# LinXueyuanStdio/LaTeX_OCR

Measured on AMD Instinct MI355X. Metric: formula-images/sec training step (batch 64, 128x512), higher is better.
Workload: dtype bf16

## Files before the change

### latex_ocr_amd/csrc/decoder_kernels.h

```cpp
#pragma once
#include "lxo_common.h"
struct Slabs { const float* p; int n; long long stride; int ld; };
struct Drop { unsigned thr; float inv_keep; unsigned seed; int t, row0, rows_total; };
struct DetScratch { float* p; size_t floats; };
int lxo_k_det_reduce(const float* part, int nslot, long long stride, int N, float* out, hipStream_t st);
int lxo_k_rowmean(int dt, const void* img, float* mean, int B, int R, int C, hipStream_t st);
int lxo_k_embed_gather(int dt, const float* table, const float* start, const int* formula, void* out, int B, int T, int D, int Dp, int V, hipStream_t st);
int lxo_k_embed_rows(int dt, const float* table, const float* start, const int* ids, void* out, int n, int D, int Dp, int V, hipStream_t st);
int lxo_k_embed_table(int dt, const float* table, const float* start, void* out, int V, int D, int Dp, hipStream_t st);
int lxo_k_lstm_fwd(const float* z, Slabs zs, const float* c_prev, float* gates, float* c_out, float* h_out, float* ht_out, int ldh, Drop dr, int B, int U, hipStream_t st);
int lxo_k_lstm_bwd(const float* gates, const float* c_prev, const float* c_cur, Slabs s1, Slabs s3, Slabs s4, int off4,
                   float* dcc, float* dz, Drop dr, int carry_rows, int B, int U, hipStream_t st);
int lxo_k_tanh_bwd(const float* a, int lda, Slabs carry, const float* o, int ldo, float* g, int ldg, void* gb, int ldgb, Drop dr, int carry_rows, int rows, int cols, hipStream_t st);
int lxo_k_slab_reduce(Slabs sl, float* o, int ldo, int rows, int cols, hipStream_t st);
int lxo_k_tanh_finalize(Slabs sl, float* o, int ldo, Drop dr, int rows, int cols, hipStream_t st);
int lxo_k_attn_fwd(int dt, const void* att_img, const void* img, const float* att_h, Slabs ahs, float* att_h_out, const float* beta, float* alpha, float* part,
                   float* ctx, int ldctx, void* ctxb, int ldcb, int nv, int R, int Rp, int E, int C, int beam, int nch, int rev, hipStream_t st, const void* att_exp = nullptr);
int lxo_k_att_exp(const void* att_img, void* att_exp, long long n, hipStream_t st);
int lxo_k_attn_bwd(int dt, const void* att_img, const void* att_exp, const void* img, const float* att_h, const float* beta, const float* alpha,
                   Slabs dcs, int dcoff, float* dctx_out, int lddc, const float* ctx, int ldctx, float* de, float* datth,
                   int nv, int R, int Rp, int E, int C, int nch, int rev, hipStream_t st);
int lxo_k_datt_img(int dt, const void* att_img, const float* att_h, const float* beta, const float* de, void* dout, float* dbeta,
                   int T, int B, int R, int Rp, int E, DetScratch det, hipStream_t st);
int lxo_k_add_mean_grad(float* dimg, const float* dmean, int B, int R, int C, hipStream_t st);
int lxo_k_ce_loss(int dt, const float* logits, const int* formula, const int* lengths, void* dlogits, float* loss_acc, float inv_ntok,
                  const float* ntok_dev, const unsigned* chain_err, int B, int T, int V, int Vp, DetScratch det, hipStream_t st);
int lxo_k_score(int dt, const float* logits, const int* formula, const int* lengths, float* logp_out, int* top1_out, float* seq_out,
                const unsigned* chain_err, int B, int T, int V, int Vp, hipStream_t st);
int lxo_k_colsum_det(const void* a, int bf16, long long lda, float* out, long long M, int N, DetScratch det, hipStream_t st);
int lxo_k_colsum(const float* a, long long lda, float* out, long long M, int N, DetScratch det, hipStream_t st);
int lxo_k_embed_scatter(const float* demb, const int* formula, float* dtable, float* dstart, int B, int T, int D, int V, int det, hipStream_t st);
int lxo_k_init_bwd(const float* dcc, Slabs dxh, const float* c0, const float* rec0, int ldr, float* dpre, int B, int U, int O, hipStream_t st);
struct DecPrefix { const int* ids; const int* len; int ld; int lim; };
struct DecAllow { const unsigned* bits; int ld; };
int lxo_k_argmax(const float* logits, int Vp, int V, int n, int id_end, int* ids_step, int* ids_out, int max_steps, int step,
                 int* finished, int* n_unfinished, hipStream_t st, float* logp_out = nullptr,
                 const DecPrefix* prefix = nullptr, const DecAllow* allow = nullptr);
int lxo_k_beam_step(float* logits, int Vp, int V, int nimg, int k, int id_end, int time, float div_gamma, float div_prob, int div_seed,
                    float* scratch, float* logp, int* finished,
                    int* ids_step, int* parents_step, int* ids_out, int* par_out, int max_steps, int* n_unfinished, hipStream_t st,
                    float* scores_out = nullptr,
                    const DecPrefix* prefix = nullptr, const DecAllow* allow = nullptr);
int lxo_k_beam_gather(float* rec, int ldr, int XH, float* cs, int U, const int* parents, int k, float* tmp_rec, float* tmp_cs, int n, void* recb, int ldrb, hipStream_t st);
int lxo_k_tile_rows(const float* src, int lds, float* dst, int ldd, int n, int k, int cols, hipStream_t st);
int lxo_k_global_norm_scale(long long n, const float* g, float clip, float* sumsq_tmp, float* out, hipStream_t st);
int lxo_k_chain_guard(const unsigned* err_fwd, const unsigned* err_bwd, const float* probe, float* scale, int have_scale, unsigned* status, hipStream_t st);
int lxo_k_chain_poison(const unsigned* err_fwd, const unsigned* err_bwd, float* probe, hipStream_t st);
int lxo_k_adam(float* p, const float* g, float* m, float* v, long long n, float lr_t, float b1, float b2, float eps, const float* scale, hipStream_t st);
int lxo_k_simple_opt(float* p, const float* g, float* slot, long long n, float lr, int mode, const float* scale, hipStream_t st);
```

### latex_ocr_amd/csrc/decoder_kernels.hip

```cpp
#include "decoder_kernels.h"
#include "api_util.h"
#include "drop.h"
#include <stdlib.h>

namespace {


LXO_DEV void load4(const float* p, float (&v)[4]) {
    f32x4 a = *reinterpret_cast<const f32x4*>(p);
    v[0] = a[0]; v[1] = a[1]; v[2] = a[2]; v[3] = a[3];
}
LXO_DEV void load4(const bf16_t* p, float (&v)[4]) {
    u32x2 a = *reinterpret_cast<const u32x2*>(p);
    v[0] = __uint_as_float(a[0] << 16); v[1] = __uint_as_float(a[0] & 0xffff0000u);
    v[2] = __uint_as_float(a[1] << 16); v[3] = __uint_as_float(a[1] & 0xffff0000u);
}
LXO_DEV void store4(float* p, const float (&v)[4]) { f32x4 a = {v[0], v[1], v[2], v[3]}; *reinterpret_cast<f32x4*>(p) = a; }
LXO_DEV void store4(bf16_t* p, const float (&v)[4]) { u32x2 a = {pack_bf2(v[0], v[1]), pack_bf2(v[2], v[3])}; *reinterpret_cast<u32x2*>(p) = a; }

LXO_DEV float slab_sum(const Slabs& sl, long long row, int col) {
    float v = 0.f;
    const float* q = sl.p + row * sl.ld + col;
    for (int s = 0; s < sl.n; ++s) v += q[(long long)s * sl.stride];
    return v;
// ... 108 lines not shown
        float cp = 0.f;
        if (ok) {
            cp = c_prev[(long long)b * U + u + q];
            const f32x4 zz = *reinterpret_cast<const f32x4*>(z + (long long)b * 4 * U + q * U + u) + slab_sum4(zs, b, q * U + u);
            f32x4 a;
#pragma unroll
            for (int e = 0; e < 4; ++e)
                a[e] = (q == 1) ? tanhf(zz[e]) : sigmoidf_(q == 2 ? zz[e] + 1.0f : zz[e]);
            if (gates) *reinterpret_cast<f32x4*>(gates + (long long)b * 4 * U + q * U + u) = a;
#pragma unroll
            for (int e = 0; e < 4; ++e) act[ugl][q][e] = a[e];
        }
        __syncthreads();
        if (ok) {
            const float gi = act[ugl][0][q], gj = act[ugl][1][q], gf = act[ugl][2][q], go = act[ugl][3][q];
            const float c = gf * cp + gi * gj;
            const float h = go * tanhf(c);
            c_out[(long long)b * U + u + q] = c;
            h_out[(long long)b * ldh + u + q] = h;
            ht_out[(long long)b * ldh + u + q] = h * drop_scale(dr, 1u, b, u + q, U);
        }
        __syncthreads();
    }
}

LXO_DEV f32x4 slab_part4(const Slabs& sl, long long row, int col, int q) {
    f32x4 v = {0.f, 0.f, 0.f, 0.f};
    const float* p = sl.p + row * sl.ld + col;
    for (int s0 = q; s0 < sl.n; s0 += 32) {
        f32x4 t[8];
#pragma unroll
        for (int j = 0; j < 8; ++j) {
            const f32x4 z = {0.f, 0.f, 0.f, 0.f};
            t[j] = (s0 + 4 * j < sl.n) ? *reinterpret_cast<const f32x4*>(p + (long long)(s0 + 4 * j) * sl.stride) : z;
        }
#pragma unroll
        for (int j = 0; j < 8; ++j) v += t[j];
    }
    return v;
}

__global__ __launch_bounds__(256) void lstm_bwd_kernel(const float* __restrict__ gates, const float* __restrict__ c_prev,
                                                      const float* __restrict__ c_cur, Slabs s1, Slabs s3, Slabs s4, int off4,
                                                      float* __restrict__ dcc, float* __restrict__ dz, Drop dr, int carry_rows,
                                                      int B, int U) {
    __shared__ float ex[64][4][8 + 1];
    const int total = B * (U >> 2);
    const int q = threadIdx.x & 3, ugl = threadIdx.x >> 2;
    for (int base = blockIdx.x * 64; base < total; base += gridDim.x * 64) {
        const int ug = base + ugl;
        const bool ok = ug < total;
        const int b = ok ? ug / (U >> 2) : 0, u = ok ? (ug - b * (U >> 2)) << 2 : 0;
        float gi = 0.f, gj = 0.f, gf = 0.f, go = 0.f, cc = 0.f, cp = 0.f, dci = 0.f;
        if (ok) {
            const float* gr = gates + (long long)b * 4 * U + u + q;
            gi = gr[0]; gj = gr[U]; gf = gr[2 * U]; go = gr[3 * U];
            cc = c_cur[(long long)b * U + u + q]; cp = c_prev[(long long)b * U + u + q]; dci = dcc[(long long)b * U + u + q];
            const f32x4 pm = slab_part4(s1, b, u, q) + slab_part4(s3, b, u, q);
            f32x4 pc = {0.f, 0.f, 0.f, 0.f};
            if (b < carry_rows) pc = slab_part4(s4, b, off4 + u, q);
#pragma unroll
            for (int e = 0; e < 4; ++e) { ex[ugl][q][e] = pm[e]; ex[ugl][q][4 + e] = pc[e]; }
        }
        __syncthreads();
        if (ok) {
            const float dhm = ex[ugl][0][q] + ex[ugl][1][q] + ex[ugl][2][q] + ex[ugl][3][q];
            const float dhc = ex[ugl][0][4 + q] + ex[ugl][1][4 + q] + ex[ugl][2][4 + q] + ex[ugl][3][4 + q];
            const float dh = dhm * drop_scale(dr, 1u, b, u + q, U) + dhc;
            const float tc = tanhf(cc);
            const float dc = dci + dh * go * (1.f - tc * tc);
            float* dzr = dz + (long long)b * 4 * U + u + q;
            dzr[0] = dc * gj * gi * (1.f - gi);
            dzr[U] = dc * gi * (1.f - gj * gj);
            dzr[2 * U] = dc * cp * gf * (1.f - gf);
            dzr[3 * U] = dh * tc * go * (1.f - go);
            dcc[(long long)b * U + u + q] = dc * gf;
        }
        __syncthreads();
    }
}

__global__ __launch_bounds__(256) void tanh_bwd_kernel(const float* __restrict__ a, int lda, Slabs carry,
                                                      const float* __restrict__ o, int ldo, float* __restrict__ g, int ldg,
                                                      bf16_t* __restrict__ gb, int ldgb, Drop dr, int carry_rows, int rows, int cols) {
    const int total = rows * (cols >> 2);
    for (int i = blockIdx.x * 256 + threadIdx.x; i < total; i += gridDim.x * 256) {
        const int r = i / (cols >> 2), c = (i - r * (cols >> 2)) << 2;
        const f32x4 ov = *reinterpret_cast<const f32x4*>(o + (long long)r * ldo + c);
        f32x4 d = *reinterpret_cast<const f32x4*>(a + (long long)r * lda + c);
        if (r < carry_rows) d += slab_sum4(carry, r, c);
        f32x4 out;
#pragma unroll
        for (int e = 0; e < 4; ++e) {
            const float sc = drop_scale(dr, 2u, r, c + e, cols);
            const float th = (dr.thr == 0u) ? ov[e] : ov[e] / dr.inv_keep;
            out[e] = d[e] * sc * (1.f - th * th);
        }
        *reinterpret_cast<f32x4*>(g + (long long)r * ldg + c) = out;
        if (gb) { u32x2 pk = {pack_bf2(out[0], out[1]), pack_bf2(out[2], out[3])}; *reinterpret_cast<u32x2*>(gb + (long long)r * ldgb + c) = pk; }
    }
}
__global__ __launch_bounds__(256) void tanh_finalize_kernel(Slabs sl, float* __restrict__ o, int ldo, Drop dr, int rows, int cols) {
    const int total = rows * (cols >> 2);
    for (int i = blockIdx.x * 256 + threadIdx.x; i < total; i += gridDim.x * 256) {
        const int r = i / (cols >> 2), c = (i - r * (cols >> 2)) << 2;
        const f32x4 v = slab_sum4(sl, r, c);
        f32x4 out;
#pragma unroll
        for (int e = 0; e < 4; ++e) out[e] = tanhf(v[e]) * drop_scale(dr, 2u, r, c + e, cols);
        *reinterpret_cast<f32x4*>(o + (long long)r * ldo + c) = out;
    }
}

constexpr int ATT_W = 8;

template <typename CT> LXO_DEV float tanh_ct(float x);
template <> LXO_DEV float tanh_ct<float>(float x) { return tanhf(x); }
template <> LXO_DEV float tanh_ct<bf16_t>(float x) { return 1.f - 2.f * __builtin_amdgcn_rcpf(__expf(2.f * x) + 1.f); }

template <typename CT, int KCT, int ATT_U>
__global__ __launch_bounds__(512) void attn_fwd_part_kernel(const CT* __restrict__ att_img, const CT* __restrict__ img,
                                                           const float* __restrict__ att_h, Slabs ahs, float* __restrict__ att_h_out,
                                                           const float* __restrict__ beta,
                                                           float* __restrict__ alpha, float* __restrict__ part,
                                                           int R, int Rp, int E, int C, int beam, int nch, int rows_per, int rev) {
    __shared__ float redc[ATT_W][512];
    __shared__ float red[2 * ATT_W];
    const int ch = blockIdx.x, v = blockIdx.y, bi = v / beam;
    const int tid = threadIdx.x, lane = tid & 63, wave = tid >> 6;
    const int r0 = ch * rows_per;
    const int n = min(R, r0 + rows_per) - r0;
    const CT* ai = att_img + ((long long)bi * R + r0) * E;
    const CT* im = img + ((long long)bi * R + r0) * C;
    float* pout = part + ((long long)v * nch + ch) * (C + 2);
    constexpr int KC = KCT;
    float ah[KCT][4], bt[KCT][4];
#pragma unroll
    for (int kc = 0; kc < KCT; ++kc) {
        const int k0 = kc * 256 + lane * 4;
#pragma unroll
        for (int j = 0; j < 4; ++j) { ah[kc][j] = 0.f; bt[kc][j] = 0.f; }
        if (kc < KC && k0 < E) {
            const f32x4 a4 = ahs.n > 0 ? slab_sum4(ahs, v, k0) : *reinterpret_cast<const f32x4*>(att_h + (long long)v * E + k0);
            const f32x4 b4 = *reinterpret_cast<const f32x4*>(beta + k0);
#pragma unroll
            for (int j = 0; j < 4; ++j) { ah[kc][j] = a4[j]; bt[kc][j] = b4[j]; }
            if (ahs.n > 0 && att_h_out && ch == 0 && wave == 0) *reinterpret_cast<f32x4*>(att_h_out + (long long)v * E + k0) = a4;
        }
    }
    const int c0 = lane * 8;
    const bool cok = c0 < C;
    float m = -3.0e38f, l = 0.f, acc[8];
#pragma unroll
    for (int e = 0; e < 8; ++e) acc[e] = 0.f;
    const int c0l = cok ? c0 : 0;
    const int nit = n > wave ? (n - wave + ATT_W * ATT_U - 1) / (ATT_W * ATT_U) : 0;
    for (int it = 0; it < nit; ++it) {
        const int base = wave + ATT_W * ATT_U * (rev ? nit - 1 - it : it);
        float xi[ATT_U][8], pt[ATT_U];
#pragma unroll
        for (int u = 0; u < ATT_U; ++u) {
            const int r = min(base + ATT_W * u, n - 1);
            load8(im + (long long)r * C + c0l, xi[u]);
            pt[u] = 0.f;
        }
#pragma unroll
        for (int kc = 0; kc < KCT; ++kc) {
// ... 702 lines not shown
                    const int t = t0 + tt, tc = min(t, T - 1);
                    load4(att_h + ((long long)tc * B + b) * E + k0, a[tt]);
                    f32x4 dq = *reinterpret_cast<const f32x4*>(de + ((long long)tc * B + b) * Rp + rbase);
#pragma unroll
                    for (int rr = 0; rr < 4; ++rr) d[tt][rr] = (t < T && rbase + rr < R) ? dq[rr] : 0.f;
                    if constexpr (is_bf16<CT>::value) {
#pragma unroll
                        for (int j = 0; j < 4; ++j) a[tt][j] = __builtin_amdgcn_exp2f(fminf(fmaxf(a[tt][j] * 2.8853900817779268f, -120.f), 120.f));
                    }
                }
#pragma unroll
                for (int tt = 0; tt < 4; ++tt) {
                    if (d[tt][0] == 0.f && d[tt][1] == 0.f && d[tt][2] == 0.f && d[tt][3] == 0.f) continue;
#pragma unroll
                    for (int rr = 0; rr < 4; ++rr) {
                        const float dd = d[tt][rr];
                        if constexpr (is_bf16<CT>::value) {
                            const f32x2 d4 = {4.f * dd, 4.f * dd}, d2 = {dd, dd}, one = {1.f, 1.f};
                            sumd += dd;
#pragma unroll
                            for (int h = 0; h < 2; ++h) {
                                const f32x2 xs = {x[rr][kc][2 * h], x[rr][kc][2 * h + 1]}, as = {a[tt][2 * h], a[tt][2 * h + 1]};
                                const f32x2 w = __builtin_elementwise_fma(xs, as, one);
                                const f32x2 r = {__builtin_amdgcn_rcpf(w[0]), __builtin_amdgcn_rcpf(w[1])};
                                const f32x2 q = __builtin_elementwise_fma(-r, r, r);
                                f32x2 ac = {acc[rr][kc][2 * h], acc[rr][kc][2 * h + 1]}, dv = {db[kc][2 * h], db[kc][2 * h + 1]};
                                ac = __builtin_elementwise_fma(d4, q, ac);
                                dv = __builtin_elementwise_fma(d2, r, dv);
                                acc[rr][kc][2 * h] = ac[0]; acc[rr][kc][2 * h + 1] = ac[1];
                                db[kc][2 * h] = dv[0]; db[kc][2 * h + 1] = dv[1];
                            }
                        } else {
#pragma unroll
                            for (int j = 0; j < 4; ++j) {
                                const float tau = tanh_ct<CT>(x[rr][kc][j] + a[tt][j]);
                                acc[rr][kc][j] = fmaf(dd, 1.f - tau * tau, acc[rr][kc][j]);
                                db[kc][j] = fmaf(dd, tau, db[kc][j]);
                            }
                        }
                    }
                }
            }
        }
    }
#pragma unroll
    for (int rr = 0; rr < 4; ++rr)
#pragma unroll
        for (int kc = 0; kc < KCT; ++kc) {
            const int k0 = kc * 256 + lane * 4;
            if (rbase + rr < R && kc < KC && k0 < E) {
                float o[4];
#pragma unroll
                for (int j = 0; j < 4; ++j) o[j] = acc[rr][kc][j] * bt[kc][j];
                store4(dout + ((long long)b * R + rbase + rr) * E + k0, o);
            }
        }
#pragma unroll
    for (int kc = 0; kc < KCT; ++kc) {
        const int k0 = kc * 256 + lane * 4;
        if (kc < KC && k0 < E) {
#pragma unroll
            for (int j = 0; j < 4; ++j) redb[wave][k0 + j] = is_bf16<CT>::value ? sumd - 2.f * db[kc][j] : db[kc][j];
        }
    }
    __syncthreads();
    if (dbeta_part) {
        float* slot = dbeta_part + ((long long)blockIdx.y * gridDim.x + blockIdx.x) * E;
        for (int k = tid; k < E; k += 256) slot[k] = redb[0][k] + redb[1][k] + redb[2][k] + redb[3][k];
        return;
    }
    for (int k = tid; k < E; k += 256) atomicAdd(&dbeta[k], redb[0][k] + redb[1][k] + redb[2][k] + redb[3][k]);
}

__global__ __launch_bounds__(256) void add_mean_grad_kernel(float* __restrict__ dimg, const float* __restrict__ dmean, int B, int R, int C) {
    const long long total = (long long)B * R * C;
    const float inv = 1.0f / (float)R;
    for (long long i = (long long)blockIdx.x * 256 + threadIdx.x; i < total; i += (long long)gridDim.x * 256) {
        const int c = (int)(i % C);
        const int b = (int)(i / ((long long)R * C));
        dimg[i] += dmean[(long long)b * C + c] * inv;
    }
}

template <typename CT>
__global__ __launch_bounds__(256) void ce_loss_kernel(const float* __restrict__ logits, const int* __restrict__ formula,
                                                     const int* __restrict__ lengths, CT* __restrict__ dlogits,
                                                     float* __restrict__ loss_acc, float* __restrict__ loss_part, float inv_ntok, const float* __restrict__ ntok_dev,
                                                     const unsigned* __restrict__ chain_err, int B, int T, int V, int Vp) {
    __shared__ float red[8];
    if (chain_err && blockIdx.x == 0 && threadIdx.x == 0 && chain_err[0] != 0u) atomicAdd(&loss_acc[0], __uint_as_float(0x7fc00000u));
    if (ntok_dev) inv_ntok = 1.0f / ntok_dev[0];
    const int lane = threadIdx.x & 63, wave = threadIdx.x >> 6;
    float ce_sum = 0.f, n_sum = 0.f;
    for (int row = blockIdx.x * 4 + wave; row < T * B; row += gridDim.x * 4) {
        const int t = row / B, b = row - t * B;
        const float* lg = logits + (long long)row * Vp;
        CT* dl = dlogits + (long long)row * Vp;
        const bool valid = t < lengths[b];
        int tgt = formula[(long long)b * T + t];
        tgt = tgt < 0 ? 0 : (tgt >= V ? V - 1 : tgt);
        float m = -3.0e38f;
        for (int j = lane; j < V; j += 64) m = fmaxf(m, lg[j]);
        m = wave_max(m);
        float l = 0.f;
        for (int j = lane; j < V; j += 64) l += expf(lg[j] - m);
        l = wave_sum(l);
        const float lse = m + logf(l);
        const float scale = valid ? inv_ntok : 0.f;
        for (int j = lane; j < Vp; j += 64) {
            float g = 0.f;
            if (j < V) g = (expf(lg[j] - lse) - (j == tgt ? 1.f : 0.f)) * scale;
            dl[j] = from_f32<CT>(g);
        }
        if (valid) { ce_sum += lse - lg[tgt]; n_sum += 1.0f; }
    }
    if (lane == 0) { red[wave] = ce_sum; red[4 + wave] = n_sum; }
    __syncthreads();
    if (threadIdx.x == 0) {
        const float c = red[0] + red[1] + red[2] + red[3], n = red[4] + red[5] + red[6] + red[7];
        if (loss_part) { loss_part[2 * blockIdx.x] = c; loss_part[2 * blockIdx.x + 1] = n; }
        else if (n > 0.f) { atomicAdd(&loss_acc[0], c); atomicAdd(&loss_acc[1], n); }
    }
}

template <typename CT, int KV>
__global__ __launch_bounds__(256) void ce_loss_rows_kernel(const float* __restrict__ logits, const int* __restrict__ formula,
                                                          const int* __restrict__ lengths, CT* __restrict__ dlogits,
                                                          float* __restrict__ loss_acc, float* __restrict__ loss_part, float inv_ntok, const float* __restrict__ ntok_dev,
                                                          const unsigned* __restrict__ chain_err, int B, int T, int V, int Vp) {
    __shared__ float red[8];
    if (chain_err && blockIdx.x == 0 && threadIdx.x == 0 && chain_err[0] != 0u) atomicAdd(&loss_acc[0], __uint_as_float(0x7fc00000u));
    if (ntok_dev) inv_ntok = 1.0f / ntok_dev[0];
    const int lane = threadIdx.x & 63, wave = threadIdx.x >> 6;
    float ce_sum = 0.f, n_sum = 0.f;
    for (int row = blockIdx.x * 4 + wave; row < T * B; row += gridDim.x * 4) {
        const int t = row / B, b = row - t * B;
        const float* lg = logits + (long long)row * Vp;
        CT* dl = dlogits + (long long)row * Vp;
        const bool valid = t < lengths[b];
        int tgt = formula[(long long)b * T + t];
        tgt = tgt < 0 ? 0 : (tgt >= V ? V - 1 : tgt);
        const float xt = lg[tgt];
        float x[KV];
#pragma unroll
        for (int q = 0; q < KV / 4; ++q) {
            const int j0 = 4 * (lane + 64 * q);
            const f32x4 v = *reinterpret_cast<const f32x4*>(lg + (j0 < Vp ? j0 : 0));
#pragma unroll
            for (int e = 0; e < 4; ++e) x[4 * q + e] = (j0 + e < V) ? v[e] : -3.0e38f;
        }
        float m = x[0];
#pragma unroll
        for (int e = 1; e < KV; ++e) m = fmaxf(m, x[e]);
        m = wave_max(m);
        float l = 0.f;
#pragma unroll
        for (int e = 0; e < KV; ++e) l += is_bf16<CT>::value ? __expf(x[e] - m) : expf(x[e] - m);
        l = wave_sum(l);
        const float lse = m + logf(l);
        const float scale = valid ? inv_ntok : 0.f;
#pragma unroll
        for (int q = 0; q < KV / 4; ++q) {
            const int j0 = 4 * (lane + 64 * q);
            if (j0 >= Vp) continue;
            float g[4];
#pragma unroll
            for (int e = 0; e < 4; ++e) {
                const int j = j0 + e;
                const float pr = is_bf16<CT>::value ? __expf(x[4 * q + e] - lse) : expf(x[4 * q + e] - lse);
                g[e] = j < V ? (pr - (j == tgt ? 1.f : 0.f)) * scale : 0.f;
            }
            if constexpr (is_bf16<CT>::value) { const u32x2 pk = {pack_bf2(g[0], g[1]), pack_bf2(g[2], g[3])}; *reinterpret_cast<u32x2*>(dl + j0) = pk; }
            else { const f32x4 gv = {g[0], g[1], g[2], g[3]}; *reinterpret_cast<f32x4*>(dl + j0) = gv; }
        }
        if (valid) { ce_sum += lse - xt; n_sum += 1.0f; }
    }
    if (lane == 0) { red[wave] = ce_sum; red[4 + wave] = n_sum; }
    __syncthreads();
    if (threadIdx.x == 0) {
        const float c = red[0] + red[1] + red[2] + red[3], n = red[4] + red[5] + red[6] + red[7];
        if (loss_part) { loss_part[2 * blockIdx.x] = c; loss_part[2 * blockIdx.x + 1] = n; }
        else if (n > 0.f) { atomicAdd(&loss_acc[0], c); atomicAdd(&loss_acc[1], n); }
    }
}

__global__ __launch_bounds__(256) void colsum_kernel(const float* __restrict__ a, int lda, float* __restrict__ out, int M, int N, int rows_per_block) {
    const int n = blockIdx.x * 256 + threadIdx.x;
    const int m0 = blockIdx.y * rows_per_block, m1 = min(M, m0 + rows_per_block);
    if (n >= N) return;
    float s = 0.f;
    for (int m = m0; m < m1; ++m) s += a[(long long)m * lda + n];
    atomicAdd(&out[n], s);
}

__global__ __launch_bounds__(256) void colsum4_kernel(const float* __restrict__ a, int lda, float* __restrict__ out, int M, int N, int rows_per_block) {
    __shared__ f32x4 red[4][64];
    const int cq = threadIdx.x & 63, ry = threadIdx.x >> 6;
    const int n = (blockIdx.x * 64 + cq) * 4;
    const int m0 = blockIdx.y * rows_per_block, m1 = min(M, m0 + rows_per_block);
    const int nl = n < N ? n : 0;
    f32x4 s = {0.f, 0.f, 0.f, 0.f};
    for (int mb = m0 + ry; mb < m1; mb += 32) {
        f32x4 v[8];
#pragma unroll
        for (int u = 0; u < 8; ++u) { const int m = min(mb + 4 * u, m1 - 1); v[u] = *reinterpret_cast<const f32x4*>(a + (long long)m * lda + nl); }
#pragma unroll
        for (int u = 0; u < 8; ++u) if (mb + 4 * u < m1) s += v[u];
    }
    red[ry][cq] = s;
    __syncthreads();
    if (ry == 0 && n < N) {
        const f32x4 t = red[0][cq] + red[1][cq] + red[2][cq] + red[3][cq];
#pragma unroll
        for (int e = 0; e < 4; ++e) atomicAdd(&out[n + e], t[e]);
    }
}


template <typename AT>
__global__ __launch_bounds__(256) void colsum_part_kernel(const AT* __restrict__ a, long long lda, float* __restrict__ part, long long M, int N, int rows_per) {
    const int n = blockIdx.x * 256 + threadIdx.x;
    const long long m0 = (long long)blockIdx.y * rows_per, m1 = m0 + rows_per < M ? m0 + rows_per : M;
    if (n >= N) return;
    float s = 0.f;
    for (long long mb = m0; mb < m1; mb += 8) {
        float v[8];
#pragma unroll
        for (int u = 0; u < 8; ++u) { const long long m = mb + u < m1 ? mb + u : m1 - 1; v[u] = to_f32(a[m * lda + n]); }
#pragma unroll
        for (int u = 0; u < 8; ++u) if (mb + u < m1) s += v[u];
    }
    part[(long long)blockIdx.y * N + n] = s;
}
__global__ __launch_bounds__(256) void det_reduce_kernel(const float* __restrict__ part, int nslot, long long stride, int N, float* __restrict__ out) {
    __shared__ float gs[16][16];
    const int c = threadIdx.x & 15, g = threadIdx.x >> 4;
    const int n = blockIdx.x * 16 + c;
    const int per = (nslot + 15) / 16;
    const int q0 = g * per, q1 = min(nslot, q0 + per);
    float s = 0.f;
    if (n < N) {
        for (int q = q0; q < q1; q += 8) {
            float v[8];
#pragma unroll
            for (int u = 0; u < 8; ++u) v[u] = part[(long long)min(q + u, q1 - 1) * stride + n];
#pragma unroll
            for (int u = 0; u < 8; ++u) if (q + u < q1) s += v[u];
        }
    }
    gs[g][c] = s;
    __syncthreads();
    if (g == 0 && n < N) {
        float tsum = gs[0][c];
#pragma unroll
        for (int k = 1; k < 16; ++k) tsum += gs[k][c];
        out[n] += tsum;
    }
}

__global__ __launch_bounds__(256) void embed_scatter_kernel(const float* __restrict__ demb, const int* __restrict__ formula,
                                                           float* __restrict__ dtable, float* __restrict__ dstart,
                                                           int B, int T, int D, int V) {
    const long long total = (long long)T * B * D;
    for (long long i = (long long)blockIdx.x * 256 + threadIdx.x; i < total; i += (long long)gridDim.x * 256) {
        const int d = (int)(i % D);
        const long long row = i / D;
        const int b = (int)(row % B), t = (int)(row / B);
        const float g = demb[i];
        if (t == 0) atomicAdd(&dstart[d], g);
        else {
            int id = formula[(long long)b * T + t - 1];
            id = id < 0 ? 0 : (id >= V ? V - 1 : id);
            atomicAdd(&dtable[(long long)id * D + d], g);
        }
    }
}

__global__ __launch_bounds__(256) void embed_scatter_rows_kernel(const float* __restrict__ demb, const int* __restrict__ formula,
                                                                float* __restrict__ dtable, float* __restrict__ dstart,
                                                                int B, int T, int D, int V, int det) {
    constexpr int CH = 2048;
    __shared__ int list[CH];
    __shared__ float part[256];
    __shared__ int cnt;
    __shared__ int wcnt[4];
    const int id = blockIdx.x;
    const int tid = threadIdx.x;
    const int rpw = 256 / D, r = tid / D, c = tid - r * D;
    float sum = 0.f;
    const int total = T * B;
    const int per = (total + (int)gridDim.y - 1) / (int)gridDim.y;
    const int s0 = blockIdx.y * per, s1 = min(total, s0 + per);
    for (int base = s0; base < s1; base += CH) {
        if (tid == 0) cnt = 0;
        __syncthreads();
        if (det) {
            for (int jb = base; jb < min(s1, base + CH); jb += 256) {
                const int j = jb + tid;
                int row = -1;
                if (j < min(s1, base + CH)) {
                    const int b = j / T, tt = j - b * T;
                    if (id == V) { if (j < B) row = j; }
                    else if (tt + 1 < T) { int tok = formula[j]; tok = tok < 0 ? 0 : (tok >= V ? V - 1 : tok); if (tok == id) row = (tt + 1) * B + b; }
                }
                const unsigned long long m = __ballot(row >= 0);
                const int lane = tid & 63, wv = tid >> 6;
                if (lane == 0) wcnt[wv] = __builtin_popcountll(m);
                __syncthreads();
                int off = cnt;
                for (int w = 0; w < wv; ++w) off += wcnt[w];
                if (row >= 0) list[off + __builtin_popcountll(m & ((1ull << lane) - 1ull))] = row;
                __syncthreads();
                if (tid == 0) cnt += wcnt[0] + wcnt[1] + wcnt[2] + wcnt[3];
                __syncthreads();
            }
        } else
        for (int j = base + tid; j < min(s1, base + CH); j += 256) {
            const int b = j / T, tt = j - b * T;
            if (id == V) { if (j < B) list[atomicAdd(&cnt, 1)] = j; continue; }
            if (tt + 1 >= T) continue;
            int tok = formula[j]; tok = tok < 0 ? 0 : (tok >= V ? V - 1 : tok);
            if (tok == id) list[atomicAdd(&cnt, 1)] = (tt + 1) * B + b;
        }
        __syncthreads();
        const int n = cnt;
        if (r < rpw) {
            for (int k = r; k < n; k += 4 * rpw) {
                float v[4];
#pragma unroll
                for (int u = 0; u < 4; ++u) { const int kk = min(k + u * rpw, n - 1); v[u] = demb[(long long)list[kk] * D + c]; }
#pragma unroll
                for (int u = 0; u < 4; ++u) if (k + u * rpw < n) sum += v[u];
            }
        }
        __syncthreads();
    }
    part[tid] = (r < rpw) ? sum : 0.f;
    __syncthreads();
    if (tid < D) {
        float t = 0.f;
// ... 555 lines not shown
    const float gn = sqrtf(ss);
    out[1] = gn;
    out[0] = clip > 0.f ? clip / fmaxf(gn, clip) : 1.0f;
}
__global__ void chain_guard_kernel(const unsigned* __restrict__ err_fwd, const unsigned* __restrict__ err_bwd, const float* __restrict__ probe,
                                   float* __restrict__ scale, int have_scale, unsigned* __restrict__ status) {
    const unsigned ef = err_fwd ? err_fwd[0] : 0u, eb = err_bwd ? err_bwd[0] : 0u;
    const float pv = probe ? probe[0] : 0.f;
    const bool drop = (ef | eb) != 0u || pv != pv;
    if (status) { status[0] = ef; status[1] = eb; status[2] = drop ? 1u : 0u; }
    scale[0] = drop ? __uint_as_float(0x7fc00000u) : (have_scale ? scale[0] : 1.0f);
}
__global__ void chain_poison_kernel(const unsigned* __restrict__ err_fwd, const unsigned* __restrict__ err_bwd, float* __restrict__ probe) {
    if ((err_fwd && err_fwd[0]) || (err_bwd && err_bwd[0])) probe[0] = __uint_as_float(0x7fc00000u);
}
__global__ __launch_bounds__(256) void adam_kernel(float* __restrict__ p, const float* __restrict__ g, float* __restrict__ m, float* __restrict__ v,
                                                  long long n, float lr_t, float b1, float b2, float eps, const float* __restrict__ scale) {
    const float sc = scale ? scale[0] : 1.0f;
    if (sc != sc) return;
    for (long long i = (long long)blockIdx.x * 256 + threadIdx.x; i < n; i += (long long)gridDim.x * 256) {
        const float gi = g[i] * sc;
        const float mi = b1 * m[i] + (1.f - b1) * gi;
        const float vi = b2 * v[i] + (1.f - b2) * gi * gi;
        m[i] = mi; v[i] = vi;
        p[i] -= lr_t * mi / (sqrtf(vi) + eps);
    }
}

__global__ __launch_bounds__(256) void simple_opt_kernel(float* __restrict__ p, const float* __restrict__ g, float* __restrict__ slot,
                                                        long long n, float lr, int mode, const float* __restrict__ scale) {
    const float sc = scale ? scale[0] : 1.0f;
    if (sc != sc) return;
    for (long long i = (long long)blockIdx.x * 256 + threadIdx.x; i < n; i += (long long)gridDim.x * 256) {
        const float gi = g[i] * sc;
        if (mode == 1) p[i] -= lr * gi;
        else if (mode == 2) { const float a = slot[i] + gi * gi; slot[i] = a; p[i] -= lr * gi / sqrtf(a); }
        else { const float ms = 0.9f * slot[i] + 0.1f * gi * gi; slot[i] = ms; p[i] -= lr * gi / sqrtf(ms + 1e-10f); }
    }
}

inline int grid1(long long items, int per_block = 256, int cap = 2048) {
    long long g = (items + per_block - 1) / per_block;
    return (int)(g < 1 ? 1 : (g > cap ? cap : g));
}
}

#define LAUNCH(kern, grid, ...) hipLaunchKernelGGL(kern, dim3(grid), dim3(256), 0, st, __VA_ARGS__)
#define BYCT(dt, kern, grid, ...) do { if ((dt) == LXO_BF16) LAUNCH((kern<bf16_t>), grid, __VA_ARGS__); else LAUNCH((kern<float>), grid, __VA_ARGS__); } while (0)
#define DONE return (int)hipGetLastError()

int lxo_k_rowmean(int dt, const void* img, float* mean, int B, int R, int C, hipStream_t st) {
    if (C % 64) return -2;
    if (dt == LXO_BF16) LAUNCH((rowmean_kernel<bf16_t>), dim3(C / 64, B), (const bf16_t*)img, mean, R, C);
    else LAUNCH((rowmean_kernel<float>), dim3(C / 64, B), (const float*)img, mean, R, C);
    DONE;
}
int lxo_k_embed_gather(int dt, const float* table, const float* start, const int* formula, void* out, int B, int T, int D, int Dp, int V, hipStream_t st) {
    const int g = grid1((long long)T * B * Dp);
    if (dt == LXO_BF16) LAUNCH((embed_gather_kernel<bf16_t>), g, table, start, formula, (bf16_t*)out, B, T, D, Dp, V);
    else LAUNCH((embed_gather_kernel<float>), g, table, start, formula, (float*)out, B, T, D, Dp, V);
    DONE;
}
int lxo_k_embed_rows(int dt, const float* table, const float* start, const int* ids, void* out, int n, int D, int Dp, int V, hipStream_t st) {
    const int g = grid1((long long)n * Dp);
    if (dt == LXO_BF16) LAUNCH((embed_rows_kernel<bf16_t>), g, table, start, ids, (bf16_t*)out, n, D, Dp, V);
    else LAUNCH((embed_rows_kernel<float>), g, table, start, ids, (float*)out, n, D, Dp, V);
    DONE;
}
int lxo_k_embed_table(int dt, const float* table, const float* start, void* out, int V, int D, int Dp, hipStream_t st) {
    const int g = grid1((long long)(V + 1) * Dp);
    if (dt == LXO_BF16) LAUNCH((embed_table_kernel<bf16_t>), g, table, start, (bf16_t*)out, V, D, Dp);
    else LAUNCH((embed_table_kernel<float>), g, table, start, (float*)out, V, D, Dp);
    DONE;
}
int lxo_k_lstm_fwd(const float* z, Slabs zs, const float* c_prev, float* gates, float* c_out, float* h_out, float* ht_out, int ldh, Drop dr, int B, int U, hipStream_t st) {
    LAUNCH(lstm_fwd_kernel, grid1((long long)B * U), z, zs, c_prev, gates, c_out, h_out, ht_out, ldh, dr, B, U);
    DONE;
}
int lxo_k_lstm_bwd(const float* gates, const float* c_prev, const float* c_cur, Slabs s1, Slabs s3, Slabs s4, int off4,
                   float* dcc, float* dz, Drop dr, int carry_rows, int B, int U, hipStream_t st) {
    LAUNCH(lstm_bwd_kernel, grid1((long long)B * U), gates, c_prev, c_cur, s1, s3, s4, off4, dcc, dz, dr, carry_rows, B, U);
    DONE;
}
int lxo_k_tanh_bwd(const float* a, int lda, Slabs carry, const float* o, int ldo, float* g, int ldg, void* gb, int ldgb, Drop dr, int carry_rows, int rows, int cols, hipStream_t st) {
    LAUNCH(tanh_bwd_kernel, grid1((long long)rows * cols / 4), a, lda, carry, o, ldo, g, ldg, (bf16_t*)gb, ldgb, dr, carry_rows, rows, cols);
    DONE;
}
__global__ __launch_bounds__(256) static void slab_reduce_kernel(Slabs sl, float* __restrict__ o, int ldo, int rows, int cols) {
    const int total = rows * (cols >> 2);
    for (int i = blockIdx.x * 256 + threadIdx.x; i < total; i += gridDim.x * 256) {
        const int r = i / (cols >> 2), c = (i - r * (cols >> 2)) << 2;
        *reinterpret_cast<f32x4*>(o + (long long)r * ldo + c) = slab_sum4(sl, r, c);
    }
}
int lxo_k_slab_reduce(Slabs sl, float* o, int ldo, int rows, int cols, hipStream_t st) {
    LAUNCH(slab_reduce_kernel, grid1((long long)rows * cols / 4), sl, o, ldo, rows, cols);
    DONE;
}
int lxo_k_tanh_finalize(Slabs sl, float* o, int ldo, Drop dr, int rows, int cols, hipStream_t st) {
    LAUNCH(tanh_finalize_kernel, grid1((long long)rows * cols / 4), sl, o, ldo, dr, rows, cols);
    DONE;
}
static int att_u(int rows_per) {
    static int forced = -1;
    if (forced < 0) { const char* e = getenv("LXO_ATT_U"); forced = e ? atoi(e) : 0; }
    if (forced == 7 || forced == 8) return forced;
    return (rows_per + 55) / 56 <= (rows_per + 63) / 64 ? 7 : 8;
}
int lxo_k_attn_fwd(int dt, const void* att_img, const void* img, const float* att_h, Slabs ahs, float* att_h_out, const float* beta, float* alpha, float* part,
                   float* ctx, int ldctx, void* ctxb, int ldcb, int nv, int R, int Rp, int E, int C, int beam, int nch, int rev, hipStream_t st, const void* att_exp) {
    if (E > 1024 || C > 512 || nch < 1 || nch > 32) return -2;
    const int rows_per = cdiv(R, nch);
    dim3 grid(nch, nv);
    static int split = -1;
    if (split < 0) { const char* e = getenv("LXO_ATT_SPLIT"); split = (e && e[0] == '1') ? 1 : 0; }
    const int epl = dt == LXO_BF16 ? 8 : 4;
    if (split && ahs.n == 0 && att_h && R <= 1024 && C % 64 == 0 && E % epl == 0 && E <= 64 * epl && ((E / epl) & (E / epl - 1)) == 0) {
        if (dt == LXO_BF16) {
            hipLaunchKernelGGL((attn_scores_kernel<bf16_t, 8>), grid, dim3(512), 0, st, (const bf16_t*)att_img, att_h, beta, part, R, Rp, E, beam, rows_per);
            hipLaunchKernelGGL((attn_ctx_kernel<bf16_t, 8>), dim3(C / 64, nv), dim3(512), 0, st, (const bf16_t*)img, part, alpha, ctx, ldctx, (bf16_t*)ctxb, ldcb, R, Rp, C, beam);
        } else {
            hipLaunchKernelGGL((attn_scores_kernel<float, 8>), grid, dim3(512), 0, st, (const float*)att_img, att_h, beta, part, R, Rp, E, beam, rows_per);
            hipLaunchKernelGGL((attn_ctx_kernel<float, 8>), dim3(C / 64, nv), dim3(512), 0, st, (const float*)img, part, alpha, ctx, ldctx, (bf16_t*)ctxb, ldcb, R, Rp, C, beam);
        }
        DONE;
    }
    static int beam_shared = -1;
    if (beam_shared < 0) { const char* e = getenv("LXO_ATT_BEAM_SHARED"); beam_shared = (e && e[0] == '0') ? 0 : 1; }
    if (beam_shared && (beam == 2 || beam == 3 || beam == 5 || (beam == 1 && att_exp && dt == LXO_BF16)) && ahs.n == 0 && att_h && E <= 256 && C <= 512 && nv % beam == 0) {
        const int nimg = nv / beam;
        int nb = cdiv(512, nimg);
        if (nb > 16) nb = 16;
        const int by_rows = R / 32 > 0 ? R / 32 : 1;
        if (nb > by_rows) nb = by_rows;
        const int need = cdiv(R, 1024);
        if (nb < need) nb = need;
        const int rpb = cdiv(R, nb);
        const dim3 gb(nb, nimg);
#define ABM(CT_, U_, NB_, X_, OCC_, AI_) hipLaunchKernelGGL((attn_fwd_part_beam_kernel<CT_, U_, NB_, X_, OCC_>), gb, dim3(512), 0, st, (const CT_*)(AI_), (const CT_*)img, att_h, beta, alpha, part, R, Rp, E, C, nb, rpb, rev)
        if (dt == LXO_BF16 && att_exp) { if (beam == 1) ABM(bf16_t, 4, 1, true, 4, att_exp); else if (beam == 2) ABM(bf16_t, 4, 2, true, 4, att_exp); else if (beam == 3) ABM(bf16_t, 4, 3, true, 4, att_exp); else ABM(bf16_t, 2, 5, true, 4, att_exp); }
        else if (dt == LXO_BF16) { if (beam == 2) ABM(bf16_t, 4, 2, false, 2, att_img); else if (beam == 3) ABM(bf16_t, 4, 3, false, 2, att_img); else ABM(bf16_t, 4, 5, false, 2, att_img); }
        else { if (beam == 2) ABM(float, 4, 2, false, 2, att_img); else if (beam == 3) ABM(float, 4, 3, false, 2, att_img); else ABM(float, 4, 5, false, 2, att_img); }
#undef ABM
        hipLaunchKernelGGL(attn_fwd_combine_kernel, dim3(4, nv), dim3(256), 0, st, part, alpha, ctx, ldctx, (bf16_t*)ctxb, ldcb, R, Rp, C, nb, rpb);
        DONE;
    }
#define AF_ARGS att_h, ahs, att_h_out, beta, alpha, part, R, Rp, E, C, beam, nch, rows_per, rev
    if (dt == LXO_BF16) {
        if (E <= 256) { if (att_u(rows_per) == 8) hipLaunchKernelGGL((attn_fwd_part_kernel<bf16_t, 1, 8>), grid, dim3(512), 0, st, (const bf16_t*)att_img, (const bf16_t*)img, AF_ARGS); else hipLaunchKernelGGL((attn_fwd_part_kernel<bf16_t, 1, 7>), grid, dim3(512), 0, st, (const bf16_t*)att_img, (const bf16_t*)img, AF_ARGS); }
        else { if (att_u(rows_per) == 8) hipLaunchKernelGGL((attn_fwd_part_kernel<bf16_t, 4, 8>), grid, dim3(512), 0, st, (const bf16_t*)att_img, (const bf16_t*)img, AF_ARGS); else hipLaunchKernelGGL((attn_fwd_part_kernel<bf16_t, 4, 7>), grid, dim3(512), 0, st, (const bf16_t*)att_img, (const bf16_t*)img, AF_ARGS); }
    } else {
        if (E <= 256) { if (att_u(rows_per) == 8) hipLaunchKernelGGL((attn_fwd_part_kernel<float, 1, 8>), grid, dim3(512), 0, st, (const float*)att_img, (const float*)img, AF_ARGS); else hipLaunchKernelGGL((attn_fwd_part_kernel<float, 1, 7>), grid, dim3(512), 0, st, (const float*)att_img, (const float*)img, AF_ARGS); }
        else { if (att_u(rows_per) == 8) hipLaunchKernelGGL((attn_fwd_part_kernel<float, 4, 8>), grid, dim3(512), 0, st, (const float*)att_img, (const float*)img, AF_ARGS); else hipLaunchKernelGGL((attn_fwd_part_kernel<float, 4, 7>), grid, dim3(512), 0, st, (const float*)att_img, (const float*)img, AF_ARGS); }
    }
#undef AF_ARGS
    hipLaunchKernelGGL(attn_fwd_combine_kernel, dim3(4, nv), dim3(256), 0, st, part, alpha, ctx, ldctx, (bf16_t*)ctxb, ldcb, R, Rp, C, nch, rows_per);
    DONE;
}
int lxo_k_att_exp(const void* att_img, void* att_exp, long long n, hipStream_t st) {
    if (n % 8) return -2;
    LAUNCH(att_exp_kernel, grid1(n / 8, 256, 4096), (const bf16_t*)att_img, (bf16_t*)att_exp, n / 8);
    DONE;
}
int lxo_k_attn_bwd(int dt, const void* att_img, const void* att_exp, const void* img, const float* att_h, const float* beta, const float* alpha,
                   Slabs dcs, int dcoff, float* dctx_out, int lddc, const float* ctx, int ldctx, float* de, float* datth,
                   int nv, int R, int Rp, int E, int C, int nch, int rev, hipStream_t st) {
    if (E > 1024 || C > 512 || nch < 1 || nch > 32) return -2;
    const int rows_per = cdiv(R, nch);
    dim3 grid(nch, nv);
    static int stream2 = -1;
    if (stream2 < 0) { const char* e = getenv("LXO_ATT_BWD2"); stream2 = (e && e[0] == '1') ? 1 : 0; }
    if (stream2 && dt == LXO_BF16 && E == 256 && C == 512 && dcs.n == 1 && lddc % 4 == 0 && ldctx % 4 == 0 && (long long)rows_per * 1024 < (1LL << 31)) {
        const float* dctx = dcs.p + dcoff;
        if (dctx_out) return -2;
        hipLaunchKernelGGL((attn_bwd_stream_kernel<4>), grid, dim3(512), 0, st, (const bf16_t*)att_img, (const bf16_t*)img, att_h, beta, alpha, dctx, dcs.ld,
                           ctx, ldctx, de, datth, R, Rp, rows_per, rev);
        DONE;
    }
#define AB_ARGS att_h, beta, alpha, dcs, dcoff, dctx_out, lddc, ctx, ldctx, de, datth, R, Rp, E, C, rows_per, rev
    if (dt == LXO_BF16 && att_exp && E <= 256) {
        if (att_u(rows_per) == 8) hipLaunchKernelGGL((attn_bwd_part_kernel<bf16_t, 1, 8, true>), grid, dim3(512), 0, st, (const bf16_t*)att_exp, (const bf16_t*)img, AB_ARGS);
        else hipLaunchKernelGGL((attn_bwd_part_kernel<bf16_t, 1, 7, true>), grid, dim3(512), 0, st, (const bf16_t*)att_exp, (const bf16_t*)img, AB_ARGS);
    } else if (dt == LXO_BF16) {
        if (E <= 256) { if (att_u(rows_per) == 8) hipLaunchKernelGGL((attn_bwd_part_kernel<bf16_t, 1, 8>), grid, dim3(512), 0, st, (const bf16_t*)att_img, (const bf16_t*)img, AB_ARGS); else hipLaunchKernelGGL((attn_bwd_part_kernel<bf16_t, 1, 7>), grid, dim3(512), 0, st, (const bf16_t*)att_img, (const bf16_t*)img, AB_ARGS); }
        else { if (att_u(rows_per) == 8) hipLaunchKernelGGL((attn_bwd_part_kernel<bf16_t, 4, 8>), grid, dim3(512), 0, st, (const bf16_t*)att_img, (const bf16_t*)img, AB_ARGS); else hipLaunchKernelGGL((attn_bwd_part_kernel<bf16_t, 4, 7>), grid, dim3(512), 0, st, (const bf16_t*)att_img, (const bf16_t*)img, AB_ARGS); }
    } else {
        if (E <= 256) { if (att_u(rows_per) == 8) hipLaunchKernelGGL((attn_bwd_part_kernel<float, 1, 8>), grid, dim3(512), 0, st, (const float*)att_img, (const float*)img, AB_ARGS); else hipLaunchKernelGGL((attn_bwd_part_kernel<float, 1, 7>), grid, dim3(512), 0, st, (const float*)att_img, (const float*)img, AB_ARGS); }
        else { if (att_u(rows_per) == 8) hipLaunchKernelGGL((attn_bwd_part_kernel<float, 4, 8>), grid, dim3(512), 0, st, (const float*)att_img, (const float*)img, AB_ARGS); else hipLaunchKernelGGL((attn_bwd_part_kernel<float, 4, 7>), grid, dim3(512), 0, st, (const float*)att_img, (const float*)img, AB_ARGS); }
    }
#undef AB_ARGS
    DONE;
}
int lxo_k_det_reduce(const float* part, int nslot, long long stride, int N, float* out, hipStream_t st) {
    if (nslot <= 0 || N <= 0) return 0;
    hipLaunchKernelGGL(det_reduce_kernel, dim3(cdiv(N, 16)), dim3(256), 0, st, part, nslot, stride, N, out);
    DONE;
}
int lxo_k_datt_img(int dt, const void* att_img, const float* att_h, const float* beta, const float* de, void* dout, float* dbeta,
                   int T, int B, int R, int Rp, int E, DetScratch det, hipStream_t st) {
    dim3 grid(cdiv(R, 16), B);
    if (E > 1024) return -2;
    float* part = nullptr;
    if (det.p) { if ((size_t)grid.x * grid.y * E > det.floats) return -6; part = det.p; }
    if (dt == LXO_BF16) {
        if (E <= 256) hipLaunchKernelGGL((datt_img_kernel<bf16_t, 1>), grid, dim3(256), 0, st, (const bf16_t*)att_img, att_h, beta, de, (bf16_t*)dout, dbeta, part, T, B, R, Rp, E);
        else hipLaunchKernelGGL((datt_img_kernel<bf16_t, 4>), grid, dim3(256), 0, st, (const bf16_t*)att_img, att_h, beta, de, (bf16_t*)dout, dbeta, part, T, B, R, Rp, E);
    } else {
        if (E <= 256) hipLaunchKernelGGL((datt_img_kernel<float, 1>), grid, dim3(256), 0, st, (const float*)att_img, att_h, beta, de, (float*)dout, dbeta, part, T, B, R, Rp, E);
        else hipLaunchKernelGGL((datt_img_kernel<float, 4>), grid, dim3(256), 0, st, (const float*)att_img, att_h, beta, de, (float*)dout, dbeta, part, T, B, R, Rp, E);
    }
    if (part) return lxo_k_det_reduce(part, (int)(grid.x * grid.y), E, E, dbeta, st);
    DONE;
}
int lxo_k_add_mean_grad(float* dimg, const float* dmean, int B, int R, int C, hipStream_t st) {
    LAUNCH(add_mean_grad_kernel, grid1((long long)B * R * C), dimg, dmean, B, R, C);
    DONE;
}
int lxo_k_ce_loss(int dt, const float* logits, const int* formula, const int* lengths, void* dlogits, float* loss_acc, float inv_ntok,
                  const float* ntok_dev, const unsigned* chain_err, int B, int T, int V, int Vp, DetScratch det, hipStream_t st) {
    int g = cdiv(T * B, 4);
    float* part = (det.p && det.floats >= 1024) ? det.p : nullptr;
    if (Vp % 4 == 0 && Vp <= 1024 && (((uintptr_t)logits | (uintptr_t)dlogits) & 15) == 0) {
        if (g > (part ? 512 : 2048)) g = part ? 512 : 2048;
#define CE_ROWS(CT_, KV_) LAUNCH((ce_loss_rows_kernel<CT_, KV_>), g, logits, formula, lengths, (CT_*)dlogits, loss_acc, part, inv_ntok, ntok_dev, chain_err, B, T, V, Vp)
        if (dt == LXO_BF16) { if (Vp <= 256) CE_ROWS(bf16_t, 4); else if (Vp <= 512) CE_ROWS(bf16_t, 8); else CE_ROWS(bf16_t, 16); }
        else { if (Vp <= 256) CE_ROWS(float, 4); else if (Vp <= 512) CE_ROWS(float, 8); else CE_ROWS(float, 16); }
#undef CE_ROWS
        if (part) return lxo_k_det_reduce(part, g, 2, 2, loss_acc, st);
        DONE;
    }
    if (g > 512) g = 512;
    if (dt == LXO_BF16) LAUNCH((ce_loss_kernel<bf16_t>), g, logits, formula, lengths, (bf16_t*)dlogits, loss_acc, part, inv_ntok, ntok_dev, chain_err, B, T, V, Vp);
    else LAUNCH((ce_loss_kernel<float>), g, logits, formula, lengths, (float*)dlogits, loss_acc, part, inv_ntok, ntok_dev, chain_err, B, T, V, Vp);
    if (part) return lxo_k_det_reduce(part, g, 2, 2, loss_acc, st);
    DONE;
}
int lxo_k_score(int dt, const float* logits, const int* formula, const int* lengths, float* logp_out, int* top1_out, float* seq_out,
                const unsigned* chain_err, int B, int T, int V, int Vp, hipStream_t st) {
    int g = cdiv(T * B, 4);
    if (Vp % 4 == 0 && Vp <= 1024 && ((uintptr_t)logits & 15) == 0) {
        if (g > 2048) g = 2048;
#define SC_ROWS(BF_, KV_) LAUNCH((score_rows_kernel<BF_, KV_>), g, logits, formula, lengths, logp_out, top1_out, chain_err, B, T, V, Vp)
        if (dt == LXO_BF16) { if (Vp <= 256) SC_ROWS(true, 4); else if (Vp <= 512) SC_ROWS(true, 8); else SC_ROWS(true, 16); }
        else { if (Vp <= 256) SC_ROWS(false, 4); else if (Vp <= 512) SC_ROWS(false, 8); else SC_ROWS(false, 16); }
#undef SC_ROWS
    } else {
        LAUNCH(score_kernel, g > 512 ? 512 : g, logits, formula, lengths, logp_out, top1_out, chain_err, B, T, V, Vp);
    }
    if (seq_out) LAUNCH(score_seq_kernel, cdiv(B, 256), logp_out, lengths, seq_out, chain_err, B, T);
    DONE;
}
int lxo_k_colsum_det(const void* a, int bf16, long long lda, float* out, long long M, int N, DetScratch det, hipStream_t st) {
    if (!det.p) return -6;
    if (M <= 0 || N <= 0) return 0;
    long long maxslots = (long long)(det.floats / (size_t)N);
    if (maxslots < 1) return -6;
    if (maxslots > 1024) maxslots = 1024;
    long long rows_per = (M + maxslots - 1) / maxslots;
    if (rows_per < 64) rows_per = 64;
    const int nrb = (int)((M + rows_per - 1) / rows_per);
    if (bf16) hipLaunchKernelGGL((colsum_part_kernel<bf16_t>), dim3(cdiv(N, 256), nrb), dim3(256), 0, st, (const bf16_t*)a, lda, det.p, M, N, (int)rows_per);
    else hipLaunchKernelGGL((colsum_part_kernel<float>), dim3(cdiv(N, 256), nrb), dim3(256), 0, st, (const float*)a, lda, det.p, M, N, (int)rows_per);
    return lxo_k_det_reduce(det.p, nrb, N, N, out, st);
}
int lxo_k_colsum(const float* a, long long lda, float* out, long long M, int N, DetScratch det, hipStream_t st) {
    if (det.p) return lxo_k_colsum_det(a, 0, lda, out, M, N, det, st);
    const int rpb = 64;
    if (N % 4 == 0 && lda % 4 == 0 && ((uintptr_t)a & 15) == 0 && M > 0)
        hipLaunchKernelGGL(colsum4_kernel, dim3(cdiv(N, 256), cdiv((int)M, rpb)), dim3(256), 0, st, a, (int)lda, out, (int)M, N, rpb);
    else
    hipLaunchKernelGGL(colsum_kernel, dim3(cdiv(N, 256), cdiv((int)M, rpb)), dim3(256), 0, st, a, (int)lda, out, (int)M, N, rpb);
    DONE;
}
int lxo_k_embed_scatter(const float* demb, const int* formula, float* dtable, float* dstart, int B, int T, int D, int V, int det, hipStream_t st) {
    if (D <= 256) { hipLaunchKernelGGL(embed_scatter_rows_kernel, dim3(V + 1, det ? 1 : 16), dim3(256), 0, st, demb, formula, dtable, dstart, B, T, D, V, det); DONE; }
    if (det) return -2;
    LAUNCH(embed_scatter_kernel, grid1((long long)T * B * D), demb, formula, dtable, dstart, B, T, D, V);
    DONE;
}
int lxo_k_init_bwd(const float* dcc, Slabs dxh, const float* c0, const float* rec0, int ldr, float* dpre, int B, int U, int O, hipStream_t st) {
    LAUNCH(init_bwd_kernel, grid1((long long)B * (2 * U + O)), dcc, dxh, c0, rec0, ldr, dpre, B, U, O);
    DONE;
}
#define DEC_VARIANT(KERNEL, grid, block, ...)                                                                         \
    do {                                                                                                               \
        if (prefix && allow) hipLaunchKernelGGL((KERNEL<true, true>), dim3(grid), dim3(block), 0, st, __VA_ARGS__);    \
        else if (prefix) hipLaunchKernelGGL((KERNEL<true, false>), dim3(grid), dim3(block), 0, st, __VA_ARGS__);       \
        else if (allow) hipLaunchKernelGGL((KERNEL<false, true>), dim3(grid), dim3(block), 0, st, __VA_ARGS__);        \
        else hipLaunchKernelGGL((KERNEL<false, false>), dim3(grid), dim3(block), 0, st, __VA_ARGS__);                  \
    } while (0)
int lxo_k_argmax(const float* logits, int Vp, int V, int n, int id_end, int* ids_step, int* ids_out, int max_steps, int step,
                 int* finished, int* n_unfinished, hipStream_t st, float* logp_out, const DecPrefix* prefix, const DecAllow* allow) {
    const DecPrefix pf = prefix ? *prefix : DecPrefix{};
    const DecAllow al = allow ? *allow : DecAllow{};
    DEC_VARIANT(argmax_kernel, cdiv(n, 4), 256, logits, Vp, V, n, id_end, ids_step, ids_out, max_steps, step, finished, n_unfinished, logp_out, pf, al);
    DONE;
}
int lxo_k_beam_step(float* logits, int Vp, int V, int nimg, int k, int id_end, int time, float div_gamma, float div_prob, int div_seed,
                    float* scratch, float* logp, int* finished,
                    int* ids_step, int* parents_step, int* ids_out, int* par_out, int max_steps, int* n_unfinished, hipStream_t st,
                    float* scores_out, const DecPrefix* prefix, const DecAllow* allow) {
    if (k > 16 || k > V) return -2;
    DivPen dp = {0.f, 0u, (unsigned)div_seed, scratch};
    if (div_gamma > 0.f && div_gamma != 1.f && div_prob > 0.f) {
        dp.log_gamma = logf(div_gamma);
        dp.thr = div_prob >= 1.f ? 16777216u : (unsigned)(div_prob * 16777216.0f);
    }
    static int fast = -1;
    if (fast < 0) { const char* e = getenv("LXO_BEAM_FAST"); fast = (e && e[0] == '0') ? 0 : 1; }
    const DecPrefix pf = prefix ? *prefix : DecPrefix{};
    const DecAllow al = allow ? *allow : DecAllow{};
    if (fast && dp.log_gamma == 0.f && (long long)k * V <= BS_TH * BS_NPT && k * BS_NW <= 64) {
        DEC_VARIANT(beam_step_fast_kernel, nimg, BS_TH, logits, Vp, V, k, id_end, time, logp, finished, ids_step, parents_step, ids_out, par_out, max_steps, n_unfinished, scores_out, pf, al);
    } else
        DEC_VARIANT(beam_step_kernel, nimg, 256, logits, Vp, V, k, id_end, time, dp, logp, finished, ids_step, parents_step, ids_out, par_out, max_steps, n_unfinished, scores_out, pf, al);
    DONE;
}
// ... 37 lines not shown
```

### latex_ocr_amd/csrc/model_decoder.hip

```cpp
#include "plan.h"
#include "impl.h"
#include "gemm.h"
#include "decoder_kernels.h"
#include "rstep.h"
#include "xdec.h"
#include "dimg.h"
#include "api_util.h"
#include "timing.h"

namespace {
int nt(const Plan& P, bool a_f32, bool c_f32, bool small, const void* A, int lda, const void* Bp, int ldb, void* C, int ldc,
       int M, int N, int K, const float* bias, int act, bool accumulate, hipStream_t st) {
    GemmNT g; memset(&g, 0, sizeof(g));
    g.A = A; g.Bp = Bp; g.C = C; g.M = M; g.N = N; g.K = K; g.lda = lda; g.ldb = ldb; g.ldc = ldc;
    g.bias = bias; g.act = act; g.alpha = 1.f; g.accumulate = accumulate ? 1 : 0; g.addend_rows = 1;
    if (P.s.dtype == LXO_F32) { a_f32 = true; c_f32 = true; }
    return lxo_launch_gemm_nt(P.s.dtype, a_f32, c_f32, small, g, st);
}
int tn(const Plan& P, bool a_f32, bool b_f32, const void* A, int lda, const void* B, int ldb, float* C, int ldc,
       int M, int I, int J, hipStream_t st, DetScratch det = DetScratch{nullptr, 0}) {
    GemmTN g; memset(&g, 0, sizeof(g));
    g.A = A; g.B = B; g.C = C; g.M = M; g.I = I; g.J = J; g.lda = lda; g.ldb = ldb; g.ldc = ldc;
    const int tiles = cdiv(I, 128) * cdiv(J, 128);
    int ns = cdiv(512, tiles);
    const int maxs = M / 64 > 0 ? M / 64 : 1;
    if (ns > maxs) ns = maxs;
    g.nsplit = ns < 1 ? 1 : ns; g.nbatch = 1; g.atomic = 1;
    if (P.bf && P.det()) { if (det.p) { g.det_slab = det.p; g.det_floats = det.floats; } else g.nsplit = 1; }
    if (P.s.dtype == LXO_F32) { a_f32 = true; b_f32 = true; }
    return lxo_launch_gemm_tn(P.s.dtype, a_f32, b_f32, g, st);
}
int slab(const Plan& P, const float* A, int lda, const void* Bp, int ldb, float* out, int M, int N, int K, hipStream_t st) {
    GemmNT g; memset(&g, 0, sizeof(g));
    g.A = A; g.Bp = Bp; g.M = M; g.N = N; g.K = K; g.lda = lda; g.ldb = ldb; g.ldc = N; g.alpha = 1.f; g.addend_rows = 1;
    return lxo_launch_gemm_slab(P.s.dtype, g, out, (long long)M * N, st);
}
Slabs view(const float* p, int K, int M, int N) { Slabs s = {p, K / 128, (long long)M * N, N}; return s; }
const Slabs kNoSlabs = {nullptr, 0, 0, 0};
}

static bool att_alternate() {
    static int v = -1;
    if (v < 0) { const char* e = getenv("LXO_ATT_ALT"); v = (e && atoi(e) == 0) ? 0 : 1; }
    return v == 1;
}
static bool fused_steps(const Plan& P);
static int rs_dense(const Plan& P, const float* A, int lda, const void* W, int ldw, float* out, int ldo, int M, int N, int K,
                    const float* bias, bool tanh_act, bool accumulate, hipStream_t st) {
    RStep a; memset(&a, 0, sizeof(a));
    a.M = M; a.N = N; a.K = K; a.U = P.s.U; a.O = P.s.O; a.zx_row = -1;
    a.A = A; a.lda = lda; a.W = W; a.ldw = ldw; a.out = out; a.ldo = ldo; a.bias = bias; a.accumulate = accumulate ? 1 : 0;
    a.epi = tanh_act ? RS_TANH_O : RS_PLAIN;
    a.dr.inv_keep = 1.f;
    return lxo_launch_rstep(P.s.dtype, 0, a, st);
}

static int attention_prepare(const Plan& P, const float* prm, const void* wp, void* ws, int beam, hipStream_t st) {
    const int B = P.s.B, C = P.s.C, E = P.s.E, U = P.s.U, O = P.s.O;
    RC(nt(P, false, false, false, P.ws<void>(ws, W_IMG), C, P.pk(wp, K_ATT_IMG_T), C, P.ws<void>(ws, W_ATT_IMG), E,
          B * P.R, E, C, nullptr, 0, false, st));
    RC(lxo_k_rowmean(P.s.dtype, P.ws<void>(ws, W_IMG), P.ws<float>(ws, W_MEAN), B, P.R, C, st));
    float* rec0 = P.ws<float>(ws, W_REC);
    float* cs0 = P.ws<float>(ws, W_CS);
    const char* wt = (const char*)P.pk(wp, K_INIT_T);
    float* mean = P.ws<float>(ws, W_MEAN);
    if (beam <= 1 && fused_steps(P)) {
        RC(rs_dense(P, mean, C, wt, C, cs0, U, B, U, C, prm + P.poff[P_BC0], true, false, st));
        RC(rs_dense(P, mean, C, wt + (size_t)U * C * P.esz, C, rec0 + O, P.REC, B, U, C, prm + P.poff[P_BH0], true, false, st));
        RC(rs_dense(P, mean, C, wt + (size_t)2 * U * C * P.esz, C, rec0, P.REC, B, O, C, prm + P.poff[P_BO0], true, false, st));
    } else if (beam <= 1) {
        RC(nt(P, true, true, true, mean, C, wt, C, cs0, U, B, U, C, prm + P.poff[P_BC0], 2, false, st));
        RC(nt(P, true, true, true, mean, C, wt + (size_t)U * C * P.esz, C, rec0 + O, P.REC, B, U, C, prm + P.poff[P_BH0], 2, false, st));
        RC(nt(P, true, true, true, mean, C, wt + (size_t)2 * U * C * P.esz, C, rec0, P.REC, B, O, C, prm + P.poff[P_BO0], 2, false, st));
    } else {
        float* tmp = P.ws<float>(ws, W_BEAM_TMP);
        float* tc = tmp; float* th = tmp + (size_t)B * U; float* to = th + (size_t)B * U;
        RC(nt(P, true, true, true, mean, C, wt, C, tc, U, B, U, C, prm + P.poff[P_BC0], 2, false, st));
        RC(nt(P, true, true, true, mean, C, wt + (size_t)U * C * P.esz, C, th, U, B, U, C, prm + P.poff[P_BH0], 2, false, st));
        RC(nt(P, true, true, true, mean, C, wt + (size_t)2 * U * C * P.esz, C, to, O, B, O, C, prm + P.poff[P_BO0], 2, false, st));
        RC(lxo_k_tile_rows(tc, U, cs0, U, B * beam, beam, U, st));
        RC(lxo_k_tile_rows(th, U, rec0 + O, P.REC, B * beam, beam, U, st));
        RC(lxo_k_tile_rows(to, O, rec0, P.REC, B * beam, beam, O, st));
    }
    return 0;
}

static thread_local hipStream_t g_side = nullptr;
static thread_local hipEvent_t g_ev_fork = nullptr, g_ev_join = nullptr;
int lxo_impl_set_side_stream(hipStream_t s) {
    g_side = s;
    if (s && !g_ev_fork) {
        HIPRC(hipEventCreateWithFlags(&g_ev_fork, hipEventDisableTiming));
        HIPRC(hipEventCreateWithFlags(&g_ev_join, hipEventDisableTiming));
    }
    return 0;
}
static int fork_side(hipStream_t st) { HIPRC(hipEventRecord(g_ev_fork, st)); HIPRC(hipStreamWaitEvent(g_side, g_ev_fork, 0)); return 0; }
static int join_side(hipStream_t st) { HIPRC(hipEventRecord(g_ev_join, g_side)); HIPRC(hipStreamWaitEvent(st, g_ev_join, 0)); return 0; }

static int cell_step(const Plan& P, const float* prm, const void* wp, void* ws, int r0, int nr, int beam,
                     const float* zx_t, const float* rec_prev, const float* cs_prev, float* rec_cur, float* cs_cur,
                     float* gates_t, float* atth_t, float* alpha_t, Drop dr, hipStream_t st) {
    const int C = P.s.C, E = P.s.E, U = P.s.U, O = P.s.O;
    const size_t r = (size_t)r0;
    float* s1 = P.ws<float>(ws, W_S_K1) + r * (P.XH / 128) * 4 * U;
    float* s2 = P.ws<float>(ws, W_S_K2) + r * (U / 128) * E;
    float* s4 = P.ws<float>(ws, W_S_K4) + r * (P.HC / 128) * O;
    zx_t += r * 4 * U; rec_prev += r * P.REC; cs_prev += r * U; rec_cur += r * P.REC; cs_cur += r * U;
    if (gates_t) gates_t += r * 4 * U;
    atth_t += r * E; alpha_t += r * P.Rp;
    const char* att_img = (const char*)P.ws<void>(ws, W_ATT_IMG) + (r / beam) * P.R * E * P.esz;
    const char* img = (const char*)P.ws<void>(ws, W_IMG) + (r / beam) * P.R * C * P.esz;
    float* part = P.ws<float>(ws, W_APART) + r * 32 * (C + 2);
    RC(slab(P, rec_prev, P.REC, P.pk(wp, K_LSTM_RT), P.ldRT, s1, nr, 4 * U, P.XH, st));
    RC(lxo_k_lstm_fwd(zx_t, view(s1, P.XH, nr, 4 * U), cs_prev, gates_t, cs_cur, rec_cur + O, rec_cur + P.OFF_HT, P.REC, dr, nr, U, st));
    RC(slab(P, rec_cur + P.OFF_HT, P.REC, P.pk(wp, K_ATT_H_T), P.ldAHT, s2, nr, E, U, st));
    RC(lxo_k_attn_fwd(P.s.dtype, att_img, img, nullptr, view(s2, U, nr, E), atth_t,
                      prm + P.poff[P_BETA], alpha_t, part, rec_cur + P.OFF_CTX, P.REC, nullptr, 0, nr, P.R, P.Rp, E, C, beam,
                      P.attn_chunks(nr), 0, st));
    RC(slab(P, rec_cur + P.OFF_HT, P.REC, P.pk(wp, K_OW_T), P.ldOWT, s4, nr, O, P.HC, st));
    RC(lxo_k_tanh_finalize(view(s4, P.HC, nr, O), rec_cur, P.REC, dr, nr, O, st));
    return 0;
}

static int cell_step_fused(const Plan& P, const float* prm, const void* wp, void* ws, int nr, int beam,
                           const float* zx_t, const float* rec_prev, const float* cs_prev, float* rec_cur, float* cs_cur,
                           const bf16_t* recb_prev, bf16_t* recb_cur,
                           float* gates_t, float* atth_t, float* alpha_t, Drop dr, hipStream_t st,
                           const int* zx_idx = nullptr, int zx_row = -1, const int* a_par = nullptr) {
    const int C = P.s.C, E = P.s.E, U = P.s.U, O = P.s.O;
    const bool bf = P.bf;
    const char* att_img = (const char*)P.ws<void>(ws, W_ATT_IMG);
    const char* img = (const char*)P.ws<void>(ws, W_IMG);
    float* part = P.ws<float>(ws, W_APART);
    RStep a; memset(&a, 0, sizeof(a));
    a.M = nr; a.U = U; a.O = O; a.dr = dr; a.zx_row = -1;
    RStep k1 = a;
    k1.A = bf ? (const void*)recb_prev : (const void*)rec_prev; k1.lda = bf ? P.RECB : P.REC;
    k1.W = P.pk(wp, K_LSTM_RT); k1.ldw = P.ldRT; k1.N = 4 * U; k1.K = P.XH; k1.epi = RS_LSTM_FWD;
    k1.zx = zx_t; k1.c_prev = cs_prev; k1.gates = gates_t; k1.c_out = cs_cur;
    k1.zx_idx = zx_idx; k1.zx_vocab = P.s.V; k1.zx_row = zx_row;
    k1.a_par = a_par; k1.a_k = beam;
    k1.out = rec_cur + O; k1.out2 = rec_cur + P.OFF_HT; k1.ldo = P.REC;
    if (bf) { k1.outb = recb_cur + O; k1.out2b = recb_cur + P.OFF_HT; k1.ldob = P.RECB; }
    RC(lxo_launch_rstep(P.s.dtype, bf, k1, st));
    RStep k2 = a;
    k2.A = bf ? (const void*)(recb_cur + P.OFF_HT) : (const void*)(rec_cur + P.OFF_HT); k2.lda = bf ? P.RECB : P.REC;
    k2.W = P.pk(wp, K_ATT_H_T); k2.ldw = P.ldAHT; k2.N = E; k2.K = U; k2.epi = RS_PLAIN;
    k2.out = atth_t; k2.ldo = E;
// ... 22 lines not shown
}
static bool fused_steps(const Plan& P) {
    if (P.s.step_kernels == 1) return false;
    const int ks[7] = {P.XH, P.s.U, P.HC, P.s.O, P.s.E, 4 * P.s.U, P.s.C};
    for (int k : ks) if (!rstep_k_ok(k, P.bf) || !rstep_k_ok(k, false)) return false;
    return true;
}
static int mirror_oh(const Plan& P, void* ws, size_t slot_rows, int rows, hipStream_t st) {
    if (!P.bf) return 0;
    return lxo_k_mirror(P.ws<float>(ws, W_REC) + slot_rows * P.REC, P.REC, P.ws<bf16_t>(ws, W_RECB) + slot_rows * P.RECB, P.RECB, rows, P.XH, st);
}

int lxo_impl_decoder_train_fwd(const Plan& P, const float* prm, const void* wp, void* ws, const int* formula, hipStream_t st) {
    const int B = P.s.B, T = P.s.T, U = P.s.U, O = P.s.O, E = P.s.E, D = P.s.D, V = P.s.V, C = P.s.C;
    RC(attention_prepare(P, prm, wp, ws, 1, st));
    if (P.att_exp()) RC(lxo_k_att_exp(P.ws<void>(ws, W_ATT_IMG), P.ws<void>(ws, W_ATT_EXP), (long long)B * P.R * E, st));
    RC(lxo_k_embed_gather(P.s.dtype, prm + P.poff[P_EMB], prm + P.poff[P_START], formula, P.ws<void>(ws, W_EMB_IN), B, T, D, P.Dp, V, st));
    float* zx = P.ws<float>(ws, W_ZX);
    RC(nt(P, false, true, false, P.ws<void>(ws, W_EMB_IN), P.Dp, P.pk(wp, K_LSTM_XT), P.Dp, zx, 4 * U, T * B, 4 * U, P.Dp,
          prm + P.poff[P_LSTM_B], 0, false, st));
    float* rec = P.ws<float>(ws, W_REC); float* cs = P.ws<float>(ws, W_CS);
    const bool dual = g_side != nullptr && B >= 2 && (B % 2) == 0;
    const int nh = dual ? 2 : 1;
    const bool fused = fused_steps(P) && !dual;
    bool chain_done = false;
    if (fused && P.bf && P.s.step_kernels == 0) {
        RC(mirror_oh(P, ws, 0, B, st));
        XDecFwd x; memset(&x, 0, sizeof(x));
        x.Wrt = (const bf16_t*)P.pk(wp, K_LSTM_RT); x.ldrt = P.ldRT;
        x.Wah = (const bf16_t*)P.pk(wp, K_ATT_H_T); x.ldah = P.ldAHT;
        x.Wow = (const bf16_t*)P.pk(wp, K_OW_T); x.ldow = P.ldOWT;
        x.beta = prm + P.poff[P_BETA];
        x.att_img = P.ws<bf16_t>(ws, W_ATT_IMG); x.img = P.ws<bf16_t>(ws, W_IMG);
        x.att_exp = P.att_exp() ? P.ws<bf16_t>(ws, W_ATT_EXP) : nullptr;
        x.zx = zx; x.rec = rec; x.recb = P.ws<bf16_t>(ws, W_RECB); x.cs = cs;
        x.gates = P.ws<float>(ws, W_GATES); x.atth = P.ws<float>(ws, W_ATTH); x.alpha = P.ws<float>(ws, W_ALPHA);
        x.part = P.ws<float>(ws, W_APART); x.sync = P.ws<unsigned>(ws, W_XSYNC);
        x.T = T; x.B = B; x.R = P.R; x.Rp = P.Rp; x.REC = P.REC; x.RECB = P.RECB;
        x.dr = P.drop(0, 0);
        LxoTimed tm("xdec_fwd", "chain", (double)T * B * P.R * (E + C) * P.esz, st);
        const int rc = lxo_launch_xdec_fwd(x, U, O, C, E, st);
        if (rc == 0) chain_done = true;
        else if (rc != -2) return rc < 0 ? rc : -rc;
    }
    if (P.bf && !chain_done) HIPRC(hipMemsetAsync(P.ws<unsigned>(ws, W_XSYNC), 0, kXDecSyncBytes, st));
    if (fused && !chain_done) {
        bf16_t* recb = P.ws<bf16_t>(ws, W_RECB);
        RC(mirror_oh(P, ws, 0, B, st));
        for (int t = 0; t < T; ++t) {
            const int nr = B;
            if (nr <= 0) break;
            RC(cell_step_fused(P, prm, wp, ws, nr, 1, zx + (size_t)t * B * 4 * U,
                               rec + (size_t)t * B * P.REC, cs + (size_t)t * B * U,
                               rec + (size_t)(t + 1) * B * P.REC, cs + (size_t)(t + 1) * B * U,
                               recb + (size_t)t * B * P.RECB, recb + (size_t)(t + 1) * B * P.RECB,
                               P.ws<float>(ws, W_GATES) + (size_t)t * B * 4 * U,
                               P.ws<float>(ws, W_ATTH) + (size_t)t * B * E,
                               P.ws<float>(ws, W_ALPHA) + (size_t)t * B * P.Rp, P.drop(t, 0), st));
        }
    }
    if (dual) RC(fork_side(st));
    for (int t = 0; t < T && !fused; ++t)
        for (int h = 0; h < nh; ++h) {
            const int hb = B / nh;
            if (hb <= 0) continue;
            RC(cell_step(P, prm, wp, ws, h * hb, hb, 1, zx + (size_t)t * B * 4 * U,
                         rec + (size_t)t * B * P.REC, cs + (size_t)t * B * U,
                         rec + (size_t)(t + 1) * B * P.REC, cs + (size_t)(t + 1) * B * U,
                         P.ws<float>(ws, W_GATES) + (size_t)t * B * 4 * U,
                         P.ws<float>(ws, W_ATTH) + (size_t)t * B * E,
                         P.ws<float>(ws, W_ALPHA) + (size_t)t * B * P.Rp, P.drop(t, h * hb), h ? g_side : st));
        }
    if (dual) RC(join_side(st));
    if (P.bf && fused)
        RC(nt(P, false, true, false, P.ws<bf16_t>(ws, W_RECB) + (size_t)B * P.RECB, P.RECB, P.pk(wp, K_YWO_T), O, P.ws<float>(ws, W_LOGITS), P.Vp,
              T * B, V, O, nullptr, 0, false, st));
    else
        RC(nt(P, true, true, false, rec + (size_t)B * P.REC, P.REC, P.pk(wp, K_YWO_T), O, P.ws<float>(ws, W_LOGITS), P.Vp,
              T * B, V, O, nullptr, 0, false, st));
    return 0;
}

int lxo_impl_ce_loss(const Plan& P, void* ws, const int* formula, const int* lengths, float inv_ntok, const float* ntok_dev, hipStream_t st) {
    HIPRC(hipMemsetAsync(P.ws<float>(ws, W_LOSS), 0, 64, st));
    RC(lxo_k_ce_loss(P.s.dtype, P.ws<float>(ws, W_LOGITS), formula, lengths, P.ws<void>(ws, W_DLOGITS), P.ws<float>(ws, W_LOSS),
                     inv_ntok, ntok_dev, P.bf ? P.ws<unsigned>(ws, W_XSYNC) + 8 * 64 : nullptr, P.s.B, P.s.T, P.s.V, P.Vp,
                     DetScratch{P.ws<float>(ws, W_DET), P.wbytes[W_DET] / 4}, st));
    return 0;
}

int lxo_impl_score_tokens(const Plan& P, void* ws, const int* formula, const int* lengths, float* logp_out, int* top1_out, float* seq_out, hipStream_t st) {
    return lxo_k_score(P.s.dtype, P.ws<float>(ws, W_LOGITS), formula, lengths, logp_out, top1_out, seq_out,
                       P.bf ? P.ws<unsigned>(ws, W_XSYNC) + 8 * 64 : nullptr, P.s.B, P.s.T, P.s.V, P.Vp, st);
}

hipStream_t lxo_impl_encoder_side_stream();
static thread_local hipEvent_t g_dbw_fork = nullptr, g_dbw_fork2 = nullptr, g_dbw_join = nullptr, g_dbw_init = nullptr;

int lxo_impl_decoder_train_bwd(const Plan& P, const float* prm, const void* wp, void* ws, const int* formula, float* grads,
                               int parts, hipStream_t st, bool defer_join, void* ready) {
    const int B = P.s.B, T = P.s.T, C = P.s.C, E = P.s.E, U = P.s.U, O = P.s.O, D = P.s.D, V = P.s.V;
    const int TB = T * B;
    auto gw = [&](int pid) { return grads + P.poff[pid]; };
    float* rec = P.ws<float>(ws, W_REC); float* cs = P.ws<float>(ws, W_CS);
    float* dolog = P.ws<float>(ws, W_DOLOG); float* gall = P.ws<float>(ws, W_G); float* dhc = P.ws<float>(ws, W_DHC);
    float* de = P.ws<float>(ws, W_DE); float* datth = P.ws<float>(ws, W_DATTH); float* dz = P.ws<float>(ws, W_DZ);
    float* dcc = P.ws<float>(ws, W_DCC);
    float* gates = P.ws<float>(ws, W_GATES); float* atth = P.ws<float>(ws, W_ATTH); float* alpha = P.ws<float>(ws, W_ALPHA);
    const void* dlog = P.ws<void>(ws, W_DLOGITS);
    const DetScratch det = P.det_scratch(ws);

    const bool dual = g_side != nullptr && B >= 2 && (B % 2) == 0;
    const bool fused = fused_steps(P) && !dual;
    if (parts & 1) {
        RC(nt(P, false, true, false, dlog, P.Vp, P.pk(wp, K_YWO), P.Vp, dolog, O, TB, O, P.Vp, nullptr, 0, false, st));
        if (P.bf && fused) RC(tn(P, false, false, P.ws<bf16_t>(ws, W_RECB) + (size_t)B * P.RECB, P.RECB, dlog, P.Vp, gw(P_YWO), V, TB, O, V, st, det));
        else RC(tn(P, true, false, rec + (size_t)B * P.REC, P.REC, dlog, P.Vp, gw(P_YWO), V, TB, O, V, st));
    }
    if ((parts & 1) && P.bf) RC(lxo_k_chain_poison(P.ws<unsigned>(ws, W_XSYNC) + 8 * 64, nullptr, grads + P.ptotal - 1, st));
    if (!(parts & 2)) return 0;

    const bool want_chain = fused && P.bf && P.s.step_kernels == 0;
    bool bwd_chain = false;
    auto zero_acc = [&]() -> int {
        HIPRC(hipMemsetAsync(dcc, 0, (size_t)B * U * 4, st));
        HIPRC(hipMemsetAsync(datth, 0, (size_t)TB * E * 4, st));
        return 0;
    };
    if (!want_chain) RC(zero_acc());
    if (P.bf && !want_chain) HIPRC(hipMemsetAsync(P.ws<unsigned>(ws, W_XSYNC) + kXDecBlockBytes / 4, 0, kXDecSyncBytes, st));
    const int nh = dual ? 2 : 1;
    float* dxh = P.ws<float>(ws, W_DXH);
    if (fused) {
        const bool bf = P.bf;
        bf16_t* gb = P.ws<bf16_t>(ws, W_GB); bf16_t* dzb = P.ws<bf16_t>(ws, W_DZB);
        float* carry_h = P.ws<float>(ws, W_CARRYH);
        const char* att_img = (const char*)P.ws<void>(ws, W_ATT_IMG);
        const char* img = (const char*)P.ws<void>(ws, W_IMG);
        const int t_last = T - 1, n_last = B;
        RC(lxo_k_tanh_bwd(dolog + (size_t)t_last * B * O, O, kNoSlabs, rec + (size_t)(t_last + 1) * B * P.REC, P.REC,
                          gall + (size_t)t_last * B * O, O, bf ? gb + (size_t)t_last * B * P.GBP : nullptr, P.GBP, P.drop(t_last, 0), 0, n_last, O, st));
        bool chain_done = false;
        if (want_chain) {
            XDecBwd x; memset(&x, 0, sizeof(x));
            x.Wow = (const bf16_t*)P.pk(wp, K_OW); x.ldow = P.ldOW;
            x.Wah = (const bf16_t*)P.pk(wp, K_ATT_H); x.ldah = P.ldAH;
            x.Wk = (const bf16_t*)P.pk(wp, K_LSTM) + (size_t)D * P.ldK; x.ldk = P.ldK;
            x.beta = prm + P.poff[P_BETA];
            x.att_img = (const bf16_t*)att_img; x.img = (const bf16_t*)img;
            x.att_exp = P.att_exp() ? P.ws<bf16_t>(ws, W_ATT_EXP) : nullptr;
            x.rec = rec; x.REC = P.REC; x.cs = cs; x.gates = gates; x.atth = atth; x.alpha = alpha; x.Rp = P.Rp;
            x.dolog = dolog; x.gall = gall; x.gb = gb; x.GBP = P.GBP; x.dhc = dhc; x.de = de; x.datth = datth; x.datthb = P.ws<bf16_t>(ws, W_DATTHB);
            x.dz = dz; x.dzb = dzb; x.DZBP = P.DZBP; x.carry_h = carry_h; x.dcc = dcc; x.dxh = dxh;
            x.part = P.ws<float>(ws, W_APART);
            x.sync = P.ws<unsigned>(ws, W_XSYNC) + kXDecBlockBytes / 4;
            x.T = T; x.B = B; x.R = P.R;
            x.dr = P.drop(0, 0);
            LxoTimed tm("xdec_bwd", "chain", (double)T * B * P.R * (E + C) * P.esz, st);
            const int rc = lxo_launch_xdec_bwd(x, U, O, C, E, st);
            if (rc == 0) chain_done = bwd_chain = true;
            else if (rc != -2) return rc < 0 ? rc : -rc;
            else { RC(zero_acc()); HIPRC(hipMemsetAsync(x.sync, 0, kXDecSyncBytes, st)); }
        }
        RStep a; memset(&a, 0, sizeof(a));
        a.U = U; a.O = O; a.zx_row = -1;
        for (int t = t_last; t >= 0 && !chain_done; --t) {
            const int nr = B;
            const int nchb = P.det() ? 1 : P.attn_chunks(nr);
            a.M = nr;
            const float* rec_cur = rec + (size_t)(t + 1) * B * P.REC;
            float* g_t = gall + (size_t)t * B * O;
            float* dhc_t = dhc + (size_t)t * B * P.HC;
            float* datth_t = datth + (size_t)t * B * E;
            float* dz_t = dz + (size_t)t * B * 4 * U;
            RStep b1 = a;
            b1.A = bf ? (const void*)(gb + (size_t)t * B * P.GBP) : (const void*)g_t; b1.lda = bf ? P.GBP : O;
            b1.W = P.pk(wp, K_OW); b1.ldw = P.ldOW; b1.N = P.HC; b1.K = O; b1.epi = RS_PLAIN;
            b1.out = dhc_t; b1.ldo = P.HC;
            RC(lxo_launch_rstep(P.s.dtype, bf, b1, st));
            const Slabs dc1 = {dhc_t, 1, 0, P.HC};
            {
            LxoTimed tm("attn_bwd", "part", (double)nr * P.R * (E + C) * P.esz, st);
            RC(lxo_k_attn_bwd(P.s.dtype, att_img, P.att_exp() ? P.ws<void>(ws, W_ATT_EXP) : nullptr, img, atth + (size_t)t * B * E, prm + P.poff[P_BETA],
                              alpha + (size_t)t * B * P.Rp, dc1, U, nullptr, P.HC, rec_cur + P.OFF_CTX, P.REC,
                              de + (size_t)t * B * P.Rp, datth_t, nr, P.R, P.Rp, E, C, nchb, att_alternate() ? (t & 1) : 0, st));
            }
            RStep b3 = a;
            b3.A = datth_t; b3.lda = E;
            b3.W = P.pk(wp, K_ATT_H); b3.ldw = P.ldAH; b3.N = U; b3.K = E; b3.epi = RS_LSTM_BWD;
            b3.dhm = dhc_t; b3.lddhm = P.HC; b3.carry_h = carry_h; b3.carry_rows = (t == t_last) ? 0 : B;
            b3.gates_in = gates + (size_t)t * B * 4 * U; b3.c_prev = cs + (size_t)t * B * U; b3.c_cur = cs + (size_t)(t + 1) * B * U;
            b3.dcc = dcc; b3.out = dz_t; b3.outb = bf ? dzb + (size_t)t * B * P.DZBP : nullptr; b3.ldob = P.DZBP; b3.dr = P.drop(t, 0);
            RC(lxo_launch_rstep(P.s.dtype, 0, b3, st));
            RStep b4 = a;
            b4.A = bf ? (const void*)(dzb + (size_t)t * B * P.DZBP) : (const void*)dz_t; b4.lda = bf ? P.DZBP : 4 * U;
            b4.W = (const char*)P.pk(wp, K_LSTM) + (size_t)D * P.ldK * P.esz; b4.ldw = P.ldK; b4.N = P.XH; b4.K = 4 * U; b4.epi = RS_CARRY;
            if (t == 0) { b4.first = 1; b4.out = dxh; b4.ldo = P.XH; }
            else {
                b4.M = B;
                b4.out = gall + (size_t)(t - 1) * B * O; b4.outb = bf ? gb + (size_t)(t - 1) * B * P.GBP : nullptr; b4.ldob = P.GBP; b4.out2 = carry_h;
                b4.dolog = dolog + (size_t)(t - 1) * B * O; b4.o_prev = rec + (size_t)t * B * P.REC; b4.ldoprev = P.REC;
                b4.dr = P.drop(t - 1, 0);
            }
            RC(lxo_launch_rstep(P.s.dtype, bf, b4, st));
        }
    }
    if (dual) RC(fork_side(st));
    for (int t = T - 1; t >= 0 && !fused; --t) {
        for (int h = 0; h < nh; ++h) {
            const int hb = B / nh;
            if (hb <= 0) continue;
            const int crows = (t == T - 1) ? 0 : hb;
            const int nchb = P.det() ? 1 : P.attn_chunks(hb);
            hipStream_t sh = h ? g_side : st;
            const size_t r0 = (size_t)h * hb;
            float* sb1 = P.ws<float>(ws, W_S_B1) + r0 * (O / 128) * P.HC;
            float* sb3 = P.ws<float>(ws, W_S_B3) + r0 * (E / 128) * U;
            float* sb4 = P.ws<float>(ws, W_S_B4) + r0 * (4 * U / 128) * P.XH;
            const float* rec_cur = rec + ((size_t)(t + 1) * B + r0) * P.REC;
            float* g_t = gall + ((size_t)t * B + r0) * O;
            float* dhc_t = dhc + ((size_t)t * B + r0) * P.HC;
            const char* att_img = (const char*)P.ws<void>(ws, W_ATT_IMG) + r0 * P.R * E * P.esz;
            const char* img = (const char*)P.ws<void>(ws, W_IMG) + r0 * P.R * C * P.esz;
            const Slabs carry = (crows <= 0) ? kNoSlabs : view(sb4, 4 * U, crows, P.XH);
// ... 397 lines not shown
```

### latex_ocr_amd/csrc/rstep.h

```cpp
#pragma once
#include "lxo_common.h"
#include "decoder_kernels.h"

enum RStepEpi {
    RS_PLAIN = 0,
    RS_TANH_O = 1,
    RS_LSTM_FWD = 2,
    RS_LSTM_BWD = 3,
    RS_CARRY = 4,
};

struct RStep {
    const void* A; int lda;
    const void* W; int ldw;
    int M, N, K, epi;
    int U, O;
    float* out; int ldo;
    bf16_t* outb; int ldob;
    float* out2; bf16_t* out2b;
    const float* zx; const float* c_prev; float* gates; float* c_out;
    const int* a_par; int a_k;
    const int* zx_idx; int zx_vocab, zx_row;
    const float* dhm; int lddhm; const float* carry_h; const float* gates_in; const float* c_cur; float* dcc; int carry_rows;
    const float* bias; int accumulate;
    const float* dolog; const float* o_prev; int ldoprev; int first;
    Drop dr;
    unsigned long long* dbg;
};

int lxo_launch_rstep(int dt, int a_bf16, const RStep& p, hipStream_t st);
#include "lxo_debug.h"
int lxo_k_mirror(const float* src, int lds, void* dst, int ldd, int rows, int cols, hipStream_t st);
```

### latex_ocr_amd/csrc/rstep.hip

```cpp
#include "rstep.h"
#include "drop.h"
#include "api_util.h"

namespace {

typedef __attribute__((ext_vector_type(4))) float v4f;

LXO_DEV v4f mfma16_bf16(u32x4 a, u32x4 b, v4f c) {
    return __builtin_amdgcn_mfma_f32_16x16x32_bf16(__builtin_bit_cast(bf16x8_t, a), __builtin_bit_cast(bf16x8_t, b), c, 0, 0, 0);
}

template <bool FAST> LXO_DEV float tanh_e(float x) {
    if constexpr (FAST) return 1.f - 2.f * __builtin_amdgcn_rcpf(__builtin_amdgcn_exp2f(x * 2.8853900817779268f) + 1.f);
    else return tanhf(x);
}
template <bool FAST> LXO_DEV float sigm_e(float x) {
    if constexpr (FAST) return __builtin_amdgcn_rcpf(1.f + __builtin_amdgcn_exp2f(x * -1.4426950408889634f));
    else return sigmoidf_(x);
}

LXO_DEV u32x4 frag8(const bf16_t* p) { return *reinterpret_cast<const u32x4*>(p); }
LXO_DEV u32x4 frag8(const float* p) {
    const f32x4 a = *reinterpret_cast<const f32x4*>(p), b = *reinterpret_cast<const f32x4*>(p + 4);
    u32x4 r = {pack_bf2(a[0], a[1]), pack_bf2(a[2], a[3]), pack_bf2(b[0], b[1]), pack_bf2(b[2], b[3])};
    return r;
}

LXO_DEV void st4(float* p, const float (&v)[4]) { f32x4 a = {v[0], v[1], v[2], v[3]}; *reinterpret_cast<f32x4*>(p) = a; }
LXO_DEV void st4b(bf16_t* p, const float (&v)[4]) { u32x2 a = {pack_bf2(v[0], v[1]), pack_bf2(v[2], v[3])}; *reinterpret_cast<u32x2*>(p) = a; }
LXO_DEV void ld4(const float* p, float (&v)[4]) { const f32x4 a = *reinterpret_cast<const f32x4*>(p); v[0] = a[0]; v[1] = a[1]; v[2] = a[2]; v[3] = a[3]; }

template <typename AT, typename WT, int EPI, int MT, int KC, int NCH, int NBUF>
__global__ __launch_bounds__(256) void rstep_kernel(const void* kA, const void* kW, int k_lda, int k_ldw, int k_M, int k_N, int k_K, int k_U, const int* k_apar, int k_ak, RStep p) {
    constexpr bool BF = is_bf16<WT>::value;
    constexpr int RB = MT / 16;
    constexpr int PITCH = KC + (BF ? 8 : 4);
    constexpr int APL = 16 / (int)sizeof(AT), WPL = 16 / (int)sizeof(WT);
    constexpr int PRA = KC / APL, PRW = KC / WPL;
    constexpr int NA = (MT * PRA) / 64, NW = (16 * PRW) / 64;
    constexpr int KSTEP = BF ? 32 : 16, NS = KC / KSTEP;
    static_assert(NW >= 1 && NA >= 1, "chunk too small");
    __shared__ __attribute__((aligned(16))) WT lds[4][(MT + 16) * PITCH];
    __shared__ float red[4][MT][16 + 1];
    const int tid = threadIdx.x, lane = tid & 63, wave = tid >> 6;
    const int r = lane & 15, g = lane >> 4;
    const int m0 = blockIdx.y * MT;
    const int kq = k_K >> 2;
    WT* As = lds[wave];
    WT* Ws = lds[wave] + MT * PITCH;
    const AT* __restrict__ Ag = reinterpret_cast<const AT*>(kA) + wave * kq;
    const WT* __restrict__ Wg = reinterpret_cast<const WT*>(kW) + wave * kq;
    int aoff[NA], woff[NW];
#pragma unroll
    for (int j = 0; j < NA; ++j) {
        const int i = j * 64 + lane, row = i / PRA, pc = i - row * PRA;
        int m = m0 + row;
        if (m >= k_M) m = k_M - 1;
        if (k_apar) m = (m / k_ak) * k_ak + k_apar[m];
        aoff[j] = m * k_lda + pc * APL;
    }
#pragma unroll
    for (int j = 0; j < NW; ++j) {
        const int i = j * 64 + lane, row = i / PRW, pc = i - row * PRW;
        int nb;
        if constexpr (EPI == RS_LSTM_FWD) nb = (row >> 2) * k_U + blockIdx.x * 4 + (row & 3);
        else nb = blockIdx.x * 16 + row;
        if (nb >= k_N) nb = k_N - 1;
        woff[j] = nb * k_ldw + pc * WPL;
    }
    u32x4 ra[NBUF][NA], rw[NBUF][NW];
#define ISSUE(buf, c) do { const int kb_ = (c) * KC; \
        _Pragma("unroll") for (int j = 0; j < NW; ++j) rw[buf][j] = *reinterpret_cast<const u32x4*>(Wg + woff[j] + kb_); \
        _Pragma("unroll") for (int j = 0; j < NA; ++j) ra[buf][j] = *reinterpret_cast<const u32x4*>(Ag + aoff[j] + kb_); } while (0)
#define STAMP(i) do { if (p.dbg && tid == 0) p.dbg[((long long)blockIdx.y * gridDim.x + blockIdx.x) * 8 + (i)] = __builtin_readcyclecounter(); } while (0)
#pragma unroll
    for (int b = 0; b < NBUF; ++b) if (b < NCH) ISSUE(b, b);
    STAMP(0);

    constexpr int ETH = MT * 4;
    const int row = (tid >> 2) % MT, part = tid & 3;
    const int m = m0 + row;
    const bool mok = m < p.M && tid < ETH;
    const int mc = m < p.M ? m : p.M - 1;
    const int n = blockIdx.x * 16 + part * 4;
    float pz[4] = {0.f, 0.f, 0.f, 0.f}, pcp = 0.f;
    float e0[4], e1[4], e2[4], e3[4], e4[4], e5[4], e6[4], e7[4], e8[4];
    if constexpr (EPI == RS_LSTM_FWD) {
        const int U = p.U, u = blockIdx.x * 4 + part;
        long long zr = mc;
        if (p.zx_idx) { int id = p.zx_idx[mc]; id = id < 0 ? 0 : (id >= p.zx_vocab ? p.zx_vocab - 1 : id); zr = id; }
        else if (p.zx_row >= 0) zr = p.zx_row;
#pragma unroll
        for (int q = 0; q < 4; ++q) pz[q] = p.zx[zr * 4 * U + q * U + u];
        pcp = p.c_prev[(long long)(k_apar ? (mc / k_ak) * k_ak + k_apar[mc] : mc) * U + u];
    } else if constexpr (EPI == RS_LSTM_BWD) {
        const int U = p.U;
        const float* gr = p.gates_in + (long long)mc * 4 * U + n;
        ld4(p.dhm + (long long)mc * p.lddhm + n, e0);
        ld4(p.carry_h + (long long)mc * U + n, e1);
        if (mc >= p.carry_rows) { e1[0] = e1[1] = e1[2] = e1[3] = 0.f; }
        ld4(gr, e2); ld4(gr + U, e3); ld4(gr + 2 * U, e4); ld4(gr + 3 * U, e5);
        ld4(p.c_cur + (long long)mc * U + n, e6); ld4(p.c_prev + (long long)mc * U + n, e7); ld4(p.dcc + (long long)mc * U + n, e8);
    } else if constexpr (EPI == RS_CARRY) {
        if (!p.first && n < p.O) {
            ld4(p.dolog + (long long)mc * p.O + n, e0);
            ld4(p.o_prev + (long long)mc * p.ldoprev + n, e1);
        }
    }
    __builtin_amdgcn_sched_barrier(0);
    STAMP(1);

    v4f acc[RB];
#pragma unroll
    for (int rb = 0; rb < RB; ++rb) acc[rb] = v4f{0.f, 0.f, 0.f, 0.f};
#pragma unroll
    for (int c = 0; c < NCH; ++c) {
        constexpr int dummy = 0; (void)dummy;
        const int b = c % NBUF;
#pragma unroll
        for (int j = 0; j < NW; ++j) {
            const int i = j * 64 + lane, trow = i / PRW, pc = i - trow * PRW;
            *reinterpret_cast<u32x4*>(&Ws[trow * PITCH + pc * WPL]) = rw[b][j];
        }
#pragma unroll
        for (int j = 0; j < NA; ++j) {
            const int i = j * 64 + lane, trow = i / PRA, pc = i - trow * PRA;
            if constexpr (sizeof(AT) == sizeof(WT)) {
                *reinterpret_cast<u32x4*>(&As[trow * PITCH + pc * APL]) = ra[b][j];
            } else {
                const f32x4 f = __builtin_bit_cast(f32x4, ra[b][j]);
                u32x2 v = {pack_bf2(f[0], f[1]), pack_bf2(f[2], f[3])};
                *reinterpret_cast<u32x2*>(&As[trow * PITCH + pc * APL]) = v;
            }
        }
        __builtin_amdgcn_wave_barrier();
        if (c == 0) STAMP(2);
        if (c + NBUF < NCH) ISSUE(b, c + NBUF);
#pragma unroll
        for (int s = 0; s < NS; ++s) {
            if constexpr (BF) {
                const u32x4 bw = *reinterpret_cast<const u32x4*>(&Ws[r * PITCH + s * 32 + g * 8]);
#pragma unroll
                for (int rb = 0; rb < RB; ++rb)
                    acc[rb] = mfma16_bf16(*reinterpret_cast<const u32x4*>(&As[(rb * 16 + r) * PITCH + s * 32 + g * 8]), bw, acc[rb]);
            } else {
                const f32x4 bw = *reinterpret_cast<const f32x4*>(&Ws[r * PITCH + s * 16 + g * 4]);
                f32x4 aw[RB];
#pragma unroll
                for (int rb = 0; rb < RB; ++rb) aw[rb] = *reinterpret_cast<const f32x4*>(&As[(rb * 16 + r) * PITCH + s * 16 + g * 4]);
#pragma unroll
                for (int e = 0; e < 4; ++e)
#pragma unroll
                    for (int rb = 0; rb < RB; ++rb)
                        acc[rb] = __builtin_amdgcn_mfma_f32_16x16x4f32(aw[rb][e], bw[e], acc[rb], 0, 0, 0);
            }
        }
        __builtin_amdgcn_wave_barrier();
        if (c == 0) STAMP(3);
    }
#undef ISSUE
    STAMP(4);
#pragma unroll
    for (int rb = 0; rb < RB; ++rb)
#pragma unroll
        for (int i = 0; i < 4; ++i) red[wave][rb * 16 + g * 4 + i][r] = acc[rb][i];
    __syncthreads();
    STAMP(5);
    if (!mok) return;

    if constexpr (EPI == RS_LSTM_FWD) {
        const int U = p.U, u = blockIdx.x * 4 + part;
        float a[4];
#pragma unroll
        for (int q = 0; q < 4; ++q) {
            const float z = pz[q] + red[0][row][q * 4 + part] + red[1][row][q * 4 + part] + red[2][row][q * 4 + part] + red[3][row][q * 4 + part];
            a[q] = (q == 1) ? tanh_e<BF>(z) : sigm_e<BF>(q == 2 ? z + 1.0f : z);
        }
        const float c = a[2] * pcp + a[0] * a[1];
        const float h = a[3] * tanh_e<BF>(c);
        const float ht = h * drop_scale(p.dr, 1u, m, u, U);
        if (p.gates) {
#pragma unroll
            for (int q = 0; q < 4; ++q) p.gates[(long long)m * 4 * U + q * U + u] = a[q];
        }
        p.c_out[(long long)m * U + u] = c;
        p.out[(long long)m * p.ldo + u] = h;
        p.out2[(long long)m * p.ldo + u] = ht;
        if (p.outb) { p.outb[(long long)m * p.ldob + u] = f2bf(h); p.out2b[(long long)m * p.ldob + u] = f2bf(ht); }
        STAMP(6);
        return;
    } else {
        if (n >= p.N) return;
        float v[4];
#pragma unroll
        for (int e = 0; e < 4; ++e) v[e] = red[0][row][part * 4 + e] + red[1][row][part * 4 + e] + red[2][row][part * 4 + e] + red[3][row][part * 4 + e];
        if constexpr (EPI == RS_PLAIN || EPI == RS_TANH_O) {
            if (p.bias) { float b4[4]; ld4(p.bias + n, b4); for (int e = 0; e < 4; ++e) v[e] += b4[e]; }
            if (p.accumulate) { float o4[4]; ld4(p.out + (long long)m * p.ldo + n, o4); for (int e = 0; e < 4; ++e) v[e] += o4[e]; }
        }
        if constexpr (EPI == RS_PLAIN) {
            st4(p.out + (long long)m * p.ldo + n, v);
            if (p.outb) st4b(p.outb + (long long)m * p.ldob + n, v);
        } else if constexpr (EPI == RS_TANH_O) {
#pragma unroll
            for (int e = 0; e < 4; ++e) v[e] = tanh_e<BF>(v[e]) * drop_scale(p.dr, 2u, m, n + e, p.N);
            st4(p.out + (long long)m * p.ldo + n, v);
            if (p.outb) st4b(p.outb + (long long)m * p.ldob + n, v);
        } else if constexpr (EPI == RS_LSTM_BWD) {
            const int U = p.U;
            float dzi[4], dzj[4], dzf[4], dzo[4], dcn[4];
#pragma unroll
            for (int e = 0; e < 4; ++e) {
                const float dh = (e0[e] + v[e]) * drop_scale(p.dr, 1u, m, n + e, U) + e1[e];
                const float tc = tanh_e<BF>(e6[e]);
                const float dc = e8[e] + dh * e5[e] * (1.f - tc * tc);
                dzi[e] = dc * e3[e] * e2[e] * (1.f - e2[e]);
                dzj[e] = dc * e2[e] * (1.f - e3[e] * e3[e]);
                dzf[e] = dc * e7[e] * e4[e] * (1.f - e4[e]);
                dzo[e] = dh * tc * e5[e] * (1.f - e5[e]);
                dcn[e] = dc * e4[e];
            }
            float* dzr = p.out + (long long)m * 4 * U + n;
            st4(dzr, dzi); st4(dzr + U, dzj); st4(dzr + 2 * U, dzf); st4(dzr + 3 * U, dzo);
            if (p.outb) {
                bf16_t* db = p.outb + (long long)m * p.ldob + n;
                st4b(db, dzi); st4b(db + U, dzj); st4b(db + 2 * U, dzf); st4b(db + 3 * U, dzo);
            }
            st4(p.dcc + (long long)m * U + n, dcn);
        } else if constexpr (EPI == RS_CARRY) {
            const int O = p.O;
            if (p.first) { st4(p.out + (long long)m * p.ldo + n, v); STAMP(6); return; }
            if (n < O) {
#pragma unroll
                for (int e = 0; e < 4; ++e) {
                    const float sc = drop_scale(p.dr, 2u, m, n + e, O);
                    const float th = (p.dr.thr == 0u) ? e1[e] : e1[e] / p.dr.inv_keep;
                    v[e] = (e0[e] + v[e]) * sc * (1.f - th * th);
                }
                st4(p.out + (long long)m * O + n, v);
                if (p.outb) st4b(p.outb + (long long)m * p.ldob + n, v);
            } else {
                st4(p.out2 + (long long)m * p.U + (n - O), v);
            }
        }
        STAMP(6);
    }
}

template <typename AT, typename WT, int EPI, int MT, int KC>
int launch_nch(const RStep& p, dim3 grid, hipStream_t st) {
    const int nch = (p.K / 4) / KC;
    switch (nch) {
    case 1: hipLaunchKernelGGL((rstep_kernel<AT, WT, EPI, MT, KC, 1, 1>), grid, dim3(256), 0, st, p.A, p.W, p.lda, p.ldw, p.M, p.N, p.K, p.U, p.a_par, p.a_k > 0 ? p.a_k : 1, p); break;
    case 2: hipLaunchKernelGGL((rstep_kernel<AT, WT, EPI, MT, KC, 2, 2>), grid, dim3(256), 0, st, p.A, p.W, p.lda, p.ldw, p.M, p.N, p.K, p.U, p.a_par, p.a_k > 0 ? p.a_k : 1, p); break;
    case 4: hipLaunchKernelGGL((rstep_kernel<AT, WT, EPI, MT, KC, 4, 4>), grid, dim3(256), 0, st, p.A, p.W, p.lda, p.ldw, p.M, p.N, p.K, p.U, p.a_par, p.a_k > 0 ? p.a_k : 1, p); break;
    case 8: hipLaunchKernelGGL((rstep_kernel<AT, WT, EPI, MT, KC, 8, 4>), grid, dim3(256), 0, st, p.A, p.W, p.lda, p.ldw, p.M, p.N, p.K, p.U, p.a_par, p.a_k > 0 ? p.a_k : 1, p); break;
    case 16: hipLaunchKernelGGL((rstep_kernel<AT, WT, EPI, MT, KC, 16, 4>), grid, dim3(256), 0, st, p.A, p.W, p.lda, p.ldw, p.M, p.N, p.K, p.U, p.a_par, p.a_k > 0 ? p.a_k : 1, p); break;
    default: return -2;
    }
    return (int)hipGetLastError();
}
template <typename AT, typename WT, int EPI>
int launch_ch(const RStep& p, hipStream_t st) {
    constexpr bool BF = is_bf16<WT>::value;
    constexpr int K0 = (BF && sizeof(AT) == 2) ? 64 : 32;
    constexpr int KMIN = BF ? 32 : 16;
    const int kq = p.K / 4;
    const int ncol = EPI == RS_LSTM_FWD ? p.U / 4 : cdiv(p.N, 16);
    const bool half = ((long long)ncol * cdiv(p.M, 64) <= 128 && p.M > 32) || (p.M > 64 && p.M <= 512);
    static int q16 = -1;
    if (q16 < 0) { const char* e = getenv("LXO_RSTEP_MT16"); q16 = (e && e[0] == '0') ? 0 : 1; }
    const bool quarter = q16 && (long long)ncol * cdiv(p.M, 32) <= 128 && p.M > 16;
    if (kq % K0 == 0) {
        if (quarter) return launch_nch<AT, WT, EPI, 16, K0>(p, dim3(ncol, cdiv(p.M, 16)), st);
        if (half) return launch_nch<AT, WT, EPI, 32, K0>(p, dim3(ncol, cdiv(p.M, 32)), st);
        return launch_nch<AT, WT, EPI, 64, K0>(p, dim3(ncol, cdiv(p.M, 64)), st);
    }
    if constexpr (K0 / 2 >= KMIN) {
        if (kq % (K0 / 2) == 0) return launch_nch<AT, WT, EPI, 64, K0 / 2>(p, dim3(ncol, cdiv(p.M, 64)), st);
    }
    return -2;
}

template <int EPI>
int launch_epi(int dt, bool a_bf16, const RStep& p, hipStream_t st) {
    if (dt == LXO_F32) return launch_ch<float, float, EPI>(p, st);
    return a_bf16 ? launch_ch<bf16_t, bf16_t, EPI>(p, st) : launch_ch<float, bf16_t, EPI>(p, st);
}

__global__ __launch_bounds__(256) void mirror_kernel(const float* __restrict__ src, int lds, bf16_t* __restrict__ dst, int ldd, int rows, int cols) {
    const int total = rows * (cols >> 2);
    for (int i = blockIdx.x * 256 + threadIdx.x; i < total; i += gridDim.x * 256) {
        const int r = i / (cols >> 2), c = (i - r * (cols >> 2)) << 2;
        float v[4];
        ld4(src + (long long)r * lds + c, v);
        st4b(dst + (long long)r * ldd + c, v);
    }
}

}

static thread_local unsigned long long* g_dbg = nullptr;
static thread_local int g_dbg_epi = -1;
extern "C" int lxo_rstep_debug(unsigned long long* buf, int epi) { g_dbg = buf; g_dbg_epi = epi; return 0; }
int lxo_launch_rstep(int dt, int a_bf16, const RStep& p0, hipStream_t st) {
    RStep p = p0;
    p.dbg = (g_dbg && p.epi == g_dbg_epi) ? g_dbg : nullptr;
    if (p.M <= 0 || p.N <= 0) return 0;
    if (p.K % 128 != 0 || p.lda % 8 != 0 || p.ldw % 8 != 0 || p.N % 4 != 0) return -2;
    if (p.epi == RS_LSTM_FWD && (p.U % 4 != 0 || p.N != 4 * p.U)) return -2;
    switch (p.epi) {
    case RS_PLAIN: return launch_epi<RS_PLAIN>(dt, a_bf16 != 0, p, st);
    case RS_TANH_O: return launch_epi<RS_TANH_O>(dt, a_bf16 != 0, p, st);
    case RS_LSTM_FWD: return launch_epi<RS_LSTM_FWD>(dt, a_bf16 != 0, p, st);
    case RS_LSTM_BWD: return launch_epi<RS_LSTM_BWD>(dt, a_bf16 != 0, p, st);
    case RS_CARRY: return launch_epi<RS_CARRY>(dt, a_bf16 != 0, p, st);
    default: return -2;
    }
}

int lxo_k_mirror(const float* src, int lds, void* dst, int ldd, int rows, int cols, hipStream_t st) {
    if (rows <= 0 || cols <= 0) return 0;
    if (cols % 4 != 0 || lds % 4 != 0 || ldd % 4 != 0) return -2;
    int g = cdiv(rows * (cols >> 2), 256);
    if (g > 1024) g = 1024;
    hipLaunchKernelGGL(mirror_kernel, dim3(g), dim3(256), 0, st, src, lds, (bf16_t*)dst, ldd, rows, cols);
    return (int)hipGetLastError();
}
```

### latex_ocr_amd/csrc/xdec.h

```cpp
#pragma once
#include "lxo_common.h"
#include "decoder_kernels.h"
#include "lxo_debug.h"

struct XDecFwd {
    const bf16_t* Wrt; int ldrt;
    const bf16_t* Wah; int ldah;
    const bf16_t* Wow; int ldow;
    const float* beta;
    const bf16_t* att_img;
    const bf16_t* att_exp;
    const bf16_t* img;
    const float* zx;
    float* rec; bf16_t* recb;
    float* cs;
    float* gates;
    float* atth;
    float* alpha;
    float* part;
    unsigned* sync;
    int T, B, R, Rp, REC, RECB;
    Drop dr;
    unsigned long long* dbg;
};

int lxo_launch_xdec_fwd(const XDecFwd& p, int U, int O, int C, int E, hipStream_t st);

struct XDecDec {
    const bf16_t* Wrt; int ldrt; const bf16_t* Wah; int ldah; const bf16_t* Wow; int ldow;
    const bf16_t* Wyo; int ldyo;
    const float* beta;
    const bf16_t* att_exp;
    const bf16_t* img;
    const float* tx;
    float* rec; bf16_t* recb;
    float* cs;
    float* part;
    unsigned* sync;
    int* ids_step;
    int* ids_out;
    int* finished;
    int* unfinished;
    int* stop;
    int B, R, REC, RECB, V, id_end, t0, nsteps, max_steps;
    float* logp_out;
    const int* prefix;
    const int* prefix_len;
    int prefix_ld, prefix_lim;
    const unsigned* allow;
    int allow_ld;
};
int lxo_launch_xdec_dec(const XDecDec& p, int U, int O, int C, int E, hipStream_t st);

struct XDecBwd {
    const bf16_t* Wow; int ldow;
    const bf16_t* Wah; int ldah;
    const bf16_t* Wk; int ldk;
    const float* beta;
    const bf16_t* att_img; const bf16_t* att_exp; const bf16_t* img;
    const float* rec; int REC;
    const float* cs; const float* gates; const float* atth; const float* alpha; int Rp;
    const float* dolog;
    float* gall; bf16_t* gb; int GBP;
    float* dhc;
    float* de;
    float* datth;
    bf16_t* datthb;
    float* dz; bf16_t* dzb; int DZBP;
    float* carry_h;
    float* dcc;
    float* dxh;
    float* part;
    unsigned* sync;
    int T, B, R;
    Drop dr;
    unsigned long long* dbg;
};
int lxo_launch_xdec_bwd(const XDecBwd& p, int U, int O, int C, int E, hipStream_t st);
constexpr size_t kXDecSyncBytes = 4096, kXDecLLBytes = 384u << 10, kXDecBlockBytes = kXDecSyncBytes + kXDecLLBytes;
constexpr size_t kLLFwdHt = 0, kLLFwdAh = 128u << 10, kLLFwdO = 256u << 10;
constexpr size_t kLLBwdGb = 0, kLLBwdDctx = 128u << 10;
```

### latex_ocr_amd/csrc/xdec.hip

```cpp
#include "xdec.h"
#include "drop.h"
#include "api_util.h"
#include <stdlib.h>

#ifdef LXO_HIPSIM
int lxo_launch_xdec_fwd(const XDecFwd&, int, int, int, int, hipStream_t) { return -2; }
int lxo_launch_xdec_bwd(const XDecBwd&, int, int, int, int, hipStream_t) { return -2; }
int lxo_launch_xdec_dec(const XDecDec&, int, int, int, int, hipStream_t) { return -2; }
extern "C" int lxo_xdec_debug(unsigned long long*) { return 0; }
extern "C" int lxo_xdec_debug_bwd(unsigned long long*) { return 0; }
#else

HIP_DYNAMIC_SHARED(char, xdec_dyn_lds)

namespace {
constexpr int XU = 512, XO = 512, XC = 512, XE = 256;
constexpr int XXH = XO + XU, XHC = XU + XC;
constexpr int OFF_H = XO, OFF_HT = XO + XU, OFF_CTX = XO + 2 * XU;
constexpr int XW = 8;
#ifndef LXO_XDEC_LLMASK
#define LXO_XDEC_LLMASK 15
#endif
constexpr int kLL = LXO_XDEC_LLMASK;
#ifndef LXO_XDEC_LLMASK_B
// ... 919 lines not shown
                            p.ids_out[(long long)bb * p.max_steps + (tg - 1)] = vi;
                            if constexpr (SC) p.logp_out[(long long)bb * p.max_steps + (tg - 1)] = (PF && fr >= 0) ? (vf - v) - logf(sr) : -logf(sr);
                            p.ids_step[bb] = vi;
                            const int fo = p.finished[bb] | (vi == p.id_end && fr < 0 ? 1 : 0);
                            p.finished[bb] = fo;
                            unf_l[row] = fo ? 0 : 1;
                        }
                    }
                }
                __syncthreads();
                if (rank == 0 && tid == 0) {
                    int cnt = 0;
#pragma unroll
                    for (int r = 0; r < NB; ++r) cnt += unf_l[r];
                    atomicAdd(p.unfinished + (t - 1), cnt | 0x10000);
                    if (t >= 2) {
                        const int w = __hip_atomic_load(p.unfinished + (t - 2), __ATOMIC_RELAXED, __HIP_MEMORY_SCOPE_AGENT);
                        pr_done = w >> 16; pr_unf = w & 0xffff;
                    }
                }
                if (s_stop) {
                    if (rank == 0 && tid == 0) *reinterpret_cast<volatile int*>(p.stop) = 1;
                    break;
                }
            }
            if (t == T) break;
            if (tid < NB * 16) {
                const int bb = b0 + erow, u = u0 + eu;
                const int id = tg == 0 ? p.V : (t == 0 ? p.ids_step[bb] : ids_l[erow]);
                const float* zr = p.tx + (long long)id * 4 * XU + u;
                float g[4];
#pragma unroll
                for (int q = 0; q < 4; ++q) g[q] = zr[q * XU];
                float cn, h;
                xdec_lstm(g, red, erow, eu, cst[erow][eu], cn, h);
                cst[erow][eu] = cn;
                p.cs[(sn + bb) * XU + u] = cn;
                float* rr = p.rec + (sn + bb) * p.REC;
                bf16_t* rb = p.recb + (sn + bb) * p.RECB;
                rr[OFF_H + u] = h; rr[OFF_HT + u] = h;
                const bf16_t htb = f2bf(h);
                rb[OFF_H + u] = htb; rb[OFF_HT + u] = htb;
                const unsigned mine = (unsigned)htb, other = (unsigned)__shfl_xor((int)mine, 1);
                if (!(eu & 1)) { const u32x2 wv = {mine | (other << 16), (unsigned)(t + 1)}; *reinterpret_cast<u32x2*>(ll_ht + ((bb * 256 + (u >> 1)) * 2)) = wv; }
            }
        }
        __syncthreads();
        xdec_p2<NB, true, false>(p, c, sp, sn, t, rll_ht, ll_ah, red, wahs);
        {
            float ah[4];
            xdec_att_h<true>(ah, c, ro.ab, rll_ah, (unsigned)(t + 1));
            float m = -3.0e38f, l = 0.f, acc[8];
#pragma unroll
            for (int e = 0; e < 8; ++e) acc[e] = 0.f;
            xdec_walk<ATT_U, true>(xiA, xaA, xiB, xaB, ro, tg & 1, ah, bt, m, l, acc, nullptr, lane);
            xdec_p3_publish<NQ, PP>(m, l, acc, c, ro.ab, ro.aq, t, p.part, wred, redc);
        }
        if constexpr (!PP) xbar(xsync, rank, ++ph, err, &s_dead);
#ifdef LXO_TEST_DEC_FAULT
        if (tg == 21 && xcc == 3u && tid == 0) { s_dead = 1; *reinterpret_cast<volatile unsigned*>(err) = 9u; }
#endif
        {
            u32x4 a[4];
            xdec_o_fetch(a, p, c, sn);
            xdec_p4_merge<NB, PP, false>(p, c, sn, t, wgt, nullptr, nullptr, redc, actx, nullptr);
            __syncthreads();
            xdec_o_proj<NB, 8>(a, p, c, sn, t, nullptr, wow, actx, red, ll_o);
        }
        __syncthreads();
    }
    if (tid == 0 && s_dead) *reinterpret_cast<volatile int*>(p.stop) = 1;
}

template <int NB, bool SC, bool PF, bool AL>
int launch_dec_sc(const XDecDec& p, hipStream_t st) { return xdec_launch<xdec_dec_kernel<NB, SC, PF, AL>>(p, st); }
template <int NB, bool PF, bool AL>
int launch_dec_pf(const XDecDec& p, hipStream_t st) { return p.logp_out ? launch_dec_sc<NB, true, PF, AL>(p, st) : launch_dec_sc<NB, false, PF, AL>(p, st); }
template <int NB, bool AL>
int launch_dec_al(const XDecDec& p, hipStream_t st) { return p.prefix ? launch_dec_pf<NB, true, AL>(p, st) : launch_dec_pf<NB, false, AL>(p, st); }
template <int NB>
int launch_dec_nb(const XDecDec& p, hipStream_t st) { return p.allow ? launch_dec_al<NB, true>(p, st) : launch_dec_al<NB, false>(p, st); }

template <int ATT_U>
LXO_DEV void attb_load(u32x4 (&xi)[ATT_U], u32x2 (&xa)[ATT_U], float (&al)[ATT_U], rsrc_t rim, rsrc_t rai, rsrc_t ral, int base, int an, int lane) {
#pragma unroll
    for (int u = 0; u < ATT_U; ++u) {
        const int r = max(min(base + XW * u, an - 1), 0);
        xi[u] = __builtin_amdgcn_raw_buffer_load_b128(rim, lane * 16, r * (XC * 2), 0);
        xa[u] = __builtin_amdgcn_raw_buffer_load_b64(rai, lane * 8, r * (XE * 2), 0);
        al[u] = __uint_as_float(__builtin_amdgcn_raw_buffer_load_b32(ral, 0, r * 4, 0));
    }
}
template <int ATT_U, bool EXPD>
LXO_DEV void attb_block(const u32x4 (&xi)[ATT_U], const u32x2 (&xa)[ATT_U], const float (&al)[ATT_U], int base, int an, const float (&dc)[8],
                        const float (&ah)[4], float s, float (&acc)[4], float* de_row, int lane) {
    float pt[ATT_U];
#pragma unroll
    for (int u = 0; u < ATT_U; ++u) {
        float a = 0.f;
#pragma unroll
        for (int e = 0; e < 4; ++e) {
            a = fmaf(__uint_as_float(xi[u][e] << 16), dc[2 * e], a);
            a = fmaf(__uint_as_float(xi[u][e] & 0xffff0000u), dc[2 * e + 1], a);
        }
        pt[u] = a;
    }
    xsum_rows<ATT_U>(pt);
#pragma unroll
    for (int u = 0; u < ATT_U; ++u) {
        const int r = base + XW * u;
        if (r >= an) continue;
        const float d = al[u] * (pt[u] - s);
        if (lane == 0) de_row[r] = d;
        const float x0 = __uint_as_float(xa[u][0] << 16), x1 = __uint_as_float(xa[u][0] & 0xffff0000u);
        const float x2 = __uint_as_float(xa[u][1] << 16), x3 = __uint_as_float(xa[u][1] & 0xffff0000u);
        if constexpr (EXPD) {
            const float d4 = 4.f * d;
            const float r0 = __builtin_amdgcn_rcpf(fmaf(x0, ah[0], 1.f)), r1 = __builtin_amdgcn_rcpf(fmaf(x1, ah[1], 1.f));
            const float r2 = __builtin_amdgcn_rcpf(fmaf(x2, ah[2], 1.f)), r3 = __builtin_amdgcn_rcpf(fmaf(x3, ah[3], 1.f));
            acc[0] = fmaf(d4, fmaf(-r0, r0, r0), acc[0]); acc[1] = fmaf(d4, fmaf(-r1, r1, r1), acc[1]);
            acc[2] = fmaf(d4, fmaf(-r2, r2, r2), acc[2]); acc[3] = fmaf(d4, fmaf(-r3, r3, r3), acc[3]);
        } else {
            const float t0 = tanh_x(x0 + ah[0]), t1 = tanh_x(x1 + ah[1]), t2 = tanh_x(x2 + ah[2]), t3 = tanh_x(x3 + ah[3]);
            acc[0] = fmaf(d, 1.f - t0 * t0, acc[0]); acc[1] = fmaf(d, 1.f - t1 * t1, acc[1]);
            acc[2] = fmaf(d, 1.f - t2 * t2, acc[2]); acc[3] = fmaf(d, 1.f - t3 * t3, acc[3]);
        }
    }
}

template <int NB, int ATT_U, bool EXPD>
__global__ __launch_bounds__(512) void xdec_bwd_kernel(XDecBwd p) {
    constexpr int NQ = 32 / NB;
    constexpr int QS = 8 / NB;
    __shared__ float red[XW][8][32];
    __shared__ __attribute__((aligned(16))) float redc[XW][XE];
    __shared__ __attribute__((aligned(16))) bf16_t adh[16][XE + 8];
    __shared__ float cst[8][16];
    __shared__ int s_rank, s_dead;

    XChain c = xchain_ticket(p.sync, NB, &s_rank, &s_dead);
    const int tid = c.tid, lane = c.lane, wave = c.wave, r16 = c.r16, g4 = c.g4;
    for (int i = tid; i < 16 * (XE + 8); i += 512) (&adh[0][0])[i] = 0;
    if (tid < 128) (&cst[0][0])[tid] = 0.f;
    __syncthreads();
    if (!xchain_rank(c, &s_rank)) return;
    const int rank = c.rank, b0 = c.b0, arow = c.arow, u0 = rank * 16, n0 = rank * 32;
    const unsigned xcc = c.xcc;
    unsigned* xsync = c.xsync; unsigned* err = c.err;
    const int B = p.B, T = p.T;

    u32x4 wow[2][2], wahb, wk0[4];
    u32x4* wl = reinterpret_cast<u32x4*>(xdec_dyn_lds) + (wave * 12) * 64 + lane;
#pragma unroll
    for (int nt = 0; nt < 2; ++nt)
#pragma unroll
        for (int ks = 0; ks < 2; ++ks)
            wow[nt][ks] = *reinterpret_cast<const u32x4*>(p.Wow + (long long)(n0 + nt * 16 + r16) * p.ldow + wave * 64 + ks * 32 + g4 * 8);
    wahb = *reinterpret_cast<const u32x4*>(p.Wah + (long long)(u0 + r16) * p.ldah + wave * 32 + g4 * 8);
#pragma unroll
    for (int nt = 0; nt < 2; ++nt)
#pragma unroll
        for (int ks = 0; ks < 8; ++ks) {
            const u32x4 w = *reinterpret_cast<const u32x4*>(p.Wk + (long long)(n0 + nt * 16 + r16) * p.ldk + wave * 256 + ks * 32 + g4 * 8);
            const int f = nt * 8 + ks;
            if (f < 4) wk0[f] = w; else wl[(f - 4) * 64] = w;
        }
    float bt[4];
    { const f32x4 b4 = *reinterpret_cast<const f32x4*>(p.beta + lane * 4); bt[0] = b4[0]; bt[1] = b4[1]; bt[2] = b4[2]; bt[3] = b4[3]; }

    const XRole<ATT_U> ro = xdec_role<NB, ATT_U>(c, p.R, p.img, EXPD ? p.att_exp : p.att_img);
    const int ab = ro.ab, aq = ro.aq, ar0 = ro.ar0, an = ro.an, nblk = ro.nblk, anq = ro.anq;
    const rsrc_t imq = ro.imq, aiq = ro.aiq;
    Drop dr = p.dr;
    unsigned ph = 0;
    const long long al_off = an > 0 ? (long long)ab * p.Rp + ar0 : 0;
    u32x4 xiA[ATT_U], xiB[ATT_U]; u32x2 xaA[ATT_U], xaB[ATT_U]; float alA[ATT_U], alB[ATT_U];
    {
        const rsrc_t ral = make_rsrc(p.alpha + (long long)(T - 1) * B * p.Rp + al_off, (unsigned)anq * 4u);
        attb_load<ATT_U>(xiA, xaA, alA, imq, aiq, ral, ro.XBASE(0, (T - 1) & 1), anq, lane);
        attb_load<ATT_U>(xiB, xaB, alB, imq, aiq, ral, ro.XBASE(1, (T - 1) & 1), anq, lane);
    }
    f32x4 cx0, cx1, ahn;
    {
        const float* cp = p.rec + ((long long)T * B + ab) * p.REC + OFF_CTX + lane * 8;
        cx0 = *reinterpret_cast<const f32x4*>(cp); cx1 = *reinterpret_cast<const f32x4*>(cp + 4);
        ahn = *reinterpret_cast<const f32x4*>(p.atth + ((long long)(T - 1) * B + ab) * XE + lane * 4);
    }
    float lg[4], lcc = 0.f, lcp = 0.f, qd = 0.f, qo = 0.f;
#pragma unroll
    for (int q = 0; q < 4; ++q) lg[q] = 0.f;
    const int e3r = min(tid >> 4, NB - 1), e3u = tid & 15;
    const int e4r = min(tid >> 5, NB - 1), e4c = tid & 31;
    unsigned* ll_gb = p.sync + kXDecSyncBytes / 4 + kLLBwdGb / 4;
    unsigned* ll_dc = p.sync + kXDecSyncBytes / 4 + kLLBwdDctx / 4;
    const rsrc_t rll_gb = make_rsrc(ll_gb, (unsigned)B * 256u * 8u);
    const rsrc_t rll_dc = make_rsrc(ll_dc, (unsigned)B * XC * 8u);
    unsigned long long* dbg = p.dbg ? p.dbg + ((long long)(xcc * 32 + rank) * T) * 16 : nullptr;
    auto fwd_values = [&](int ts) {
        const long long sq = (long long)ts * B;
        const int tq = max(ts - 1, 0);
        const float* cp = p.rec + ((long long)(tq + 1) * B + ab) * p.REC + OFF_CTX + lane * 8;
        cx0 = *reinterpret_cast<const f32x4*>(cp); cx1 = *reinterpret_cast<const f32x4*>(cp + 4);
        ahn = *reinterpret_cast<const f32x4*>(p.atth + ((long long)tq * B + ab) * XE + lane * 4);
        const float* gr = p.gates + (sq + b0 + e3r) * 4 * XU + u0 + e3u;
#pragma unroll
        for (int q = 0; q < 4; ++q) lg[q] = gr[q * XU];
        lcc = p.cs[(sq + B + b0 + e3r) * XU + u0 + e3u];
        lcp = p.cs[(sq + b0 + e3r) * XU + u0 + e3u];
        const int nq4 = min(n0 + e4c, XO - 1);
        qd = p.dolog[((long long)tq * B + b0 + e4r) * XO + nq4];
        qo = p.rec[((long long)(tq + 1) * B + b0 + e4r) * p.REC + nq4];
    };
    auto prefetch_b = [&](int ts) {
        const int rv = ts & 1;
        const rsrc_t ralq = make_rsrc(p.alpha + (long long)ts * B * p.Rp + al_off, (unsigned)anq * 4u);
        attb_load<ATT_U>(xiA, xaA, alA, imq, aiq, ralq, wave + XW * ATT_U * (rv ? nblk - 1 : 0), anq, lane);
        attb_load<ATT_U>(xiB, xaB, alB, imq, aiq, ralq, wave + XW * ATT_U * (rv ? nblk - 2 : 1), anq, lane);
    };
    for (int t = T - 1; t >= 0; --t) {
        dr.t = t;
        XSTAMP(T - 1 - t, 0);
        const long long sp = (long long)t * B;
        const rsrc_t rdh = make_rsrc(p.dhc + sp * XHC, (unsigned)B * XHC * 4u);
        {
            const rsrc_t rg = make_rsrc(p.gb + sp * p.GBP, (unsigned)B * p.GBP * 2u);
            u32x4 a[2];
            if ((kLLB & 1) && t < T - 1) {
                u32x4 w[4];
                unsigned off[4];
#pragma unroll
                for (int j = 0; j < 4; ++j) off[j] = (unsigned)(((b0 + arow) * 256 + ((wave * 64 + (j >> 1) * 32 + g4 * 8) >> 1)) * 8 + (j & 1) * 16);
                ll_wait<4>(w, rll_gb, off, (unsigned)(t + 1), err, &s_dead);
#pragma unroll
                for (int ks = 0; ks < 2; ++ks) a[ks] = u32x4{w[2 * ks][0], w[2 * ks][2], w[2 * ks + 1][0], w[2 * ks + 1][2]};
            } else {
#pragma unroll
                for (int ks = 0; ks < 2; ++ks) a[ks] = l2_load16(rg, (unsigned)(((b0 + arow) * p.GBP + wave * 64 + ks * 32 + g4 * 8) * 2));
            }
            v4f acc[2] = {v4f{0.f, 0.f, 0.f, 0.f}, v4f{0.f, 0.f, 0.f, 0.f}};
#pragma unroll
            for (int ks = 0; ks < 2; ++ks) { acc[0] = mfma16(a[ks], wow[0][ks], acc[0]); acc[1] = mfma16(a[ks], wow[1][ks], acc[1]); }
            if (g4 * 4 < NB) {
#pragma unroll
                for (int nt = 0; nt < 2; ++nt)
#pragma unroll
                    for (int i = 0; i < 4; ++i) if (NB >= 4 || i < NB) red[wave][g4 * 4 + i][nt * 16 + r16] = acc[nt][i];
            }
            __syncthreads();
            if (tid < NB * 32) {
                float v = 0.f;
#pragma unroll
                for (int w = 0; w < XW; ++w) v += red[w][e4r][e4c];
                p.dhc[(sp + b0 + e4r) * XHC + n0 + e4c] = v;
                if ((kLLB & 2) && n0 >= XU) {
                    const u32x2 wv = {__float_as_uint(v), (unsigned)(t + 1)};
                    *reinterpret_cast<u32x2*>(ll_dc + (((b0 + e4r) * XC + (n0 - XU) + e4c) * 2)) = wv;
                }
            }
        }
        XSTAMP(T - 1 - t, 1);
        if (!(kLLB & 2)) xbar(xsync, rank, ++ph, err, &s_dead);
        XSTAMP(T - 1 - t, 2);
        {
            float dc[8], ah[4], acc[4] = {0.f, 0.f, 0.f, 0.f};
            if (kLLB & 2) {
                u32x4 w[4];
                unsigned off[4];
#pragma unroll
                for (int j = 0; j < 4; ++j) off[j] = (unsigned)((ab * XC + lane * 8 + 2 * j) * 8);
                ll_wait<4>(w, rll_dc, off, (unsigned)(t + 1), err, &s_dead);
#pragma unroll
                for (int e = 0; e < 8; ++e) dc[e] = __uint_as_float(w[e >> 1][(e & 1) * 2]);
            } else {
                const u32x4 d0 = l2_load16(rdh, (unsigned)((ab * XHC + XU + lane * 8) * 4)), d1 = l2_load16(rdh, (unsigned)((ab * XHC + XU + lane * 8 + 4) * 4));
#pragma unroll
                for (int e = 0; e < 4; ++e) { dc[e] = __uint_as_float(d0[e]); dc[4 + e] = __uint_as_float(d1[e]); }
            }
            float s = 0.f;
#pragma unroll
            for (int e = 0; e < 4; ++e) s = fmaf(cx0[e], dc[e], fmaf(cx1[e], dc[4 + e], s));
            { float sv[1] = {s}; xsum_rows<1>(sv); s = sv[0]; }
#pragma unroll
            for (int j = 0; j < 4; ++j) {
                ah[j] = ahn[j];
                if constexpr (EXPD) ah[j] = __builtin_amdgcn_exp2f(fminf(fmaxf(ah[j] * 2.8853900817779268f, -60.f), 60.f));
            }
            float* de_row = p.de + (sp + ab) * p.Rp + ar0;
            const int rev = t & 1;
            const int tn = max(t - 1, 0);
            const rsrc_t ral = make_rsrc(p.alpha + sp * p.Rp + al_off, (unsigned)anq * 4u);
            const rsrc_t raln = make_rsrc(p.alpha + (long long)tn * B * p.Rp + al_off, (unsigned)anq * 4u);
            if constexpr (kPFB == 0) {
            for (int it = 0; it < nblk; it += 2) {
                const bool moreA = it + 2 < nblk, moreB = it + 3 < nblk;
                attb_block<ATT_U, EXPD>(xiA, xaA, alA, ro.XBASE(it, rev), an, dc, ah, s, acc, de_row, lane);
                __builtin_amdgcn_sched_barrier(0);
                attb_load<ATT_U>(xiA, xaA, alA, imq, aiq, moreA ? ral : raln, moreA ? ro.XBASE(it + 2, rev) : ro.XBASE(0, rev ^ 1), anq, lane);
                __builtin_amdgcn_sched_barrier(0);
                if (it + 1 < nblk) {
                    attb_block<ATT_U, EXPD>(xiB, xaB, alB, ro.XBASE(it + 1, rev), an, dc, ah, s, acc, de_row, lane);
                    __builtin_amdgcn_sched_barrier(0);
                    attb_load<ATT_U>(xiB, xaB, alB, imq, aiq, moreB ? ral : raln, moreB ? ro.XBASE(it + 3, rev) : ro.XBASE(1, rev ^ 1), anq, lane);
                    __builtin_amdgcn_sched_barrier(0);
                }
            }
            } else {
            int it = 0;
            for (; it + 3 < nblk; it += 2) {
                attb_block<ATT_U, EXPD>(xiA, xaA, alA, ro.XBASE(it, rev), an, dc, ah, s, acc, de_row, lane);
                __builtin_amdgcn_sched_barrier(0);
                attb_load<ATT_U>(xiA, xaA, alA, imq, aiq, ral, ro.XBASE(it + 2, rev), anq, lane);
                __builtin_amdgcn_sched_barrier(0);
                attb_block<ATT_U, EXPD>(xiB, xaB, alB, ro.XBASE(it + 1, rev), an, dc, ah, s, acc, de_row, lane);
                __builtin_amdgcn_sched_barrier(0);
                attb_load<ATT_U>(xiB, xaB, alB, imq, aiq, ral, ro.XBASE(it + 3, rev), anq, lane);
                __builtin_amdgcn_sched_barrier(0);
            }
            const int rem = nblk - it;
            if (rem >= 1) attb_block<ATT_U, EXPD>(xiA, xaA, alA, ro.XBASE(it, rev), an, dc, ah, s, acc, de_row, lane);
            if (rem == 3) { __builtin_amdgcn_sched_barrier(0); attb_load<ATT_U>(xiA, xaA, alA, imq, aiq, ral, ro.XBASE(it + 2, rev), anq, lane); __builtin_amdgcn_sched_barrier(0); }
            if (rem >= 2) attb_block<ATT_U, EXPD>(xiB, xaB, alB, ro.XBASE(it + 1, rev), an, dc, ah, s, acc, de_row, lane);
            if (rem == 3) attb_block<ATT_U, EXPD>(xiA, xaA, alA, ro.XBASE(it + 2, rev), an, dc, ah, s, acc, de_row, lane);
            }
            fwd_values(t);
#pragma unroll
            for (int j = 0; j < 4; ++j) redc[wave][lane * 4 + j] = acc[j] * bt[j];
            __syncthreads();
            if (tid < XE) {
                float v = 0.f;
#pragma unroll
                for (int w = 0; w < XW; ++w) v += redc[w][tid];
                if constexpr (kLLB & 4) {
                    const float other = __shfl_xor(v, 1);
                    if (!(tid & 1)) *reinterpret_cast<u32x2*>(reinterpret_cast<unsigned*>(p.part) + (((long long)ab * NQ + aq) * (XE / 2) + (tid >> 1)) * 2) = pack28(v, other, tag8_of(t));
                } else p.part[((long long)ab * NQ + aq) * XE + tid] = v;
            }
        }
        XSTAMP(T - 1 - t, 3);
        if constexpr (!(kLLB & 4)) xbar(xsync, rank, ++ph, err, &s_dead);
        XSTAMP(T - 1 - t, 4);
        {
            const rsrc_t rpart = make_rsrc(p.part + (long long)b0 * NQ * XE, (unsigned)(NB * NQ * XE) * 4u);
            const rsrc_t rcar = make_rsrc(p.carry_h, (unsigned)B * XU * 4u);
            const int srow = wave / QS, sqg = wave - srow * QS;
            u32x4 pc[4];
            if constexpr (kLLB & 4) {
                unsigned off[4];
#pragma unroll
                for (int j = 0; j < 4; ++j) off[j] = (unsigned)((((srow * NQ + sqg * 4 + j) * (XE / 2)) + lane * 2) * 8);
                ll_wait8<4>(pc, rpart, off, tag8_of(t), err, &s_dead);
                XSTAMP(T - 1 - t, 12);
            } else {
#pragma unroll
            for (int j = 0; j < 4; ++j) pc[j] = l2_load16(rpart, (unsigned)((((srow * NQ + sqg * 4 + j) * XE) + lane * 4) * 4));
            }
            const float dhm = l2_load4(rdh, (unsigned)(((b0 + e3r) * XHC + u0 + e3u) * 4));
            const float chv = l2_load4(rcar, (unsigned)(((b0 + e3r) * XU + u0 + e3u) * 4));
            {
                f32x4 v;
                if constexpr (kLLB & 4) {
#pragma unroll
                    for (int h = 0; h < 2; ++h) {
                        v[2 * h] = (unpack28_lo(pc[0][2 * h]) + unpack28_lo(pc[1][2 * h])) + (unpack28_lo(pc[2][2 * h]) + unpack28_lo(pc[3][2 * h]));
                        v[2 * h + 1] = (unpack28_hi(pc[0][2 * h], pc[0][2 * h + 1]) + unpack28_hi(pc[1][2 * h], pc[1][2 * h + 1])) + (unpack28_hi(pc[2][2 * h], pc[2][2 * h + 1]) + unpack28_hi(pc[3][2 * h], pc[3][2 * h + 1]));
                    }
                } else {
#pragma unroll
                for (int e = 0; e < 4; ++e) v[e] = (__uint_as_float(pc[0][e]) + __uint_as_float(pc[1][e])) + (__uint_as_float(pc[2][e]) + __uint_as_float(pc[3][e]));
                }
                *reinterpret_cast<f32x4*>(&redc[wave][lane * 4]) = v;
            }
            __syncthreads();
            if (kPFB == 1 && t > 0) prefetch_b(t - 1);
            if (tid < NB * 64) {
                const int row = tid >> 6, k4 = (tid & 63) * 4;
                f32x4 v = *reinterpret_cast<const f32x4*>(&redc[row * QS][k4]);
#pragma unroll
                for (int g = 1; g < QS; ++g) { const f32x4 w = *reinterpret_cast<const f32x4*>(&redc[row * QS + g][k4]); v += w; }
                const u32x2 vb = {pack_bf2(v[0], v[1]), pack_bf2(v[2], v[3])};
                *reinterpret_cast<u32x2*>(&adh[row][k4]) = vb;
                if (rank == row) {
                    *reinterpret_cast<f32x4*>(p.datth + (sp + b0 + row) * XE + k4) = v;
                    if (p.datthb) *reinterpret_cast<u32x2*>(p.datthb + (sp + b0 + row) * XE + k4) = vb;
                }
            }
            __syncthreads();
            const u32x4 a = *reinterpret_cast<const u32x4*>(&adh[r16][wave * 32 + g4 * 8]);
            v4f acc = v4f{0.f, 0.f, 0.f, 0.f};
            acc = mfma16(a, wahb, acc);
            if (g4 * 4 < NB) {
#pragma unroll
                for (int i = 0; i < 4; ++i) if (NB >= 4 || i < NB) red[wave][g4 * 4 + i][r16] = acc[i];
            }
            __syncthreads();
            if (tid < NB * 16) {
                float v = 0.f;
#pragma unroll
                for (int w = 0; w < XW; ++w) v += red[w][e3r][e3u];
                const int bb = b0 + e3r, u = u0 + e3u;
                const float dh = (dhm + v) * drop_scale(dr, 1u, bb, u, XU) + (t == T - 1 ? 0.f : chv);
                const float tc = tanh_x(lcc);
                const float dcv = cst[e3r][e3u] + dh * lg[3] * (1.f - tc * tc);
                const float dzi = dcv * lg[1] * lg[0] * (1.f - lg[0]);
                const float dzj = dcv * lg[0] * (1.f - lg[1] * lg[1]);
                const float dzf = dcv * lcp * lg[2] * (1.f - lg[2]);
                const float dzo = dh * tc * lg[3] * (1.f - lg[3]);
                cst[e3r][e3u] = dcv * lg[2];
                float* dzr = p.dz + (sp + bb) * 4 * XU + u;
                dzr[0] = dzi; dzr[XU] = dzj; dzr[2 * XU] = dzf; dzr[3 * XU] = dzo;
                bf16_t* db = p.dzb + (sp + bb) * p.DZBP + u;
                db[0] = f2bf(dzi); db[XU] = f2bf(dzj); db[2 * XU] = f2bf(dzf); db[3 * XU] = f2bf(dzo);
            }
        }
        XSTAMP(T - 1 - t, 5);
        xbar(xsync, rank, ++ph, err, &s_dead);
        XSTAMP(T - 1 - t, 6);
        {
            const rsrc_t rdz = make_rsrc(p.dzb + sp * p.DZBP, (unsigned)B * p.DZBP * 2u);
            u32x4 a[8];
#pragma unroll
            for (int ks = 0; ks < 8; ++ks) a[ks] = l2_load16(rdz, (unsigned)(((b0 + arow) * p.DZBP + wave * 256 + ks * 32 + g4 * 8) * 2));
            v4f acc[2] = {v4f{0.f, 0.f, 0.f, 0.f}, v4f{0.f, 0.f, 0.f, 0.f}};
#pragma unroll
            for (int ks = 0; ks < 8; ++ks) {
                acc[0] = mfma16(a[ks], ks < 4 ? wk0[ks < 4 ? ks : 0] : wl[(ks - 4) * 64], acc[0]);
                acc[1] = mfma16(a[ks], wl[(8 + ks - 4) * 64], acc[1]);
            }
            if (g4 * 4 < NB) {
#pragma unroll
                for (int nt = 0; nt < 2; ++nt)
#pragma unroll
                    for (int i = 0; i < 4; ++i) if (NB >= 4 || i < NB) red[wave][g4 * 4 + i][nt * 16 + r16] = acc[nt][i];
            }
            __syncthreads();
            if (kPFB == 3 && t > 0) prefetch_b(t - 1);
            if (tid < NB * 32) {
                float v = 0.f;
#pragma unroll
                for (int w = 0; w < XW; ++w) v += red[w][e4r][e4c];
                const int bb = b0 + e4r, n = n0 + e4c;
                if (t == 0) p.dxh[(long long)bb * XXH + n] = v;
                else if (n < XO) {
                    Drop dq = dr; dq.t = t - 1;
                    const float sc = drop_scale(dq, 2u, bb, n, XO);
                    const float th = (dq.thr == 0u) ? qo : qo / dq.inv_keep;
                    const float g = (qd + v) * sc * (1.f - th * th);
                    p.gall[(sp - B + bb) * XO + n] = g;
                    const bf16_t gbv = f2bf(g);
                    p.gb[(sp - B + bb) * p.GBP + n] = gbv;
                    if (kLLB & 1) {
                        const unsigned mine = (unsigned)gbv, other = (unsigned)__shfl_xor((int)mine, 1);
                        if (!(e4c & 1)) { const u32x2 wv = {mine | (other << 16), (unsigned)t}; *reinterpret_cast<u32x2*>(ll_gb + ((bb * 256 + (n >> 1)) * 2)) = wv; }
                    }
                } else p.carry_h[(long long)bb * XU + (n - XO)] = v;
            }
        }
        XSTAMP(T - 1 - t, 7);
        if (kLLB & 1) __syncthreads();
        else xbar(xsync, rank, ++ph, err, &s_dead);
        XSTAMP(T - 1 - t, 8);
    }
    if (tid < NB * 16) p.dcc[(long long)(b0 + e3r) * XU + u0 + e3u] = cst[e3r][e3u];
}

template <int NB>
int launch_bwd_nb(const XDecBwd& p, hipStream_t st) {
    return p.att_exp ? xdec_launch<xdec_bwd_kernel<NB, 4, true>>(p, st) : xdec_launch<xdec_bwd_kernel<NB, 4, false>>(p, st);
}
}

static int xdec_gate(int& on, const char* own, int U, int O, int C, int E, int B, int R, int rows_max) {
    if (on < 0) { const char* e = own ? getenv(own) : nullptr; const char* f = getenv("LXO_XDEC"); on = ((e && e[0] == '0') || (f && f[0] == '0')) ? 0 : 1; }
    if (!on) return 0;
    if (U != XU || O != XO || C != XC || E != XE) return 0;
    if (B % 8 != 0 || B > 64) return 0;
    const int nb = B / 8;
    if (nb != 1 && nb != 2 && nb != 4 && nb != 8) return 0;
    const int nq = 32 / nb, rows_per = (R + nq - 1) / nq;
    if (rows_per > rows_max || rows_per < 1) return 0;
    static int dev_ok = -1;
    if (dev_ok < 0) {
        int dev = 0; hipDeviceProp_t pr;
        dev_ok = (hipGetDevice(&dev) == hipSuccess && hipGetDeviceProperties(&pr, dev) == hipSuccess && pr.multiProcessorCount == 256) ? 1 : 0;
    }
    return dev_ok ? nb : 0;
}

static thread_local unsigned long long* g_xdbg = nullptr;
extern "C" int lxo_xdec_debug(unsigned long long* buf) { g_xdbg = buf; return 0; }
int lxo_launch_xdec_fwd(const XDecFwd& p0, int U, int O, int C, int E, hipStream_t st) {
    XDecFwd p = p0;
    p.dbg = g_xdbg;
    static int on = -1;
    const int nb = xdec_gate(on, nullptr, U, O, C, E, p.B, p.R, SCMAX);
    if (!nb || p.T < 1) return -2;
    if ((long long)p.B * p.RECB * 2 >= (1LL << 31) || p.ldrt % 8 || p.ldah % 8 || p.ldow % 8 || p.RECB % 8) return -2;
    HIPRC(hipMemsetAsync(p.sync, 0, kXDecBlockBytes, st));
    if (kLL & 4) HIPRC(hipMemsetAsync(p.part, 0, (size_t)p.B * (32 / nb) * PLW * 8, st));

    static int forced = -1;
    if (forced < 0) { const char* e = getenv("LXO_XDEC_U"); forced = e ? atoi(e) : 0; }
    int att_u = 4;
    if (forced >= 4 && forced <= 7) att_u = forced;
    switch (nb) {
    case 1: return launch_nb<1>(p, att_u, st);
    case 2: return launch_nb<2>(p, att_u, st);
    case 4: return launch_nb<4>(p, att_u, st);
    default: return launch_nb<8>(p, att_u, st);
    }
}
int lxo_launch_xdec_dec(const XDecDec& p, int U, int O, int C, int E, hipStream_t st) {
    static int on = -1;
    const int nb = xdec_gate(on, "LXO_XDEC_DEC", U, O, C, E, p.B, p.R, 1 << 30);
    if (!nb || p.nsteps < 1 || p.nsteps > 16 || p.V < 1 || p.V > 512 || !p.stop) return -2;
    if ((long long)p.B * p.RECB * 2 >= (1LL << 31) || p.ldrt % 8 || p.ldah % 8 || p.ldow % 8 || p.ldyo % 8 || p.RECB % 8 || !p.att_exp) return -2;
    HIPRC(hipMemsetAsync(p.sync, 0, 8 * 64 * 4, st));
    HIPRC(hipMemsetAsync(p.sync + 8 * 64 + 1, 0, kXDecBlockBytes - (8 * 64 + 1) * 4, st));
    HIPRC(hipMemsetAsync(p.sync + kXDecBlockBytes / 4 + kXDecSyncBytes / 4, 0, (size_t)p.B * 32 * 8 * (p.logp_out ? (p.prefix ? 3 : 2) : 1), st));
    if (kLL & 4) HIPRC(hipMemsetAsync(p.part, 0, (size_t)p.B * (32 / nb) * PLW * 8, st));
    switch (nb) {
    case 1: return launch_dec_nb<1>(p, st);
    case 2: return launch_dec_nb<2>(p, st);
    case 4: return launch_dec_nb<4>(p, st);
    default: return launch_dec_nb<8>(p, st);
    }
}
static thread_local unsigned long long* g_xdbg_b = nullptr;
extern "C" int lxo_xdec_debug_bwd(unsigned long long* buf) { g_xdbg_b = buf; return 0; }
int lxo_launch_xdec_bwd(const XDecBwd& p0, int U, int O, int C, int E, hipStream_t st) {
    XDecBwd p = p0;
    p.dbg = g_xdbg_b;
    static int on = -1;
    const int nb = xdec_gate(on, "LXO_XDEC_BWD", U, O, C, E, p.B, p.R, SCMAX);
    if (!nb || p.T < 1) return -2;
    if (p.ldow % 8 || p.ldah % 8 || p.ldk % 8 || p.GBP % 8 || p.DZBP % 8 || p.REC % 4 || (long long)p.B * p.DZBP * 2 >= (1LL << 31)) return -2;
    HIPRC(hipMemsetAsync(p.sync, 0, kXDecBlockBytes, st));
    if (kLLB & 4) HIPRC(hipMemsetAsync(p.part, 0, (size_t)p.B * (32 / nb) * XE * 4, st));
    switch (nb) {
    case 1: return launch_bwd_nb<1>(p, st);
    case 2: return launch_bwd_nb<2>(p, st);
    case 4: return launch_bwd_nb<4>(p, st);
    default: return launch_bwd_nb<8>(p, st);
    }
}
#endif
```

Baseline: 8674.

## Fuse small launches: ticketed CE loss reduce, merged memsets, poison in tanh_bwd

Several unrelated launch-reduction changes land together. The CE loss kernel now does its deterministic final reduction in the last block via an atomic ticket, replacing the separate det_reduce launch and the loss memset. The chain-poison check moves into tanh_bwd, the two xdec memsets become one zeroing kernel, and the three init dense projections are fused into a single rstep launch. The backward xdec kernel also stages alpha and de through shared memory instead of per-block buffer loads and stores. Together these add last-block ticket logic and more shared-memory use, which must stay correct across calls.

```diff
diff --git a/latex_ocr_amd/csrc/decoder_kernels.h b/latex_ocr_amd/csrc/decoder_kernels.h
--- a/latex_ocr_amd/csrc/decoder_kernels.h
+++ b/latex_ocr_amd/csrc/decoder_kernels.h
@@ -11,7 +11,8 @@
 int lxo_k_lstm_fwd(const float* z, Slabs zs, const float* c_prev, float* gates, float* c_out, float* h_out, float* ht_out, int ldh, Drop dr, int B, int U, hipStream_t st);
 int lxo_k_lstm_bwd(const float* gates, const float* c_prev, const float* c_cur, Slabs s1, Slabs s3, Slabs s4, int off4,
                    float* dcc, float* dz, Drop dr, int carry_rows, int B, int U, hipStream_t st);
-int lxo_k_tanh_bwd(const float* a, int lda, Slabs carry, const float* o, int ldo, float* g, int ldg, void* gb, int ldgb, Drop dr, int carry_rows, int rows, int cols, hipStream_t st);
+int lxo_k_tanh_bwd(const float* a, int lda, Slabs carry, const float* o, int ldo, float* g, int ldg, void* gb, int ldgb, Drop dr, int carry_rows, int rows, int cols, hipStream_t st,
+                   const unsigned* poison_err = nullptr, float* poison_probe = nullptr);
 int lxo_k_slab_reduce(Slabs sl, float* o, int ldo, int rows, int cols, hipStream_t st);
 int lxo_k_tanh_finalize(Slabs sl, float* o, int ldo, Drop dr, int rows, int cols, hipStream_t st);
 int lxo_k_attn_fwd(int dt, const void* att_img, const void* img, const float* att_h, Slabs ahs, float* att_h_out, const float* beta, float* alpha, float* part,
@@ -24,7 +25,7 @@
                    int T, int B, int R, int Rp, int E, DetScratch det, hipStream_t st);
 int lxo_k_add_mean_grad(float* dimg, const float* dmean, int B, int R, int C, hipStream_t st);
 int lxo_k_ce_loss(int dt, const float* logits, const int* formula, const int* lengths, void* dlogits, float* loss_acc, float inv_ntok,
-                  const float* ntok_dev, const unsigned* chain_err, int B, int T, int V, int Vp, DetScratch det, hipStream_t st);
+                  const float* ntok_dev, const unsigned* chain_err, unsigned* ticket, int B, int T, int V, int Vp, DetScratch det, hipStream_t st);
 int lxo_k_score(int dt, const float* logits, const int* formula, const int* lengths, float* logp_out, int* top1_out, float* seq_out,
                 const unsigned* chain_err, int B, int T, int V, int Vp, hipStream_t st);
 int lxo_k_colsum_det(const void* a, int bf16, long long lda, float* out, long long M, int N, DetScratch det, hipStream_t st);
diff --git a/latex_ocr_amd/csrc/decoder_kernels.hip b/latex_ocr_amd/csrc/decoder_kernels.hip
--- a/latex_ocr_amd/csrc/decoder_kernels.hip
+++ b/latex_ocr_amd/csrc/decoder_kernels.hip
@@ -214,7 +214,9 @@
 
 __global__ __launch_bounds__(256) void tanh_bwd_kernel(const float* __restrict__ a, int lda, Slabs carry,
                                                       const float* __restrict__ o, int ldo, float* __restrict__ g, int ldg,
-                                                      bf16_t* __restrict__ gb, int ldgb, Drop dr, int carry_rows, int rows, int cols) {
+                                                      bf16_t* __restrict__ gb, int ldgb, Drop dr, int carry_rows, int rows, int cols,
+                                                      const unsigned* __restrict__ poison_err, float* __restrict__ poison_probe) {
+    if (poison_err && blockIdx.x == 0 && threadIdx.x == 0 && poison_err[0]) poison_probe[0] = __uint_as_float(0x7fc00000u);
     const int total = rows * (cols >> 2);
     for (int i = blockIdx.x * 256 + threadIdx.x; i < total; i += gridDim.x * 256) {
         const int r = i / (cols >> 2), c = (i - r * (cols >> 2)) << 2;
@@ -1083,13 +1085,58 @@
     }
 }
 
+LXO_DEV float det_reduce_tree(const float* part, int nslot, long long stride, int N, int n, float (*gs)[16]) {
+    const int c = threadIdx.x & 15, g = threadIdx.x >> 4;
+    const int per = (nslot + 15) / 16;
+    const int q0 = g * per, q1 = min(nslot, q0 + per);
+    float s = 0.f;
+    if (n < N) {
+        for (int q = q0; q < q1; q += 8) {
+            float v[8];
+#pragma unroll
+            for (int u = 0; u < 8; ++u) v[u] = part[(long long)min(q + u, q1 - 1) * stride + n];
+#pragma unroll
+            for (int u = 0; u < 8; ++u) if (q + u < q1) s += v[u];
+        }
+    }
+    gs[g][c] = s;
+    __syncthreads();
+    float tsum = 0.f;
+    if (g == 0 && n < N) {
+        tsum = gs[0][c];
+#pragma unroll
+        for (int k = 1; k < 16; ++k) tsum += gs[k][c];
+    }
+    return tsum;
+}
+LXO_DEV void ce_loss_finish(float* loss_part, float* loss_acc, unsigned* ticket, const unsigned* chain_err) {
+    __shared__ float gs[16][16];
+    __shared__ int s_last;
+    if (threadIdx.x == 0) {
+        __threadfence();
+        s_last = atomicAdd(ticket, 1u) == gridDim.x - 1 ? 1 : 0;
+    }
+    __syncthreads();
+    if (!s_last) return;
+    __threadfence();
+    const int n = threadIdx.x & 15;
+    const float tsum = det_reduce_tree(loss_part, (int)gridDim.x, 2, 2, n, gs);
+    if (threadIdx.x < 16) {
+        float v = 0.f;
+        if (n == 0 && chain_err && chain_err[0] != 0u) v += __uint_as_float(0x7fc00000u);
+        if (n < 2) v += tsum;
+        loss_acc[n] = v;
+    }
+    if (threadIdx.x == 0) *ticket = 0u;
+}
+
 template <typename CT>
 __global__ __launch_bounds__(256) void ce_loss_kernel(const float* __restrict__ logits, const int* __restrict__ formula,
                                                      const int* __restrict__ lengths, CT* __restrict__ dlogits,
                                                      float* __restrict__ loss_acc, float* __restrict__ loss_part, float inv_ntok, const float* __restrict__ ntok_dev,
-                                                     const unsigned* __restrict__ chain_err, int B, int T, int V, int Vp) {
+                                                     const unsigned* __restrict__ chain_err, unsigned* __restrict__ ticket, int B, int T, int V, int Vp) {
     __shared__ float red[8];
-    if (chain_err && blockIdx.x == 0 && threadIdx.x == 0 && chain_err[0] != 0u) atomicAdd(&loss_acc[0], __uint_as_float(0x7fc00000u));
+    if (!ticket && chain_err && blockIdx.x == 0 && threadIdx.x == 0 && chain_err[0] != 0u) atomicAdd(&loss_acc[0], __uint_as_float(0x7fc00000u));
     if (ntok_dev) inv_ntok = 1.0f / ntok_dev[0];
     const int lane = threadIdx.x & 63, wave = threadIdx.x >> 6;
     float ce_sum = 0.f, n_sum = 0.f;
@@ -1122,15 +1169,16 @@
         if (loss_part) { loss_part[2 * blockIdx.x] = c; loss_part[2 * blockIdx.x + 1] = n; }
         else if (n > 0.f) { atomicAdd(&loss_acc[0], c); atomicAdd(&loss_acc[1], n); }
     }
+    if (ticket) ce_loss_finish(loss_part, loss_acc, ticket, chain_err);
 }
 
 template <typename CT, int KV>
 __global__ __launch_bounds__(256) void ce_loss_rows_kernel(const float* __restrict__ logits, const int* __restrict__ formula,
                                                           const int* __restrict__ lengths, CT* __restrict__ dlogits,
                                                           float* __restrict__ loss_acc, float* __restrict__ loss_part, float inv_ntok, const float* __restrict__ ntok_dev,
-                                                          const unsigned* __restrict__ chain_err, int B, int T, int V, int Vp) {
+                                                          const unsigned* __restrict__ chain_err, unsigned* __restrict__ ticket, int B, int T, int V, int Vp) {
     __shared__ float red[8];
-    if (chain_err && blockIdx.x == 0 && threadIdx.x == 0 && chain_err[0] != 0u) atomicAdd(&loss_acc[0], __uint_as_float(0x7fc00000u));
+    if (!ticket && chain_err && blockIdx.x == 0 && threadIdx.x == 0 && chain_err[0] != 0u) atomicAdd(&loss_acc[0], __uint_as_float(0x7fc00000u));
     if (ntok_dev) inv_ntok = 1.0f / ntok_dev[0];
     const int lane = threadIdx.x & 63, wave = threadIdx.x >> 6;
     float ce_sum = 0.f, n_sum = 0.f;
@@ -1183,6 +1231,7 @@
         if (loss_part) { loss_part[2 * blockIdx.x] = c; loss_part[2 * blockIdx.x + 1] = n; }
         else if (n > 0.f) { atomicAdd(&loss_acc[0], c); atomicAdd(&loss_acc[1], n); }
     }
+    if (ticket) ce_loss_finish(loss_part, loss_acc, ticket, chain_err);
 }
 
 __global__ __launch_bounds__(256) void colsum_kernel(const float* __restrict__ a, int lda, float* __restrict__ out, int M, int N, int rows_per_block) {
@@ -1235,28 +1284,9 @@
 }
 __global__ __launch_bounds__(256) void det_reduce_kernel(const float* __restrict__ part, int nslot, long long stride, int N, float* __restrict__ out) {
     __shared__ float gs[16][16];
-    const int c = threadIdx.x & 15, g = threadIdx.x >> 4;
-    const int n = blockIdx.x * 16 + c;
-    const int per = (nslot + 15) / 16;
-    const int q0 = g * per, q1 = min(nslot, q0 + per);
-    float s = 0.f;
-    if (n < N) {
-        for (int q = q0; q < q1; q += 8) {
-            float v[8];
-#pragma unroll
-            for (int u = 0; u < 8; ++u) v[u] = part[(long long)min(q + u, q1 - 1) * stride + n];
-#pragma unroll
-            for (int u = 0; u < 8; ++u) if (q + u < q1) s += v[u];
-        }
-    }
-    gs[g][c] = s;
-    __syncthreads();
-    if (g == 0 && n < N) {
-        float tsum = gs[0][c];
-#pragma unroll
-        for (int k = 1; k < 16; ++k) tsum += gs[k][c];
-        out[n] += tsum;
-    }
+    const int n = blockIdx.x * 16 + (threadIdx.x & 15);
+    const float tsum = det_reduce_tree(part, nslot, stride, N, n, gs);
+    if ((threadIdx.x >> 4) == 0 && n < N) out[n] += tsum;
 }
 
 __global__ __launch_bounds__(256) void embed_scatter_kernel(const float* __restrict__ demb, const int* __restrict__ formula,
@@ -1978,8 +2008,9 @@
     LAUNCH(lstm_bwd_kernel, grid1((long long)B * U), gates, c_prev, c_cur, s1, s3, s4, off4, dcc, dz, dr, carry_rows, B, U);
     DONE;
 }
-int lxo_k_tanh_bwd(const float* a, int lda, Slabs carry, const float* o, int ldo, float* g, int ldg, void* gb, int ldgb, Drop dr, int carry_rows, int rows, int cols, hipStream_t st) {
-    LAUNCH(tanh_bwd_kernel, grid1((long long)rows * cols / 4), a, lda, carry, o, ldo, g, ldg, (bf16_t*)gb, ldgb, dr, carry_rows, rows, cols);
+int lxo_k_tanh_bwd(const float* a, int lda, Slabs carry, const float* o, int ldo, float* g, int ldg, void* gb, int ldgb, Drop dr, int carry_rows, int rows, int cols, hipStream_t st,
+                   const unsigned* poison_err, float* poison_probe) {
+    LAUNCH(tanh_bwd_kernel, grid1((long long)rows * cols / 4), a, lda, carry, o, ldo, g, ldg, (bf16_t*)gb, ldgb, dr, carry_rows, rows, cols, poison_err, poison_probe);
     DONE;
 }
 __global__ __launch_bounds__(256) static void slab_reduce_kernel(Slabs sl, float* __restrict__ o, int ldo, int rows, int cols) {
@@ -2113,22 +2144,23 @@
     DONE;
 }
 int lxo_k_ce_loss(int dt, const float* logits, const int* formula, const int* lengths, void* dlogits, float* loss_acc, float inv_ntok,
-                  const float* ntok_dev, const unsigned* chain_err, int B, int T, int V, int Vp, DetScratch det, hipStream_t st) {
+                  const float* ntok_dev, const unsigned* chain_err, unsigned* ticket, int B, int T, int V, int Vp, DetScratch det, hipStream_t st) {
     int g = cdiv(T * B, 4);
     float* part = (det.p && det.floats >= 1024) ? det.p : nullptr;
+    if (!part) ticket = nullptr;
     if (Vp % 4 == 0 && Vp <= 1024 && (((uintptr_t)logits | (uintptr_t)dlogits) & 15) == 0) {
         if (g > (part ? 512 : 2048)) g = part ? 512 : 2048;
-#define CE_ROWS(CT_, KV_) LAUNCH((ce_loss_rows_kernel<CT_, KV_>), g, logits, formula, lengths, (CT_*)dlogits, loss_acc, part, inv_ntok, ntok_dev, chain_err, B, T, V, Vp)
+#define CE_ROWS(CT_, KV_) LAUNCH((ce_loss_rows_kernel<CT_, KV_>), g, logits, formula, lengths, (CT_*)dlogits, loss_acc, part, inv_ntok, ntok_dev, chain_err, ticket, B, T, V, Vp)
         if (dt == LXO_BF16) { if (Vp <= 256) CE_ROWS(bf16_t, 4); else if (Vp <= 512) CE_ROWS(bf16_t, 8); else CE_ROWS(bf16_t, 16); }
         else { if (Vp <= 256) CE_ROWS(float, 4); else if (Vp <= 512) CE_ROWS(float, 8); else CE_ROWS(float, 16); }
 #undef CE_ROWS
-        if (part) return lxo_k_det_reduce(part, g, 2, 2, loss_acc, st);
+        if (part && !ticket) return lxo_k_det_reduce(part, g, 2, 2, loss_acc, st);
         DONE;
     }
     if (g > 512) g = 512;
-    if (dt == LXO_BF16) LAUNCH((ce_loss_kernel<bf16_t>), g, logits, formula, lengths, (bf16_t*)dlogits, loss_acc, part, inv_ntok, ntok_dev, chain_err, B, T, V, Vp);
-    else LAUNCH((ce_loss_kernel<float>), g, logits, formula, lengths, (float*)dlogits, loss_acc, part, inv_ntok, ntok_dev, chain_err, B, T, V, Vp);
-    if (part) return lxo_k_det_reduce(part, g, 2, 2, loss_acc, st);
+    if (dt == LXO_BF16) LAUNCH((ce_loss_kernel<bf16_t>), g, logits, formula, lengths, (bf16_t*)dlogits, loss_acc, part, inv_ntok, ntok_dev, chain_err, ticket, B, T, V, Vp);
+    else LAUNCH((ce_loss_kernel<float>), g, logits, formula, lengths, (float*)dlogits, loss_acc, part, inv_ntok, ntok_dev, chain_err, ticket, B, T, V, Vp);
+    if (part && !ticket) return lxo_k_det_reduce(part, g, 2, 2, loss_acc, st);
     DONE;
 }
 int lxo_k_score(int dt, const float* logits, const int* formula, const int* lengths, float* logp_out, int* top1_out, float* seq_out,
diff --git a/latex_ocr_amd/csrc/model_decoder.hip b/latex_ocr_amd/csrc/model_decoder.hip
--- a/latex_ocr_amd/csrc/model_decoder.hip
+++ b/latex_ocr_amd/csrc/model_decoder.hip
@@ -55,6 +55,18 @@
     return lxo_launch_rstep(P.s.dtype, 0, a, st);
 }
 
+static int rs_dense3(const Plan& P, const float* A, int lda, const void* const (&W)[3], int ldw, float* const (&out)[3], const int (&ldo)[3],
+                     int M, int N, int K, const float* const (&bias)[3], bool tanh_act, hipStream_t st) {
+    RStep a; memset(&a, 0, sizeof(a));
+    a.M = M; a.N = N; a.K = K; a.U = P.s.U; a.O = P.s.O; a.zx_row = -1;
+    a.A = A; a.lda = lda; a.W = W[0]; a.ldw = ldw; a.out = out[0]; a.ldo = ldo[0]; a.bias = bias[0];
+    a.nz = 3;
+    for (int z = 0; z < 2; ++z) { a.Wz[z] = W[z + 1]; a.outz[z] = out[z + 1]; a.ldoz[z] = ldo[z + 1]; a.biasz[z] = bias[z + 1]; }
+    a.epi = tanh_act ? RS_TANH_O : RS_PLAIN;
+    a.dr.inv_keep = 1.f;
+    return lxo_launch_rstep(P.s.dtype, 0, a, st);
+}
+
 static int attention_prepare(const Plan& P, const float* prm, const void* wp, void* ws, int beam, hipStream_t st) {
     const int B = P.s.B, C = P.s.C, E = P.s.E, U = P.s.U, O = P.s.O;
     RC(nt(P, false, false, false, P.ws<void>(ws, W_IMG), C, P.pk(wp, K_ATT_IMG_T), C, P.ws<void>(ws, W_ATT_IMG), E,
@@ -64,7 +76,10 @@
     float* cs0 = P.ws<float>(ws, W_CS);
     const char* wt = (const char*)P.pk(wp, K_INIT_T);
     float* mean = P.ws<float>(ws, W_MEAN);
-    if (beam <= 1 && fused_steps(P)) {
+    if (beam <= 1 && fused_steps(P) && U == O) {
+        RC(rs_dense3(P, mean, C, {wt, wt + (size_t)U * C * P.esz, wt + (size_t)2 * U * C * P.esz}, C, {cs0, rec0 + O, rec0}, {U, P.REC, P.REC},
+                     B, U, C, {prm + P.poff[P_BC0], prm + P.poff[P_BH0], prm + P.poff[P_BO0]}, true, st));
+    } else if (beam <= 1 && fused_steps(P)) {
         RC(rs_dense(P, mean, C, wt, C, cs0, U, B, U, C, prm + P.poff[P_BC0], true, false, st));
         RC(rs_dense(P, mean, C, wt + (size_t)U * C * P.esz, C, rec0 + O, P.REC, B, U, C, prm + P.poff[P_BH0], true, false, st));
         RC(rs_dense(P, mean, C, wt + (size_t)2 * U * C * P.esz, C, rec0, P.REC, B, O, C, prm + P.poff[P_BO0], true, false, st));
@@ -253,9 +268,10 @@
 }
 
 int lxo_impl_ce_loss(const Plan& P, void* ws, const int* formula, const int* lengths, float inv_ntok, const float* ntok_dev, hipStream_t st) {
-    HIPRC(hipMemsetAsync(P.ws<float>(ws, W_LOSS), 0, 64, st));
+    unsigned* xs = P.bf ? P.ws<unsigned>(ws, W_XSYNC) : nullptr;
+    if (!xs) HIPRC(hipMemsetAsync(P.ws<float>(ws, W_LOSS), 0, 64, st));
     RC(lxo_k_ce_loss(P.s.dtype, P.ws<float>(ws, W_LOGITS), formula, lengths, P.ws<void>(ws, W_DLOGITS), P.ws<float>(ws, W_LOSS),
-                     inv_ntok, ntok_dev, P.bf ? P.ws<unsigned>(ws, W_XSYNC) + 8 * 64 : nullptr, P.s.B, P.s.T, P.s.V, P.Vp,
+                     inv_ntok, ntok_dev, xs ? xs + 8 * 64 : nullptr, xs ? xs + kXDecLossTicketWord : nullptr, P.s.B, P.s.T, P.s.V, P.Vp,
                      DetScratch{P.ws<float>(ws, W_DET), P.wbytes[W_DET] / 4}, st));
     return 0;
 }
@@ -288,7 +304,8 @@
         if (P.bf && fused) RC(tn(P, false, false, P.ws<bf16_t>(ws, W_RECB) + (size_t)B * P.RECB, P.RECB, dlog, P.Vp, gw(P_YWO), V, TB, O, V, st, det));
         else RC(tn(P, true, false, rec + (size_t)B * P.REC, P.REC, dlog, P.Vp, gw(P_YWO), V, TB, O, V, st));
     }
-    if ((parts & 1) && P.bf) RC(lxo_k_chain_poison(P.ws<unsigned>(ws, W_XSYNC) + 8 * 64, nullptr, grads + P.ptotal - 1, st));
+    const bool poison_in_tanh = (parts & 1) && (parts & 2) && P.bf && fused;
+    if ((parts & 1) && P.bf && !poison_in_tanh) RC(lxo_k_chain_poison(P.ws<unsigned>(ws, W_XSYNC) + 8 * 64, nullptr, grads + P.ptotal - 1, st));
     if (!(parts & 2)) return 0;
 
     const bool want_chain = fused && P.bf && P.s.step_kernels == 0;
@@ -310,7 +327,8 @@
         const char* img = (const char*)P.ws<void>(ws, W_IMG);
         const int t_last = T - 1, n_last = B;
         RC(lxo_k_tanh_bwd(dolog + (size_t)t_last * B * O, O, kNoSlabs, rec + (size_t)(t_last + 1) * B * P.REC, P.REC,
-                          gall + (size_t)t_last * B * O, O, bf ? gb + (size_t)t_last * B * P.GBP : nullptr, P.GBP, P.drop(t_last, 0), 0, n_last, O, st));
+                          gall + (size_t)t_last * B * O, O, bf ? gb + (size_t)t_last * B * P.GBP : nullptr, P.GBP, P.drop(t_last, 0), 0, n_last, O, st,
+                          poison_in_tanh ? P.ws<unsigned>(ws, W_XSYNC) + 8 * 64 : nullptr, grads + P.ptotal - 1));
         bool chain_done = false;
         if (want_chain) {
             XDecBwd x; memset(&x, 0, sizeof(x));
diff --git a/latex_ocr_amd/csrc/rstep.h b/latex_ocr_amd/csrc/rstep.h
--- a/latex_ocr_amd/csrc/rstep.h
+++ b/latex_ocr_amd/csrc/rstep.h
@@ -23,6 +23,7 @@
     const int* zx_idx; int zx_vocab, zx_row;
     const float* dhm; int lddhm; const float* carry_h; const float* gates_in; const float* c_cur; float* dcc; int carry_rows;
     const float* bias; int accumulate;
+    int nz; const void* Wz[2]; float* outz[2]; int ldoz[2]; const float* biasz[2];
     const float* dolog; const float* o_prev; int ldoprev; int first;
     Drop dr;
     unsigned long long* dbg;
diff --git a/latex_ocr_amd/csrc/rstep.hip b/latex_ocr_amd/csrc/rstep.hip
--- a/latex_ocr_amd/csrc/rstep.hip
+++ b/latex_ocr_amd/csrc/rstep.hip
@@ -46,6 +46,11 @@
     const int r = lane & 15, g = lane >> 4;
     const int m0 = blockIdx.y * MT;
     const int kq = k_K >> 2;
+    float* out_ = p.out; int ldo_ = p.ldo; const float* bias_ = p.bias;
+    if constexpr (EPI == RS_PLAIN || EPI == RS_TANH_O) {
+        if (blockIdx.z == 1) { kW = p.Wz[0]; out_ = p.outz[0]; ldo_ = p.ldoz[0]; bias_ = p.biasz[0]; }
+        else if (blockIdx.z == 2) { kW = p.Wz[1]; out_ = p.outz[1]; ldo_ = p.ldoz[1]; bias_ = p.biasz[1]; }
+    }
     WT* As = lds[wave];
     WT* Ws = lds[wave] + MT * PITCH;
     const AT* __restrict__ Ag = reinterpret_cast<const AT*>(kA) + wave * kq;
@@ -195,16 +200,16 @@
 #pragma unroll
         for (int e = 0; e < 4; ++e) v[e] = red[0][row][part * 4 + e] + red[1][row][part * 4 + e] + red[2][row][part * 4 + e] + red[3][row][part * 4 + e];
         if constexpr (EPI == RS_PLAIN || EPI == RS_TANH_O) {
-            if (p.bias) { float b4[4]; ld4(p.bias + n, b4); for (int e = 0; e < 4; ++e) v[e] += b4[e]; }
-            if (p.accumulate) { float o4[4]; ld4(p.out + (long long)m * p.ldo + n, o4); for (int e = 0; e < 4; ++e) v[e] += o4[e]; }
+            if (bias_) { float b4[4]; ld4(bias_ + n, b4); for (int e = 0; e < 4; ++e) v[e] += b4[e]; }
+            if (p.accumulate) { float o4[4]; ld4(out_ + (long long)m * ldo_ + n, o4); for (int e = 0; e < 4; ++e) v[e] += o4[e]; }
         }
         if constexpr (EPI == RS_PLAIN) {
-            st4(p.out + (long long)m * p.ldo + n, v);
+            st4(out_ + (long long)m * ldo_ + n, v);
             if (p.outb) st4b(p.outb + (long long)m * p.ldob + n, v);
         } else if constexpr (EPI == RS_TANH_O) {
 #pragma unroll
             for (int e = 0; e < 4; ++e) v[e] = tanh_e<BF>(v[e]) * drop_scale(p.dr, 2u, m, n + e, p.N);
-            st4(p.out + (long long)m * p.ldo + n, v);
+            st4(out_ + (long long)m * ldo_ + n, v);
             if (p.outb) st4b(p.outb + (long long)m * p.ldob + n, v);
         } else if constexpr (EPI == RS_LSTM_BWD) {
             const int U = p.U;
@@ -271,13 +276,14 @@
     static int q16 = -1;
     if (q16 < 0) { const char* e = getenv("LXO_RSTEP_MT16"); q16 = (e && e[0] == '0') ? 0 : 1; }
     const bool quarter = q16 && (long long)ncol * cdiv(p.M, 32) <= 128 && p.M > 16;
+    const int gz = p.nz > 1 ? p.nz : 1;
     if (kq % K0 == 0) {
-        if (quarter) return launch_nch<AT, WT, EPI, 16, K0>(p, dim3(ncol, cdiv(p.M, 16)), st);
-        if (half) return launch_nch<AT, WT, EPI, 32, K0>(p, dim3(ncol, cdiv(p.M, 32)), st);
-        return launch_nch<AT, WT, EPI, 64, K0>(p, dim3(ncol, cdiv(p.M, 64)), st);
+        if (quarter) return launch_nch<AT, WT, EPI, 16, K0>(p, dim3(ncol, cdiv(p.M, 16), gz), st);
+        if (half) return launch_nch<AT, WT, EPI, 32, K0>(p, dim3(ncol, cdiv(p.M, 32), gz), st);
+        return launch_nch<AT, WT, EPI, 64, K0>(p, dim3(ncol, cdiv(p.M, 64), gz), st);
     }
     if constexpr (K0 / 2 >= KMIN) {
-        if (kq % (K0 / 2) == 0) return launch_nch<AT, WT, EPI, 64, K0 / 2>(p, dim3(ncol, cdiv(p.M, 64)), st);
+        if (kq % (K0 / 2) == 0) return launch_nch<AT, WT, EPI, 64, K0 / 2>(p, dim3(ncol, cdiv(p.M, 64), gz), st);
     }
     return -2;
 }
@@ -309,6 +315,7 @@
     if (p.M <= 0 || p.N <= 0) return 0;
     if (p.K % 128 != 0 || p.lda % 8 != 0 || p.ldw % 8 != 0 || p.N % 4 != 0) return -2;
     if (p.epi == RS_LSTM_FWD && (p.U % 4 != 0 || p.N != 4 * p.U)) return -2;
+    if (p.nz > 1 && (p.nz > 3 || (p.epi != RS_PLAIN && p.epi != RS_TANH_O) || p.outb)) return -2;
     switch (p.epi) {
     case RS_PLAIN: return launch_epi<RS_PLAIN>(dt, a_bf16 != 0, p, st);
     case RS_TANH_O: return launch_epi<RS_TANH_O>(dt, a_bf16 != 0, p, st);
diff --git a/latex_ocr_amd/csrc/xdec.h b/latex_ocr_amd/csrc/xdec.h
--- a/latex_ocr_amd/csrc/xdec.h
+++ b/latex_ocr_amd/csrc/xdec.h
@@ -79,4 +79,5 @@
 int lxo_launch_xdec_bwd(const XDecBwd& p, int U, int O, int C, int E, hipStream_t st);
 constexpr size_t kXDecSyncBytes = 4096, kXDecLLBytes = 384u << 10, kXDecBlockBytes = kXDecSyncBytes + kXDecLLBytes;
 constexpr size_t kLLFwdHt = 0, kLLFwdAh = 128u << 10, kLLFwdO = 256u << 10;
+constexpr int kXDecLossTicketWord = 8 * 64 + 16;
 constexpr size_t kLLBwdGb = 0, kLLBwdDctx = 128u << 10;
diff --git a/latex_ocr_amd/csrc/xdec.hip b/latex_ocr_amd/csrc/xdec.hip
--- a/latex_ocr_amd/csrc/xdec.hip
+++ b/latex_ocr_amd/csrc/xdec.hip
@@ -1025,18 +1025,15 @@
 int launch_dec_nb(const XDecDec& p, hipStream_t st) { return p.allow ? launch_dec_al<NB, true>(p, st) : launch_dec_al<NB, false>(p, st); }
 
 template <int ATT_U>
-LXO_DEV void attb_load(u32x4 (&xi)[ATT_U], u32x2 (&xa)[ATT_U], float (&al)[ATT_U], rsrc_t rim, rsrc_t rai, rsrc_t ral, int base, int an, int lane) {
-#pragma unroll
-    for (int u = 0; u < ATT_U; ++u) {
-        const int r = max(min(base + XW * u, an - 1), 0);
-        xi[u] = __builtin_amdgcn_raw_buffer_load_b128(rim, lane * 16, r * (XC * 2), 0);
-        xa[u] = __builtin_amdgcn_raw_buffer_load_b64(rai, lane * 8, r * (XE * 2), 0);
-        al[u] = __uint_as_float(__builtin_amdgcn_raw_buffer_load_b32(ral, 0, r * 4, 0));
-    }
+LXO_DEV int attb_alpha_slot(int r) {
+    const int q = r % (XW * ATT_U);
+    return r - q + (q % XW) * ATT_U + q / XW;
 }
 template <int ATT_U, bool EXPD>
-LXO_DEV void attb_block(const u32x4 (&xi)[ATT_U], const u32x2 (&xa)[ATT_U], const float (&al)[ATT_U], int base, int an, const float (&dc)[8],
-                        const float (&ah)[4], float s, float (&acc)[4], float* de_row, int lane) {
+LXO_DEV void attb_block(const u32x4 (&xi)[ATT_U], const u32x2 (&xa)[ATT_U], const float* als, int base, int an, const float (&dc)[8],
+                        const float (&ah)[4], float s, float (&acc)[4], float* des, int lane) {
+    static_assert(ATT_U == 4, "one 16-byte LDS read carries a wave's alpha values of a block");
+    const f32x4 al = *reinterpret_cast<const f32x4*>(als + (base - base % XW) + (base % XW) * ATT_U);
     float pt[ATT_U];
 #pragma unroll
     for (int u = 0; u < ATT_U; ++u) {
@@ -1054,7 +1051,7 @@
         const int r = base + XW * u;
         if (r >= an) continue;
         const float d = al[u] * (pt[u] - s);
-        if (lane == 0) de_row[r] = d;
+        if (lane == 0) des[r] = d;
         const float x0 = __uint_as_float(xa[u][0] << 16), x1 = __uint_as_float(xa[u][0] & 0xffff0000u);
         const float x2 = __uint_as_float(xa[u][1] << 16), x3 = __uint_as_float(xa[u][1] & 0xffff0000u);
         if constexpr (EXPD) {
@@ -1079,6 +1076,8 @@
     __shared__ __attribute__((aligned(16))) float redc[XW][XE];
     __shared__ __attribute__((aligned(16))) bf16_t adh[16][XE + 8];
     __shared__ float cst[8][16];
+    __shared__ __attribute__((aligned(16))) float als[SCMAX];
+    __shared__ float des[SCMAX];
     __shared__ int s_rank, s_dead;
 
     XChain c = xchain_ticket(p.sync, NB, &s_rank, &s_dead);
@@ -1117,11 +1116,22 @@
     Drop dr = p.dr;
     unsigned ph = 0;
     const long long al_off = an > 0 ? (long long)ab * p.Rp + ar0 : 0;
-    u32x4 xiA[ATT_U], xiB[ATT_U]; u32x2 xaA[ATT_U], xaB[ATT_U]; float alA[ATT_U], alB[ATT_U];
+    float alq = 0.f;
+    auto alpha_request = [&](int ts) {
+        const rsrc_t ral = make_rsrc(p.alpha + (long long)ts * B * p.Rp + al_off, (unsigned)anq * 4u);
+        alq = __uint_as_float(__builtin_amdgcn_raw_buffer_load_b32(ral, tid * 4, 0, 0));
+    };
+    auto alpha_stage = [&](int ts) {
+        if (tid < an) als[attb_alpha_slot<ATT_U>(tid)] = alq;
+        const float* ap = p.alpha + (long long)ts * B * p.Rp + al_off;
+#pragma unroll 1
+        for (int i = tid + 512; i < an; i += 512) als[attb_alpha_slot<ATT_U>(i)] = ap[i];
+    };
+    u32x4 xiA[ATT_U], xiB[ATT_U]; u32x2 xaA[ATT_U], xaB[ATT_U];
+    alpha_request(T - 1);
     {
-        const rsrc_t ral = make_rsrc(p.alpha + (long long)(T - 1) * B * p.Rp + al_off, (unsigned)anq * 4u);
-        attb_load<ATT_U>(xiA, xaA, alA, imq, aiq, ral, ro.XBASE(0, (T - 1) & 1), anq, lane);
-        attb_load<ATT_U>(xiB, xaB, alB, imq, aiq, ral, ro.XBASE(1, (T - 1) & 1), anq, lane);
+        att_load<ATT_U>(xiA, xaA, imq, aiq, ro.XBASE(0, (T - 1) & 1), anq, lane);
+        att_load<ATT_U>(xiB, xaB, imq, aiq, ro.XBASE(1, (T - 1) & 1), anq, lane);
     }
     f32x4 cx0, cx1, ahn;
     {
@@ -1129,6 +1139,7 @@
         cx0 = *reinterpret_cast<const f32x4*>(cp); cx1 = *reinterpret_cast<const f32x4*>(cp + 4);
         ahn = *reinterpret_cast<const f32x4*>(p.atth + ((long long)(T - 1) * B + ab) * XE + lane * 4);
     }
+    alpha_stage(T - 1);
     float lg[4], lcc = 0.f, lcp = 0.f, qd = 0.f, qo = 0.f;
 #pragma unroll
     for (int q = 0; q < 4; ++q) lg[q] = 0.f;
@@ -1156,9 +1167,8 @@
     };
     auto prefetch_b = [&](int ts) {
         const int rv = ts & 1;
-        const rsrc_t ralq = make_rsrc(p.alpha + (long long)ts * B * p.Rp + al_off, (unsigned)anq * 4u);
-        attb_load<ATT_U>(xiA, xaA, alA, imq, aiq, ralq, wave + XW * ATT_U * (rv ? nblk - 1 : 0), anq, lane);
-        attb_load<ATT_U>(xiB, xaB, alB, imq, aiq, ralq, wave + XW * ATT_U * (rv ? nblk - 2 : 1), anq, lane);
+        att_load<ATT_U>(xiA, xaA, imq, aiq, wave + XW * ATT_U * (rv ? nblk - 1 : 0), anq, lane);
+        att_load<ATT_U>(xiB, xaB, imq, aiq, wave + XW * ATT_U * (rv ? nblk - 2 : 1), anq, lane);
     };
     for (int t = T - 1; t >= 0; --t) {
         dr.t = t;
@@ -1189,6 +1199,7 @@
 #pragma unroll
                     for (int i = 0; i < 4; ++i) if (NB >= 4 || i < NB) red[wave][g4 * 4 + i][nt * 16 + r16] = acc[nt][i];
             }
+            if (t < T - 1) alpha_stage(t);
             __syncthreads();
             if (tid < NB * 32) {
                 float v = 0.f;
@@ -1228,42 +1239,38 @@
                 ah[j] = ahn[j];
                 if constexpr (EXPD) ah[j] = __builtin_amdgcn_exp2f(fminf(fmaxf(ah[j] * 2.8853900817779268f, -60.f), 60.f));
             }
-            float* de_row = p.de + (sp + ab) * p.Rp + ar0;
             const int rev = t & 1;
-            const int tn = max(t - 1, 0);
-            const rsrc_t ral = make_rsrc(p.alpha + sp * p.Rp + al_off, (unsigned)anq * 4u);
-            const rsrc_t raln = make_rsrc(p.alpha + (long long)tn * B * p.Rp + al_off, (unsigned)anq * 4u);
             if constexpr (kPFB == 0) {
             for (int it = 0; it < nblk; it += 2) {
                 const bool moreA = it + 2 < nblk, moreB = it + 3 < nblk;
-                attb_block<ATT_U, EXPD>(xiA, xaA, alA, ro.XBASE(it, rev), an, dc, ah, s, acc, de_row, lane);
+                attb_block<ATT_U, EXPD>(xiA, xaA, als, ro.XBASE(it, rev), an, dc, ah, s, acc, des, lane);
                 __builtin_amdgcn_sched_barrier(0);
-                attb_load<ATT_U>(xiA, xaA, alA, imq, aiq, moreA ? ral : raln, moreA ? ro.XBASE(it + 2, rev) : ro.XBASE(0, rev ^ 1), anq, lane);
+                att_load<ATT_U>(xiA, xaA, imq, aiq, moreA ? ro.XBASE(it + 2, rev) : ro.XBASE(0, rev ^ 1), anq, lane);
                 __builtin_amdgcn_sched_barrier(0);
                 if (it + 1 < nblk) {
-                    attb_block<ATT_U, EXPD>(xiB, xaB, alB, ro.XBASE(it + 1, rev), an, dc, ah, s, acc, de_row, lane);
+                    attb_block<ATT_U, EXPD>(xiB, xaB, als, ro.XBASE(it + 1, rev), an, dc, ah, s, acc, des, lane);
                     __builtin_amdgcn_sched_barrier(0);
-                    attb_load<ATT_U>(xiB, xaB, alB, imq, aiq, moreB ? ral : raln, moreB ? ro.XBASE(it + 3, rev) : ro.XBASE(1, rev ^ 1), anq, lane);
+                    att_load<ATT_U>(xiB, xaB, imq, aiq, moreB ? ro.XBASE(it + 3, rev) : ro.XBASE(1, rev ^ 1), anq, lane);
                     __builtin_amdgcn_sched_barrier(0);
                 }
             }
             } else {
             int it = 0;
             for (; it + 3 < nblk; it += 2) {
-                attb_block<ATT_U, EXPD>(xiA, xaA, alA, ro.XBASE(it, rev), an, dc, ah, s, acc, de_row, lane);
+                attb_block<ATT_U, EXPD>(xiA, xaA, als, ro.XBASE(it, rev), an, dc, ah, s, acc, des, lane);
                 __builtin_amdgcn_sched_barrier(0);
-                attb_load<ATT_U>(xiA, xaA, alA, imq, aiq, ral, ro.XBASE(it + 2, rev), anq, lane);
+                att_load<ATT_U>(xiA, xaA, imq, aiq, ro.XBASE(it + 2, rev), anq, lane);
                 __builtin_amdgcn_sched_barrier(0);
-                attb_block<ATT_U, EXPD>(xiB, xaB, alB, ro.XBASE(it + 1, rev), an, dc, ah, s, acc, de_row, lane);
+                attb_block<ATT_U, EXPD>(xiB, xaB, als, ro.XBASE(it + 1, rev), an, dc, ah, s, acc, des, lane);
                 __builtin_amdgcn_sched_barrier(0);
-                attb_load<ATT_U>(xiB, xaB, alB, imq, aiq, ral, ro.XBASE(it + 3, rev), anq, lane);
+                att_load<ATT_U>(xiB, xaB, imq, aiq, ro.XBASE(it + 3, rev), anq, lane);
                 __builtin_amdgcn_sched_barrier(0);
             }
             const int rem = nblk - it;
-            if (rem >= 1) attb_block<ATT_U, EXPD>(xiA, xaA, alA, ro.XBASE(it, rev), an, dc, ah, s, acc, de_row, lane);
-            if (rem == 3) { __builtin_amdgcn_sched_barrier(0); attb_load<ATT_U>(xiA, xaA, alA, imq, aiq, ral, ro.XBASE(it + 2, rev), anq, lane); __builtin_amdgcn_sched_barrier(0); }
-            if (rem >= 2) attb_block<ATT_U, EXPD>(xiB, xaB, alB, ro.XBASE(it + 1, rev), an, dc, ah, s, acc, de_row, lane);
-            if (rem == 3) attb_block<ATT_U, EXPD>(xiA, xaA, alA, ro.XBASE(it + 2, rev), an, dc, ah, s, acc, de_row, lane);
+            if (rem >= 1) attb_block<ATT_U, EXPD>(xiA, xaA, als, ro.XBASE(it, rev), an, dc, ah, s, acc, des, lane);
+            if (rem == 3) { __builtin_amdgcn_sched_barrier(0); att_load<ATT_U>(xiA, xaA, imq, aiq, ro.XBASE(it + 2, rev), anq, lane); __builtin_amdgcn_sched_barrier(0); }
+            if (rem >= 2) attb_block<ATT_U, EXPD>(xiB, xaB, als, ro.XBASE(it + 1, rev), an, dc, ah, s, acc, des, lane);
+            if (rem == 3) attb_block<ATT_U, EXPD>(xiA, xaA, als, ro.XBASE(it + 2, rev), an, dc, ah, s, acc, des, lane);
             }
             fwd_values(t);
 #pragma unroll
@@ -1315,6 +1322,11 @@
             }
             __syncthreads();
             if (kPFB == 1 && t > 0) prefetch_b(t - 1);
+            {
+                float* de_row = p.de + (sp + ab) * p.Rp + ar0;
+#pragma unroll 1
+                for (int i = tid; i < an; i += 512) de_row[i] = des[i];
+            }
             if (tid < NB * 64) {
                 const int row = tid >> 6, k4 = (tid & 63) * 4;
                 f32x4 v = *reinterpret_cast<const f32x4*>(&redc[row * QS][k4]);
@@ -1377,6 +1389,7 @@
             }
             __syncthreads();
             if (kPFB == 3 && t > 0) prefetch_b(t - 1);
+            if (t > 0) alpha_request(t - 1);
             if (tid < NB * 32) {
                 float v = 0.f;
 #pragma unroll
@@ -1429,6 +1442,25 @@
     return dev_ok ? nb : 0;
 }
 
+namespace {
+__global__ __launch_bounds__(256) void xdec_zero2_kernel(u32x4* __restrict__ a, unsigned na, u32x4* __restrict__ b, unsigned nb) {
+    const u32x4 z = {0u, 0u, 0u, 0u};
+    for (unsigned i = blockIdx.x * 256 + threadIdx.x; i < na + nb; i += gridDim.x * 256) {
+        if (i < na) a[i] = z; else b[i - na] = z;
+    }
+}
+int xdec_zero2(void* a, size_t abytes, void* b, size_t bbytes, hipStream_t st) {
+    if (((uintptr_t)a | (uintptr_t)b | abytes | bbytes) & 15) {
+        HIPRC(hipMemsetAsync(a, 0, abytes, st));
+        if (bbytes) HIPRC(hipMemsetAsync(b, 0, bbytes, st));
+        return 0;
+    }
+    const unsigned na = (unsigned)(abytes / 16), nb = (unsigned)(bbytes / 16);
+    hipLaunchKernelGGL(xdec_zero2_kernel, dim3(min(cdiv((int)(na + nb), 256), 1024)), dim3(256), 0, st, (u32x4*)a, na, (u32x4*)b, nb);
+    return (int)hipGetLastError();
+}
+}
+
 static thread_local unsigned long long* g_xdbg = nullptr;
 extern "C" int lxo_xdec_debug(unsigned long long* buf) { g_xdbg = buf; return 0; }
 int lxo_launch_xdec_fwd(const XDecFwd& p0, int U, int O, int C, int E, hipStream_t st) {
@@ -1438,8 +1470,7 @@
     const int nb = xdec_gate(on, nullptr, U, O, C, E, p.B, p.R, SCMAX);
     if (!nb || p.T < 1) return -2;
     if ((long long)p.B * p.RECB * 2 >= (1LL << 31) || p.ldrt % 8 || p.ldah % 8 || p.ldow % 8 || p.RECB % 8) return -2;
-    HIPRC(hipMemsetAsync(p.sync, 0, kXDecBlockBytes, st));
-    if (kLL & 4) HIPRC(hipMemsetAsync(p.part, 0, (size_t)p.B * (32 / nb) * PLW * 8, st));
+    RC(xdec_zero2(p.sync, kXDecBlockBytes, p.part, (kLL & 4) ? (size_t)p.B * (32 / nb) * PLW * 8 : 0, st));
 
     static int forced = -1;
     if (forced < 0) { const char* e = getenv("LXO_XDEC_U"); forced = e ? atoi(e) : 0; }
@@ -1477,8 +1508,7 @@
     const int nb = xdec_gate(on, "LXO_XDEC_BWD", U, O, C, E, p.B, p.R, SCMAX);
     if (!nb || p.T < 1) return -2;
     if (p.ldow % 8 || p.ldah % 8 || p.ldk % 8 || p.GBP % 8 || p.DZBP % 8 || p.REC % 4 || (long long)p.B * p.DZBP * 2 >= (1LL << 31)) return -2;
-    HIPRC(hipMemsetAsync(p.sync, 0, kXDecBlockBytes, st));
-    if (kLLB & 4) HIPRC(hipMemsetAsync(p.part, 0, (size_t)p.B * (32 / nb) * XE * 4, st));
+    RC(xdec_zero2(p.sync, kXDecBlockBytes, p.part, (kLLB & 4) ? (size_t)p.B * (32 / nb) * XE * 4 : 0, st));
     switch (nb) {
     case 1: return launch_bwd_nb<1>(p, st);
     case 2: return launch_bwd_nb<2>(p, st);
```

Result: no change. 8733, median of 6 (+0.7%).
